# yassram/iterative-closest-point

Measured on AMD Instinct MI355X. Metric: ICP iterations/sec (synthetic 1048576-point pair, C4, exact NN), higher is better.
Workload: dtype f64 (30 exact fp64 grid searches (fp32 screen, candidates decided in fp64: the first from cell seeds, the seeded ones the fused grid iteration nn_grid_iter2_kernel, 75% of its queries kept their correspondence by the exclusion certificate without a walk); fp64 transform and reductions)

## Files before the change

### include/icp_capi.h

```cpp
#ifndef ICP_CAPI_H
#define ICP_CAPI_H

#include <stddef.h>
#include <stdint.h>

#ifdef __cplusplus
extern "C" {
#endif

#define ICP_OK 0
#define ICP_E_ARG (-1)
#define ICP_E_HIP (-2)
#define ICP_E_SIZE_MISMATCH (-3)
#define ICP_E_TOO_FEW_POINTS (-4)
#define ICP_E_NO_MODEL (-5)
#define ICP_E_RCCL (-6)
#define ICP_E_NO_DEVICE (-7)
#define ICP_E_IO (-8)
#define ICP_E_RANGE (-9)

#define ICP_NN_CERTIFIED 0
#define ICP_NN_FP64 1

#define ICP_NN_VARIANT_AUTO 0
#define ICP_NN_VARIANT_VALU 1
#define ICP_NN_VARIANT_MFMA 2
#define ICP_NN_VARIANT_MFMA16 3
#define ICP_NN_VARIANT_GRID 4
#define ICP_NN_VARIANT_BUNDLE 5

typedef struct icp_ctx icp_ctx;

typedef struct icp_result {
    int iterations;
    int converged;
    double err;
    double s;
    double R[9];
    double t[3];
} icp_result;

typedef struct icp_stats {
    double nn_ms;
    long long nn_launches;
    long long nn_pairs;
    long long ambiguous;
    long long level1_queued;
    long long level1_unrecovered;
    double iter_ms;
    long long iterations;
    long long grid_fallback;
    double allreduce_ms;
    long long allreduce_calls;
    double cert_max_err_ratio;
    double cert_min_margin;
    long long cert_audited;
    long long persistent_runs;
    long long cpu_rule_ties;
    long long cpu_rule_changed;
    long long persistent_fallbacks;
    int last_filter;
    long long bundle_builds;
    long long bundle_builds_in_run;
    long long run_bundle_searches;
    long long run_grid_searches;
    long long run_certified;
    long long run_walked;
    unsigned long long run_path_bits;
} icp_stats;
#define ICP_FILTER_VALU 0
#define ICP_FILTER_MFMA 1
#define ICP_FILTER_MFMA16 2
#define ICP_FILTER_BUNDLE 3
#define ICP_FILTER_GRID 4
#define ICP_FILTER_FP64 5
#define ICP_FILTER_ONE_LAUNCH 6

int icp_ctx_create(int device, int nn_mode, icp_ctx **out);

int icp_ctx_create_dist(int device, int nn_mode, int rank, int world_size, const void *rccl_id,
                        icp_ctx **out);
int icp_rccl_unique_id(void *out128);
typedef int (*icp_allreduce_fn)(double *buf, size_t count, void *user);
int icp_ctx_create_sharded(int device, int nn_mode, int rank, int world_size, icp_allreduce_fn fn,
                           void *user, icp_ctx **out);
void icp_ctx_destroy(icp_ctx *ctx);
const char *icp_last_error(const icp_ctx *ctx);
const char *icp_strerror(int code);
int icp_device_count(int *count);

int icp_set_model(icp_ctx *ctx, const double *m_xyz, size_t nm);
int icp_set_scene(icp_ctx *ctx, const double *p_xyz, size_t np_local, size_t np_total);
int icp_set_model_device(icp_ctx *ctx, const double *m_xyz_dev, size_t nm);
int icp_set_scene_device(icp_ctx *ctx, const double *p_xyz_dev, size_t np_local, size_t np_total);
int icp_set_model_device_stream(icp_ctx *ctx, const double *m_xyz_dev, size_t nm, void *producer);
int icp_set_scene_device_stream(icp_ctx *ctx, const double *p_xyz_dev, size_t np_local, size_t np_total,
                                void *producer);
int icp_get_scene(icp_ctx *ctx, double *p_xyz_out);
int icp_ensure_model(icp_ctx *ctx, const double *m_xyz, size_t nm, int *uploaded);
typedef void (*icp_progress_fn)(int iteration, double err, void *user);
int icp_set_progress(icp_ctx *ctx, icp_progress_fn fn, void *user);
int icp_set_allow_unequal(icp_ctx *ctx, int allow);
int icp_set_nn_variant(icp_ctx *ctx, int variant);
#define ICP_NN_RULE_SQUARED 0
#define ICP_NN_RULE_CPU_SQRT 1
int icp_set_nn_rule(icp_ctx *ctx, int rule);

#define ICP_RUN_AUTO 0
#define ICP_RUN_LAUNCHES 1
#define ICP_RUN_PERSISTENT 2
int icp_set_run_mode(icp_ctx *ctx, int mode);

int icp_set_max_distance(icp_ctx *ctx, double dmax);
int icp_get_inliers(icp_ctx *ctx, uint8_t *mask_out, long long *count_out);
int icp_get_inlier_trace(icp_ctx *ctx, long long *counts_out, size_t cap);

int icp_run(icp_ctx *ctx, int max_iter, double threshold, double *err_trace, icp_result *res);

int icp_closest_matrix(icp_ctx *ctx, const double *p_xyz, size_t np, double *y_xyz_out,
                       int32_t *idx_out);
int icp_compute_centroid(icp_ctx *ctx, const double *xyz, size_t n, double mu[3],
                         double *centred_out);
int icp_subtract_col(icp_ctx *ctx, const double *xyz, size_t n, const double m[3], double *out);
int icp_y_p_norm(icp_ctx *ctx, const double *y_xyz, const double *p_xyz, size_t n,
                 double *d_caps, double *sp);
int icp_err_compute(icp_ctx *ctx, const double *y_xyz, double *p_xyz, size_t n, int in_place,
                    const double sR[9], const double t[3], double *err);
int icp_find_alignment(icp_ctx *ctx, const double *p_xyz, const double *y_xyz, size_t n,
                       double *s, double R[9], double t[3], double *err);

int icp_horn_solve(const double S[9], const double mu_p[3], const double mu_y[3], double d_caps,
                   double sp, double *s, double R[9], double t[3]);
int icp_max_element_index(const double ev[4]);
int icp_shard_range(size_t n_total, int rank, int world_size, size_t *begin, size_t *count);
int icp_synthetic_pair(uint64_t seed, size_t n, double angle_deg, const double axis[3],
                       const double t[3], double *model_xyz_out, double *scene_xyz_out);
int icp_load_matrix(const char *path, double **xyz_out, size_t *n_out);
int icp_write_matrix(const char *path, const double *xyz, size_t n);
void icp_free(void *p);

int icp_get_indices(icp_ctx *ctx, int32_t *idx_out);
int icp_set_index_digest(icp_ctx *ctx, size_t cap);
int icp_set_cert_audit(icp_ctx *ctx, int enable);
typedef struct icp_bundle_audit_result {
    double max_err_ratio;
    double min_gap;
    long long pairs, excluded, checked, violations;
} icp_bundle_audit_result;
int icp_bundle_audit(icp_ctx *ctx, int groups, icp_bundle_audit_result *out);
int icp_get_index_digest(icp_ctx *ctx, uint64_t *out, size_t cap);

int icp_get_stats(const icp_ctx *ctx, icp_stats *out);
int icp_reset_stats(icp_ctx *ctx);
int icp_set_bundle_counters(icp_ctx *ctx, int enable);
int icp_get_bundle_counters(icp_ctx *ctx, uint64_t out[16]);
int icp_get_comm_info(icp_ctx *ctx, int *comm_count, int *comm_rank, char *bus_id, int len);
int icp_get_model_order(icp_ctx *ctx, int32_t *kd_out);
int icp_sort_pairs(int device, const uint32_t *keys, size_t n, int bits, uint32_t *keys_out, int32_t *order_out);

#ifdef __cplusplus
}
#endif
#endif
```

### iterative-closest-point_amd/csrc/icp_engine.hip

```cpp
#include <hip/hip_runtime.h>
#include <rccl/rccl.h>

#include <algorithm>
#include <chrono>
#include <thread>
#include <cmath>
#include <cstdio>
#include <climits>
#include <cstring>
#include <string>
#include <vector>

#include "icp_horn.h"
#include "icp_canon.h"
#include "icp_kernels.h"

using namespace icp;

std::vector<double> icp::persist_model_image(const double *m, size_t nm, size_t *blocks_out)
{
    std::vector<uint32_t> ord(nm);
    for (size_t j = 0; j < nm; ++j) ord[j] = (uint32_t)j;
    std::vector<std::pair<size_t, size_t>> stack{{0, nm}};
    while (!stack.empty()) {
        const auto [lo, hi] = stack.back();
        stack.pop_back();
        const size_t cnt = hi - lo;
        const size_t unit = cnt > 1024 ? 1024 : cnt > 64 ? 64 : cnt > 16 ? 16 : 0;
        if (!unit) continue;
        double bl[3] = {INFINITY, INFINITY, INFINITY}, bh[3] = {-INFINITY, -INFINITY, -INFINITY};
        for (size_t k = lo; k < hi; ++k)
            for (int a = 0; a < 3; ++a) {
                bl[a] = std::min(bl[a], m[3 * ord[k] + a]);
                bh[a] = std::max(bh[a], m[3 * ord[k] + a]);
            }
        int ax = 0;
        for (int a = 1; a < 3; ++a)
            if (bh[a] - bl[a] > bh[ax] - bl[ax]) ax = a;
        const size_t units = (cnt + unit - 1) / unit, mid = lo + unit * ((units + 1) / 2);
        if (mid >= hi) continue;
        std::nth_element(ord.begin() + lo, ord.begin() + mid, ord.begin() + hi, [&](uint32_t x, uint32_t y) {
            const double vx = m[3 * x + ax], vy = m[3 * y + ax];
            return vx < vy || (vx == vy && x < y);
        });
        stack.push_back({lo, mid});
        stack.push_back({mid, hi});
    }
    const size_t nb = (nm + 63) / 64;
    const size_t nsb = (nb + 15) / 16, nb16 = (nm + 15) / 16;
    const size_t nf32 = 6 * (nb + nb16);
    std::vector<double> img(3 * nm + 6 * nb + (nm + 1) / 2 + 6 * nsb + (nf32 + 1) / 2);
    int32_t *orig = (int32_t *)(img.data() + 3 * nm + 6 * nb);
    for (size_t k = 0; k < nm; ++k) {
        const size_t j = ord[k];
        for (int a = 0; a < 3; ++a) img[a * nm + k] = m[3 * j + a];
        orig[k] = (int32_t)j;
    }
    for (size_t b = 0; b < nb; ++b) {
        double *box = img.data() + 3 * nm + 6 * b;
        for (int a = 0; a < 3; ++a) {
            box[a] = img[a * nm + 64 * b];
            box[3 + a] = box[a];
        }
        for (size_t k = 64 * b + 1; k < std::min(nm, 64 * b + 64); ++k)
            for (int a = 0; a < 3; ++a) {
                box[a] = std::min(box[a], img[a * nm + k]);
                box[3 + a] = std::max(box[3 + a], img[a * nm + k]);
            }
    }
    double *sbox = img.data() + 3 * nm + 6 * nb + (nm + 1) / 2;
    for (size_t s = 0; s < nsb; ++s) {
        const double *first = img.data() + 3 * nm + 6 * (16 * s);
        for (int a = 0; a < 6; ++a) sbox[6 * s + a] = first[a];
        for (size_t b = 16 * s + 1; b < std::min(nb, 16 * s + 16); ++b) {
            const double *box = img.data() + 3 * nm + 6 * b;
            for (int a = 0; a < 3; ++a) {
                sbox[6 * s + a] = std::min(sbox[6 * s + a], box[a]);
                sbox[6 * s + 3 + a] = std::max(sbox[6 * s + 3 + a], box[3 + a]);
            }
        }
    }
    float *f32 = (float *)(sbox + 6 * nsb);
    auto down = [](double v) {
        float f = (float)v;
        return (double)f > v ? std::nextafter(f, -INFINITY) : f;
    };
    auto up = [](double v) {
        float f = (float)v;
        return (double)f < v ? std::nextafter(f, INFINITY) : f;
    };
    for (size_t b = 0; b < nb; ++b)
        for (int a = 0; a < 3; ++a) {
            f32[6 * b + a] = down(img[3 * nm + 6 * b + a]);
            f32[6 * b + 3 + a] = up(img[3 * nm + 6 * b + 3 + a]);
        }
    float *f16b = f32 + 6 * nb;
    for (size_t b = 0; b < nb16; ++b)
        for (int a = 0; a < 3; ++a) {
            double lo = img[a * nm + 16 * b], hi = lo;
            for (size_t k = 16 * b + 1; k < std::min(nm, 16 * b + 16); ++k) {
                lo = std::min(lo, img[a * nm + k]);
                hi = std::max(hi, img[a * nm + k]);
            }
            f16b[6 * b + a] = down(lo);
            f16b[6 * b + 3 + a] = up(hi);
        }
    *blocks_out = nb;
    return img;
}

namespace {

struct DevCloud {
    double *x = nullptr, *y = nullptr, *z = nullptr;
    float4 *f = nullptr;
    size_t n = 0, cap = 0;
};

}

struct icp_ctx {
    int device = 0;
    int nn_mode = ICP_NN_CERTIFIED;
    int rank = 0, world = 1;
    bool allow_unequal = false;
    hipStream_t st = nullptr;
    ncclComm_t comm = nullptr;
    icp_allreduce_fn host_reduce = nullptr;
    void *host_reduce_user = nullptr;
    icp_progress_fn progress_fn = nullptr;
    void *progress_user = nullptr;
    int progress_next = 0;

    DevCloud model;
    float4 *m32 = nullptr;
    float4 *mperm = nullptr;
    float *mm = nullptr;
    char *mimg16 = nullptr;
    bool mimg16_pending = false;
    float *mms16 = nullptr;
    double scale16 = 1.0;
    size_t nm = 0, nm_pad = 0, m32_cap = 0, mperm_cap = 0, mm_cap = 0, mimg16_cap = 0, mms16_cap = 0;
    int nn_variant = ICP_NN_VARIANT_AUTO;
    double c[3] = {0, 0, 0};
    std::vector<double> model_host;
    double rm = 0.0;
    double *mstat_part = nullptr, *mstat_out = nullptr, *h_mstat = nullptr;
    int *cmp_diff = nullptr;
    KdPlan kd_plan;
    char *kd_scratch = nullptr;
    size_t kd_scratch_cap = 0;
    bool has_model = false;

    DevCloud scene, Y;
    size_t np_total = 0;
    bool has_scene = false;

    DevCloud qa, qb;

    int *idx = nullptr;
    size_t idx_cap = 0;
    void *part = nullptr, *part2 = nullptr;
    size_t part_cap = 0, part2_cap = 0;
    int *amb1 = nullptr;
    size_t amb1_cap = 0;
    int *amb_count = nullptr, *amb_list = nullptr;
    double *amb_T = nullptr;
    size_t amb_cap = 0;
    GridParams grid{};
    int *g_start = nullptr;
    char *g_sort = nullptr;
    size_t g_sort_cap = 0;
    double4 *g_pts = nullptr;
    float4 *g_pts32 = nullptr;
    size_t g_pts32_cap = 0;
    size_t g_start_cap = 0, g_pts_cap = 0;
    IterState *iter_state = nullptr;
    size_t iter_state_cap = 0;
    IterState *h_iter = nullptr;
    IterState *d_iter_mirror = nullptr;
    double *h_trace = nullptr, *d_trace = nullptr;
    size_t trace_cap = 0;
    int *h_sig = nullptr, *d_sig = nullptr;
    int sig_ticket = 0;
    double *h_few = nullptr;
    double *d_few = nullptr;
    int *h_flags = nullptr;
    int *d_flags = nullptr;
    int flag_ticket = 0;
    double *err_trace_dev = nullptr;
    size_t err_trace_cap = 0;
    std::vector<hipEvent_t> iter_ev;
    unsigned long long *digest = nullptr;
    unsigned *cert_audit = nullptr;
    size_t digest_cap = 0;
    double4 *m4 = nullptr;
    size_t m4_cap = 0;
    DevCloud model_alt;
    double4 *m4_alt = nullptr;
    size_t m4_alt_cap = 0;
    hipEvent_t mstat_ev = nullptr;
    unsigned *seed16 = nullptr;
    size_t seed16_cap = 0;
    bool last_search_timed = false;
    bool seeds_valid = false;
    bool seedd_valid = false;
    int last_far = -1;
    int second_pass_items = 0;
    int last_q2 = -1;
    int *amb1_hint = nullptr, *amb_hint = nullptr;
    int *fb_list = nullptr;
    double *fb_T = nullptr;
    size_t amb1_hint_cap = 0, amb_hint_cap = 0, fb_list_cap = 0, fb_T_cap = 0;

    double *partials = nullptr;
    double *err_part = nullptr;
    size_t err_part_cap = 0;
    double *canon_rowbuf = nullptr;
    int *canon_ticket = nullptr;
    size_t canon_rowbuf_cap = 0;
    int *h_far = nullptr;
    double *sums = nullptr;
    double *h_sums = nullptr;
    int *h_amb = nullptr;
    double *stage = nullptr;
    size_t stage_cap = 0;
    double *h_io = nullptr, *d_io = nullptr;
    size_t io_cap = 0, io_off = 0;
    bool io_pending = false;

    int nn_rule = ICP_NN_RULE_SQUARED;
    CpuRuleEntry *cr_entries = nullptr;
    int *cr_count = nullptr;
    int *cr_fix = nullptr;
    size_t cr_cap = 0, cr_count_cap = 0, cr_fix_cap = 0;

    int run_mode = ICP_RUN_AUTO;
    int n_cu = 0;
    size_t lds_per_cu = 0, lds_per_block = 0;
    double *pers_part = nullptr;
    unsigned *pers_sync = nullptr;
    size_t pers_part_cap = 0, pers_sync_cap = 0;
    double *tail_part = nullptr;
    unsigned *tail_sync = nullptr;
    double *mid_q4 = nullptr;
    int *mid_res = nullptr;
    int *mid_perm = nullptr;
    char *mid_cnt = nullptr;
    double m_lo[3] = {0, 0, 0}, m_hi[3] = {0, 0, 0};
    double pm_seed_big = 0.0;
    size_t mid_q4_cap = 0, mid_res_cap = 0, mid_perm_cap = 0, mid_cnt_cap = 0;
    size_t tail_part_cap = 0, tail_sync_cap = 0;
    bool pers_sync_valid = false;
    unsigned pers_epoch_base = 0;
    int pers_grid = 0;
    unsigned long long *pers_stamps = nullptr;
    size_t pers_stamps_cap = 0;
    double *pm_img = nullptr;
    size_t pm_img_cap = 0, pm_blocks = 0;
    char *b_img = nullptr, *b_pimg = nullptr;
    int *b_kd_orig = nullptr;
    double4 *b_bctr = nullptr, *b_blk = nullptr;
    int *b_kd = nullptr;
    int nb_pad = 0;
    bool bundle_pending = false;
    size_t b_img_cap = 0, b_pimg_cap = 0, b_kd_orig_cap = 0, b_bctr_cap = 0, b_blk_cap = 0, b_kd_cap = 0;
    int *q_order = nullptr;
    int *q_pos = nullptr;
    size_t q_pos_cap = 0;
    char *q_order_tmp = nullptr;
    size_t q_order_cap = 0, q_order_tmp_cap = 0;
    const double *q_order_src = nullptr;
    size_t q_order_n = 0;
    unsigned long long *b_counters = nullptr;
    char *b_qop = nullptr, *b_gop = nullptr;
    double4 *b_qraw = nullptr;
    int *b_glist = nullptr;
    double *b_seedd = nullptr;
    size_t b_seedd_cap = 0;
    hipEvent_t order_ev = nullptr;
    int4 *cert_state = nullptr;
    size_t cert_state_cap = 0;
    unsigned long long *cert_counts = nullptr;
    size_t cert_counts_cap = 0;
    int cert_counts_rows = 0;
    char *tail_backup = nullptr;
    size_t tail_backup_cap = 0;
    double4 *b_gctr = nullptr;
    int *b_cand = nullptr, *b_cand_n = nullptr;
    int *b_wsplit = nullptr, *b_tctl = nullptr;
    int2 *b_tasks = nullptr;
    size_t b_gctr_cap = 0, b_cand_cap = 0, b_cand_n_cap = 0, b_wsplit_cap = 0, b_tctl_cap = 0, b_tasks_cap = 0;
// ... 295 lines not shown
    if (off) return ICP_OK;
    if (ctx->q_order_src != q.x || ctx->q_order_n != n) {
        TRY(grow(ctx, &ctx->q_order, &ctx->q_order_cap, n));
        TRY(grow(ctx, &ctx->q_pos, &ctx->q_pos_cap, n));
        const size_t bytes = query_order_scratch_bytes((int)n);
        TRY(grow(ctx, &ctx->q_order_tmp, &ctx->q_order_tmp_cap, bytes));
        if (launch_query_order(q.x, q.y, q.z, (int)n, ctx->m_lo, ctx->m_hi, ctx->q_order_tmp, bytes, ctx->q_order,
                               ctx->st, ctx->q_pos) != 0)
            return fail(ctx, ICP_E_HIP, "query_order: radix sort failed");
        LAUNCHCHK("query_order");
        ctx->q_order_src = q.x;
        ctx->q_order_n = n;
    }
    *order = ctx->q_order;
    return ICP_OK;
}

static bool want_slot_order(const icp_ctx *ctx, size_t n)
{
    static const bool off = [] {
        const char *e = getenv("ICP_SCENE_ORDER");
        return e && atoi(e) == 0;
    }();
    return !off && n > (size_t)kTailMaxBlocks * kBlock && ctx->nm >= (size_t)kBundleMinModel &&
           (double)n * (double)ctx->nm >= 2147483648.0;
}

static int scene_revert_now(icp_ctx *ctx)
{
    if (!ctx->scene_revert) return ICP_OK;
    DevCloud &P = ctx->scene;
    TRY(grow_cloud(ctx, ctx->s_tmp, P.n, true));
    launch_permute_cloud(ctx->s_order, (int)P.n, 1, P.x, P.y, P.z, nullptr, nullptr, ctx->s_tmp.x, ctx->s_tmp.y,
                         ctx->s_tmp.z, nullptr, nullptr, ctx->st);
    std::swap(ctx->scene, ctx->s_tmp);
    launch_make_f32(ctx->scene.x, ctx->scene.y, ctx->scene.z, ctx->scene.n, ctx->c[0], ctx->c[1], ctx->c[2],
                    ctx->scene.f, ctx->st);
    LAUNCHCHK("scene_to_file_order");
    ctx->scene_slot = false;
    ctx->scene_revert = false;
    ctx->p32_stale = false;
    return ICP_OK;
}

static int scene_to_slot_order(icp_ctx *ctx)
{
    if (ctx->scene_slot || !ctx->scene.n) return ICP_OK;
    DevCloud &P = ctx->scene;
    const size_t n = P.n;
    TRY(grow(ctx, &ctx->s_order, &ctx->s_order_cap, n));
    const size_t bytes = query_order_scratch_bytes((int)n);
    TRY(grow(ctx, &ctx->q_order_tmp, &ctx->q_order_tmp_cap, bytes));
    if (launch_query_order(P.x, P.y, P.z, (int)n, ctx->m_lo, ctx->m_hi, ctx->q_order_tmp, bytes, ctx->s_order,
                           ctx->st) != 0)
        return fail(ctx, ICP_E_HIP, "scene order: radix sort failed");
    TRY(grow_cloud(ctx, ctx->s_tmp, n, true));
    const bool with_idx = ctx->seeds_valid;
    if (with_idx) TRY(grow(ctx, &ctx->s_tmp_idx, &ctx->s_tmp_idx_cap, n));
    launch_permute_cloud(ctx->s_order, (int)n, 0, P.x, P.y, P.z, P.f, with_idx ? ctx->idx : nullptr, ctx->s_tmp.x,
                         ctx->s_tmp.y, ctx->s_tmp.z, ctx->s_tmp.f, with_idx ? ctx->s_tmp_idx : nullptr, ctx->st);
    LAUNCHCHK("scene_to_slot_order");
    std::swap(ctx->scene, ctx->s_tmp);
    if (with_idx) {
        std::swap(ctx->idx, ctx->s_tmp_idx);
        std::swap(ctx->idx_cap, ctx->s_tmp_idx_cap);
    }
    ctx->scene_slot = true;
    return ICP_OK;
}

constexpr size_t kInlineFallbackModel = 8192;

static int sum_cert_counts(const icp_ctx *ctx, long long out[2])
{
    out[0] = out[1] = 0;
    if (ctx->cert_counts_rows <= 0 || !ctx->cert_counts) return ICP_OK;
    std::vector<unsigned long long> h(2 * (size_t)ctx->cert_counts_rows);
    if (hipStreamSynchronize(ctx->st) != hipSuccess ||
        hipMemcpy(h.data(), ctx->cert_counts, h.size() * sizeof(h[0]), hipMemcpyDeviceToHost) != hipSuccess)
        return ICP_E_HIP;
    for (size_t r = 0; r < h.size(); r += 2) {
        out[0] += h[r];
        out[1] += h[r + 1];
    }
    return ICP_OK;
}

static int fold_cert_counts(icp_ctx *ctx)
{
    long long c[2];
    TRY(sum_cert_counts(ctx, c));
    ctx->stats.run_certified += c[0];
    ctx->stats.run_walked += c[1];
    ctx->cert_counts_rows = 0;
    return ICP_OK;
}

constexpr int kSeededBox = 125;
static int grid_seeded_search(icp_ctx *ctx, const DevCloud &q, size_t n, const int *stop, const double *seedd,
                              hipEvent_t ev1)
{
    TRY(grow(ctx, &ctx->amb1, &ctx->amb1_cap, n));
    TRY(grow(ctx, &ctx->amb1_hint, &ctx->amb1_hint_cap, n));
    TRY(grow(ctx, &ctx->fb_list, &ctx->fb_list_cap, n));
    TRY(grow(ctx, &ctx->fb_T, &ctx->fb_T_cap, n));
    int *kpos_out = nullptr;
    if (ctx->nn_rule == ICP_NN_RULE_SQUARED && ctx->m4kd && ctx->kd_of && ctx->nb_pad > 0) {
        TRY(grow(ctx, &ctx->kpos, &ctx->kpos_cap, n));
        kpos_out = ctx->kpos;
    }
    const bool xcd = grid_xcd() == 2 || (grid_xcd() == 1 && 4 * n <= ctx->nm);
    const DevCloud &Y = ctx->Y;
    const bool y_out = seedd && Y.x && Y.cap >= n;
    double *yx = y_out ? Y.x : nullptr, *yy = y_out ? Y.y : nullptr, *yz = y_out ? Y.z : nullptr;
    if (y_out) {
        kpos_out = nullptr;
        launch_nn_grid_seeded((int)n, q.x, q.y, q.z, grid_view(ctx), kSeededBox, seedd, ctx->m4, ctx->idx, yx, yy,
                              yz, ctx->amb_count + 2, ctx->amb1, ctx->amb1_hint, stop, xcd, ctx->st,
                              (long long)ctx->nm);
    } else {
        launch_nn_grid_resolve_all((int)n, q.x, q.y, q.z, ctx->m4, grid_view(ctx), kSeededBox, ctx->idx,
                                   ctx->amb_count + 1, ctx->fb_list, ctx->fb_T, ctx->st, stop, 0, xcd,
                                   ctx->amb_count + 2, ctx->amb1, ctx->amb1_hint, kpos_out, ctx->kd_of, seedd);
    }
    if (ev1) HIPCHK(hipEventRecord(ev1, ctx->st));
    const int sp_items = ctx->second_pass_items > 0 ? std::min(ctx->second_pass_items, 4096) : 4096;
    launch_nn_grid_resolve(ctx->amb_count + 2, (int)std::min<size_t>(n, sp_items), ctx->amb1, ctx->amb1_hint, q.x, q.y, q.z, ctx->m4,
                           grid_view(ctx), grid_budget(ctx), ctx->idx, ctx->amb_count + 1, ctx->fb_list, nullptr,
                           ctx->fb_T, ctx->st, stop, (int)ctx->nm, kpos_out, ctx->kd_of, 64, yx, yy, yz);
    LAUNCHCHK("grid_seeded_search");
    static const bool dbg_far = getenv("ICP_DEBUG_FAR") != nullptr;
    if (dbg_far) {
        int h[4];
        HIPCHK(hipMemcpy(h, ctx->amb_count, sizeof(h), hipMemcpyDeviceToHost));
        fprintf(stderr, "[far] second pass %d fallback %d\n", h[2], h[1]);
    }
    ctx->kpos_valid = kpos_out != nullptr;
    ctx->y_ready = y_out;
    return ICP_OK;
}

static int ensure_mimage16(icp_ctx *ctx)
{
    if (!ctx->mimg16_pending) return ICP_OK;
    TRY(grow(ctx, &ctx->mimg16, &ctx->mimg16_cap, ctx->nm_pad * 32));
    TRY(grow(ctx, &ctx->mms16, &ctx->mms16_cap, ctx->nm_pad));
    launch_build_mimage16(ctx->model.x, ctx->model.y, ctx->model.z, (int)ctx->nm, (int)ctx->nm_pad, ctx->c,
                          ctx->scale16, ctx->mimg16, ctx->mms16, ctx->st);
    LAUNCHCHK("build_mimage16");
    ctx->mimg16_pending = false;
    return ICP_OK;
}

static bool cell_seed_on()
{
    static const bool on = [] {
        const char *e = getenv("ICP_CELL_SEED");
        return !(e && atoi(e) == 0);
    }();
    return on;
}

static int grid_unseeded_slot(icp_ctx *ctx, const DevCloud &q, size_t n, const int *stop, hipEvent_t ev1)
{
    TRY(grow(ctx, &ctx->b_seedd, &ctx->b_seedd_cap, n));
    launch_nn_grid_cell_seed((int)n, q.x, q.y, q.z, grid_view(ctx), (int)ctx->nm, ctx->idx, ctx->b_seedd, ctx->st);
    LAUNCHCHK("nn_grid_cell_seed");
    return grid_seeded_search(ctx, q, n, stop, ctx->b_seedd, ev1);
}

struct SeedState {
    bool seedd = false;
    int seed16 = 0;
    bool records = false;
    double rec_local = -1.0;
};

int nn_search_begin(icp_ctx *ctx, const DevCloud &q, size_t n, bool seeded, hipEvent_t ev0, hipEvent_t ev1,
                    bool zero_counts = true, const SeedState *ws = nullptr, const int *stop = nullptr,
                    bool slot_order = false, bool grid_seeded = false, const double *seedd = nullptr)
{
    const SeedState none;
    const SeedState &w = ws ? *ws : none;
    TRY(grow(ctx, &ctx->idx, &ctx->idx_cap, n));
    ctx->kpos_valid = false;
    ctx->y_ready = false;
    if (!n) return ICP_OK;
    int *kpos_out = nullptr;
    const int inline_nm = ctx->nm <= (size_t)kInlineFallbackModel ? (int)ctx->nm : 0;
    TRY(ensure_queue(ctx, n));
    if (zero_counts) HIPCHK(hipMemsetAsync(ctx->amb_count, 0, sizeof(int) * 4, ctx->st));
    if (ctx->nn_mode == ICP_NN_FP64) {
        ctx->stats.last_filter = ICP_FILTER_FP64;
        const NNPlan pl = plan_nn64(n, ctx->nm);
        const size_t need = (size_t)pl.splits * n * (sizeof(double) + sizeof(int));
        TRY(grow(ctx, (char **)&ctx->part, &ctx->part_cap, need));
        double *pb = (double *)ctx->part;
        int *pi = (int *)(pb + (size_t)pl.splits * n);
        if (ev0) HIPCHK(hipEventRecord(ev0, ctx->st));
        launch_nn_fp64(q.x, q.y, q.z, (int)n, ctx->model.x, ctx->model.y, ctx->model.z, (int)ctx->nm,
                       pl, pb, pi, ctx->st, stop);
        if (ev1) HIPCHK(hipEventRecord(ev1, ctx->st));
        launch_nn_finalize64(pb, pi, pl.splits, (int)n, ctx->idx, ctx->st, stop);
        LAUNCHCHK("nn_fp64");
    } else if (seeded && slot_order && (grid_seeded || ctx->nn_variant == ICP_NN_VARIANT_GRID)) {
        ctx->stats.last_filter = ICP_FILTER_GRID;
        if (ev0) HIPCHK(hipEventRecord(ev0, ctx->st));
        TRY(grid_seeded_search(ctx, q, n, stop, seedd, ev1));
        return ICP_OK;
    } else if (ctx->nn_variant == ICP_NN_VARIANT_GRID) {
        ctx->stats.last_filter = ICP_FILTER_GRID;
        TRY(grow(ctx, &ctx->fb_list, &ctx->fb_list_cap, n));
        TRY(grow(ctx, &ctx->fb_T, &ctx->fb_T_cap, n));
        if (ev0) HIPCHK(hipEventRecord(ev0, ctx->st));
        if (!seeded && slot_order && cell_seed_on()) return grid_unseeded_slot(ctx, q, n, stop, ev1);
        if (seeded)
            launch_nn_grid_resolve_all((int)n, q.x, q.y, q.z, ctx->m4, grid_view(ctx), grid_budget(ctx), ctx->idx,
                                       ctx->amb_count + 1, ctx->fb_list, ctx->fb_T, ctx->st, stop, 0,
                                       slot_order && grid_xcd() != 0);
        else
            launch_nn_grid_search((int)n, q.x, q.y, q.z, grid_view(ctx), grid_budget(ctx), ctx->idx,
                                  ctx->amb_count + 1, ctx->fb_list, ctx->fb_T, ctx->st);
        if (ev1) HIPCHK(hipEventRecord(ev1, ctx->st));
        launch_nn_resolve(ctx->amb_count + 1, ctx->fb_list, ctx->fb_T, q.f, q.x, q.y, q.z, ctx->m32,
                          ctx->model.x, ctx->model.y, ctx->model.z, (int)ctx->nm, (int)n, ctx->idx, ctx->st,
                          stop);
        LAUNCHCHK("nn_grid_search");
    } else if (int l1 = level1_kind(ctx, n)) {
        static const bool grid_seed = [] {
            const char *e = getenv("ICP_GRID_SEED");
            return !(e && atoi(e) == 0);
        }();
        if (l1 == 3 && !seeded && !(grid_seed && ctx->g_pts)) l1 = 2;
        if (l1 == 3 && !seeded && slot_order && ctx->bundle_pending && ctx->nn_variant == ICP_NN_VARIANT_AUTO) {
            ctx->stats.last_filter = ICP_FILTER_GRID;
            TRY(grow(ctx, &ctx->fb_list, &ctx->fb_list_cap, n));
            TRY(grow(ctx, &ctx->fb_T, &ctx->fb_T_cap, n));
            if (ev0) HIPCHK(hipEventRecord(ev0, ctx->st));
            if (cell_seed_on()) return grid_unseeded_slot(ctx, q, n, stop, ev1);
            launch_nn_grid_search((int)n, q.x, q.y, q.z, grid_view(ctx), grid_budget(ctx), ctx->idx, ctx->amb_count + 1,
                                  ctx->fb_list, ctx->fb_T, ctx->st);
            if (ev1) HIPCHK(hipEventRecord(ev1, ctx->st));
            launch_nn_resolve(ctx->amb_count + 1, ctx->fb_list, ctx->fb_T, q.f, q.x, q.y, q.z, ctx->m32, ctx->model.x,
                              ctx->model.y, ctx->model.z, (int)ctx->nm, (int)n, ctx->idx, ctx->st, stop);
            LAUNCHCHK("nn_grid_search (first)");
            return ICP_OK;
        }
        if (l1 >= 2) TRY(ensure_mimage16(ctx));
        if (l1 == 3 && ctx->bundle_pending && ws) ctx->stats.bundle_builds_in_run += 1;
        if (l1 == 3) TRY(ensure_bundle(ctx));
        const bool gseed = l1 >= 2 && !seeded && grid_seed && ctx->g_pts;
        if (gseed) {
            launch_nn_grid_seed((int)n, q.x, q.y, q.z, grid_view(ctx), (int)ctx->nm, ctx->idx, ctx->st);
            LAUNCHCHK("nn_grid_seed");
        }
        const SeedState &wu = gseed ? none : w;
        const bool sd = (seeded || gseed) && l1 >= 2;
        const bool v2 = l1 == 3 && bundle_v2();
        ctx->stats.last_filter = l1 == 3 ? ICP_FILTER_BUNDLE : l1 == 2 ? ICP_FILTER_MFMA16 : ICP_FILTER_MFMA;
        const NNPlan pl = l1 == 3   ? (v2 ? plan_nn_bundle2(n, ctx->nb_pad) : plan_nn_bundle(n, ctx->nb_pad))
                          : l1 == 2 ? plan_nn_mfma16(n, ctx->nm_pad, sd)
                                    : plan_nn_mfma(n, ctx->nm_pad);
        const bool local = v2 && slot_order && ctx->b_rlmax >= 0.0 && bundle_local();
        if (local && ctx->nn_rule == ICP_NN_RULE_SQUARED && ctx->m4kd) {
            TRY(grow(ctx, &ctx->kpos, &ctx->kpos_cap, n));
            kpos_out = ctx->kpos;
        }
        const bool records_ready = v2 && wu.records && sd &&
                                   (local ? wu.rec_local >= 0.0 && wu.rec_local == ctx->b_rlmax : wu.rec_local < 0.0);
        const bool seeds_ready = local ? records_ready && wu.seed16 == 2 : wu.seed16 == 1;
        if (sd && !seeds_ready) {
            TRY(grow(ctx, &ctx->seed16, &ctx->seed16_cap, n));
            if (!local)
                launch_mfma16_seed(q.x, q.y, q.z, (int)n, ctx->idx, ctx->m4, ctx->c, ctx->scale16, ctx->seed16,
                                   ctx->st);
        }
        const unsigned *seeds = sd ? ctx->seed16 : nullptr;
        TRY(grow(ctx, (char **)&ctx->part, &ctx->part_cap,
                 (size_t)pl.splits * n * (2 * sizeof(float) + sizeof(int))));
        float *pb = (float *)ctx->part;
        float *ps = pb + (size_t)pl.splits * n;
        int *pi = (int *)(ps + (size_t)pl.splits * n);
        TRY(grow(ctx, &ctx->amb1, &ctx->amb1_cap, n));
        TRY(grow(ctx, &ctx->amb1_hint, &ctx->amb1_hint_cap, n));
        TRY(grow(ctx, &ctx->fb_list, &ctx->fb_list_cap, n));
        TRY(grow(ctx, &ctx->fb_T, &ctx->fb_T_cap, n));
        const int *order = nullptr;
        if (l1 == 3 && !slot_order) TRY(query_order(ctx, q, n, &order));
        if (v2) {
            const size_t nslots = bundle2_slots(pl);
            TRY(grow(ctx, &ctx->b_qop, &ctx->b_qop_cap, nslots * 64));
            TRY(grow(ctx, &ctx->b_qraw, &ctx->b_qraw_cap, nslots));
            TRY(grow(ctx, &ctx->b_gop, &ctx->b_gop_cap, nslots));
            TRY(grow(ctx, &ctx->b_glist, &ctx->b_glist_cap, bundle2_list_ints(pl, ctx->nb_pad)));
            TRY(grow(ctx, &ctx->b_cand, &ctx->b_cand_cap, (size_t)pl.qblocks * (ctx->nb_pad >> 5)));
            TRY(grow(ctx, &ctx->b_cand_n, &ctx->b_cand_n_cap, (size_t)pl.qblocks));
            TRY(grow(ctx, &ctx->b_wsplit, &ctx->b_wsplit_cap, (size_t)pl.qblocks));
            TRY(grow(ctx, &ctx->b_tasks, &ctx->b_tasks_cap, bundle2_task_count(pl)));
            if (ctx->b_tctl_cap < (size_t)kBundleTctlInts || !ctx->b_tctl) {
                TRY(grow(ctx, &ctx->b_tctl, &ctx->b_tctl_cap, kBundleTctlInts));
                HIPCHK(hipMemsetAsync(ctx->b_tctl, 0, sizeof(int) * kBundleTctlInts, ctx->st));
            }
            TRY(grow(ctx, &ctx->b_gctr, &ctx->b_gctr_cap, nslots / 32));
            if (ctx->b_counters && ctx->b_counters_rows < bundle2_counter_rows(pl)) {
                HIPCHK(hipFree(ctx->b_counters));
                ctx->b_counters = nullptr;
                ctx->b_counters_rows = bundle2_counter_rows(pl);
                HIPCHK(hipMalloc((void **)&ctx->b_counters,
                                 sizeof(unsigned long long) * kBundleCounterFields * ctx->b_counters_rows));
                HIPCHK(hipMemsetAsync(ctx->b_counters, 0,
                                      sizeof(unsigned long long) * kBundleCounterFields * ctx->b_counters_rows,
                                      ctx->st));
            }
            if (!records_ready) launch_bundle_prep(q.x, q.y, q.z, (int)n, order ? ctx->q_pos : nullptr, ctx->idx, ctx->m4,
                               sd && wu.seedd && ctx->b_seedd ? ctx->b_seedd : nullptr, ctx->c, ctx->scale16, sd ? ctx->seed16 : nullptr, nslots, ctx->b_qop,
                               order ? ctx->b_qraw : nullptr, ctx->st, stop, order ? nullptr : ctx->b_gop,
                               order ? nullptr : ctx->b_gctr, local ? ctx->b_rlmax : -1.0);
            if (order && !records_ready) launch_bundle_groups(ctx->b_qop, nslots, ctx->b_gop, ctx->b_gctr, ctx->st, stop);
            launch_bundle_candidates(pl, ctx->b_gctr, ctx->b_blk, ctx->nb_pad, ctx->b_cand, ctx->b_cand_n,
                                     ctx->b_wsplit, ctx->b_tasks, ctx->b_tctl, ctx->st, stop);
        }
        if (ev0) HIPCHK(hipEventRecord(ev0, ctx->st));
        if (v2)
            launch_nn_bundle2(ctx->b_qop, ctx->b_gop, (int)n, ctx->b_img, ctx->nb_pad, ctx->b_cand, ctx->b_cand_n,
                              ctx->b_tasks, ctx->b_tctl, local ? ctx->b_pimg_l : ctx->b_pimg, ctx->b_kd_orig,
                              ctx->b_glist, pl, pb, ps, pi, ctx->st, stop, ctx->b_counters,
                              local ? ctx->b_frame : nullptr);
        else if (l1 == 3)
            launch_nn_bundle(q.x, q.y, q.z, (int)n, order, ctx->idx, ctx->m4, ctx->c, ctx->scale16, seeds, ctx->b_img,
                             ctx->nb_pad, ctx->b_pimg, ctx->b_kd_orig, (int)ctx->nm, pl, pb, ps, pi, ctx->st, stop,
                             ctx->b_counters);
        else if (l1 == 2)
            launch_nn_mfma16(q.x, q.y, q.z, (int)n, ctx->c, ctx->scale16, seeds, ctx->mimg16, (int)ctx->nm_pad,
                             pl, pb, ps, pi, ctx->st, stop);
        else
            launch_nn_mfma(q.f, (int)n, ctx->mperm, (int)ctx->nm_pad, pl, pb, ps, pi, ctx->st);
        if (ev1) HIPCHK(hipEventRecord(ev1, ctx->st));
        if (l1 >= 2)
            launch_nn_finalize_mfma16(pb, ps, pi, pl.splits, q.x, q.y, q.z, (int)n, (int)ctx->nm, ctx->c,
                                      ctx->scale16, seeds, ctx->mms16, ctx->idx, ctx->amb_count + 2, ctx->amb1,
                                      ctx->amb1_hint, ctx->st, stop, ctx->m4, ctx->cert_audit,
                                      v2 && order ? ctx->b_qraw : nullptr,
                                      v2 ? ctx->b_wsplit : nullptr, v2 ? 4 * pl.q_per_lane * 32 : 0,
                                      local ? ctx->b_rlmax : -1.0, local ? ctx->b_kd_orig : nullptr, kpos_out);
        else
            launch_nn_finalize_mfma(pb, ps, pi, pl.splits, q.f, (int)n, ctx->mm, (int)ctx->nm, ctx->idx, ctx->amb_count + 2,
                                    ctx->amb1, ctx->amb1_hint, ctx->st);
        launch_nn_grid_resolve(ctx->amb_count + 2, (int)n, ctx->amb1, ctx->amb1_hint, q.x, q.y, q.z, ctx->m4,
                               grid_view(ctx), grid_budget(ctx), ctx->idx, ctx->amb_count + 1, ctx->fb_list, nullptr,
                               ctx->fb_T, ctx->st, stop, inline_nm, kpos_out, ctx->kd_of);
        if (!inline_nm)
            launch_nn_resolve(ctx->amb_count + 1, ctx->fb_list, ctx->fb_T, q.f, q.x, q.y, q.z, ctx->m32,
                              ctx->model.x, ctx->model.y, ctx->model.z, (int)ctx->nm, (int)n, ctx->idx, ctx->st,
                              stop, kpos_out, ctx->kd_of);
        LAUNCHCHK("nn_mfma");
        ctx->kpos_valid = kpos_out != nullptr;
    } else {
        ctx->stats.last_filter = ICP_FILTER_VALU;
        const NNPlan pl = plan_nn32(n, ctx->nm_pad);
        const size_t need = (size_t)pl.splits * n * (2 * sizeof(float) + sizeof(int));
        TRY(grow(ctx, (char **)&ctx->part, &ctx->part_cap, need));
        float *pb = (float *)ctx->part;
        float *ps = pb + (size_t)pl.splits * n;
        int *pi = (int *)(ps + (size_t)pl.splits * n);
        TRY(grow(ctx, &ctx->amb_hint, &ctx->amb_hint_cap, n));
        TRY(grow(ctx, &ctx->fb_list, &ctx->fb_list_cap, n));
        TRY(grow(ctx, &ctx->fb_T, &ctx->fb_T_cap, n));
        if (ev0) HIPCHK(hipEventRecord(ev0, ctx->st));
        launch_nn_filter(q.f, (int)n, ctx->m32, (int)ctx->nm_pad, pl, pb, ps, pi, ctx->st, stop);
        if (ev1) HIPCHK(hipEventRecord(ev1, ctx->st));
        CertParams cp{ctx->rm, (int)ctx->nm};
        launch_nn_finalize(pb, ps, pi, pl.splits, q.f, (int)n, cp, ctx->idx, ctx->amb_count, ctx->amb_list,
                           ctx->amb_T, ctx->amb_hint, ctx->st, stop);
        launch_nn_grid_resolve(ctx->amb_count, (int)n, ctx->amb_list, ctx->amb_hint, q.x, q.y, q.z, ctx->m4,
                               grid_view(ctx), grid_budget(ctx), ctx->idx, ctx->amb_count + 1, ctx->fb_list,
                               ctx->amb_T, ctx->fb_T, ctx->st, stop, inline_nm);
        if (!inline_nm)
            launch_nn_resolve(ctx->amb_count + 1, ctx->fb_list, ctx->fb_T, q.f, q.x, q.y, q.z, ctx->m32,
                              ctx->model.x, ctx->model.y, ctx->model.z, (int)ctx->nm, (int)n, ctx->idx, ctx->st,
                              stop);
        LAUNCHCHK("nn_certified");
    }
    return ICP_OK;
}

int nn_counts_to_host(icp_ctx *ctx)
{
    HIPCHK(hipMemcpyAsync(ctx->h_amb, ctx->amb_count, sizeof(int) * 4, hipMemcpyDeviceToHost, ctx->st));
    return ICP_OK;
}

constexpr double kTimedPairs = 4294967296.0;

int nn_search(icp_ctx *ctx, const DevCloud &q, size_t n)
{
    ctx->last_search_timed = n && (double)n * (double)ctx->nm >= kTimedPairs;
    TRY(nn_search_begin(ctx, q, n, false, ctx->last_search_timed ? ctx->ev[0] : nullptr,
                        ctx->last_search_timed ? ctx->ev[1] : nullptr));
    return n ? nn_counts_to_host(ctx) : ICP_OK;
}

static double (*volatile g_libm_pow)(double, double) = std::pow;
static double cpu_rule_distance(const double q[3], const double *m)
{
    const double dx = q[0] - m[0], dy = q[1] - m[1], dz = q[2] - m[2];
    const double t = (g_libm_pow(dx, 2.0) + g_libm_pow(dy, 2.0)) + g_libm_pow(dz, 2.0);
    return std::sqrt(t);
}

int cpu_rule_fixup(icp_ctx *ctx, const DevCloud &q, size_t n, const int *stop)
{
    if (ctx->nn_rule != ICP_NN_RULE_CPU_SQRT || n == 0) return ICP_OK;
    TRY(grow(ctx, &ctx->cr_count, &ctx->cr_count_cap, 1));
    size_t want = std::min<size_t>(n, 4096);
    for (int pass = 0; pass < 2; ++pass) {
        TRY(grow(ctx, &ctx->cr_entries, &ctx->cr_cap, want));
        HIPCHK(hipMemsetAsync(ctx->cr_count, 0, sizeof(int), ctx->st));
        launch_nn_cpu_rule_window((int)n, q.x, q.y, q.z, ctx->m4, grid_view(ctx), grid_budget(ctx), ctx->idx,
                                  ctx->cr_count, ctx->cr_entries, (int)ctx->cr_cap, ctx->st, stop);
        LAUNCHCHK("nn_cpu_rule_window");
        int cnt = 0;
        HIPCHK(hipMemcpyAsync(&cnt, ctx->cr_count, sizeof(int), hipMemcpyDeviceToHost, ctx->st));
        HIPCHK(hipStreamSynchronize(ctx->st));
        if ((size_t)cnt > ctx->cr_cap) {
            want = (size_t)cnt;
            continue;
        }
        if (cnt == 0) return ICP_OK;
        std::vector<CpuRuleEntry> h((size_t)cnt);
        HIPCHK(hipMemcpyAsync(h.data(), ctx->cr_entries, sizeof(CpuRuleEntry) * (size_t)cnt,
                              hipMemcpyDeviceToHost, ctx->st));
        HIPCHK(hipStreamSynchronize(ctx->st));
        const double *m = nullptr;
        TRY(model_host_copy(ctx, &m));
        std::vector<int> cand;
        std::vector<int> changed;
        for (const CpuRuleEntry &e : h) {
            cand.clear();
            if (e.n >= 0) {
                cand.assign(e.cand, e.cand + e.n);
                std::sort(cand.begin(), cand.end());
            } else {
                cand.resize(ctx->nm);
                for (size_t k = 0; k < ctx->nm; ++k) cand[k] = (int)k;
            }
            int best = cand.empty() ? e.h : cand[0];
            double bd = cand.empty() ? 0.0 : cpu_rule_distance(e.q, m + 3 * (size_t)best);
            for (size_t c = 1; c < cand.size(); ++c) {
                const double d = cpu_rule_distance(e.q, m + 3 * (size_t)cand[c]);
                if (d < bd) {
                    bd = d;
                    best = cand[c];
                }
            }
            ctx->stats.cpu_rule_ties += 1;
            if (best != e.h) {
                ctx->stats.cpu_rule_changed += 1;
                changed.push_back(e.j);
                changed.push_back(best);
            }
        }
        if (!changed.empty()) {
            const size_t npairs = changed.size() / 2;
            TRY(grow(ctx, &ctx->cr_fix, &ctx->cr_fix_cap, changed.size()));
            HIPCHK(hipMemcpyAsync(ctx->cr_fix, changed.data(), sizeof(int) * changed.size(), hipMemcpyHostToDevice,
                                  ctx->st));
            launch_scatter_pairs(ctx->cr_fix, (int)npairs, ctx->idx, ctx->st);
            LAUNCHCHK("scatter_pairs");
            HIPCHK(hipStreamSynchronize(ctx->st));
        }
        return ICP_OK;
    }
    return fail(ctx, ICP_E_HIP, "cpu_rule_fixup: the near-tie list kept growing");
}

void account_nn(icp_ctx *ctx, size_t n)
{
    float ms = 0.f;
    if (ctx->last_search_timed) {
        if (hipEventElapsedTime(&ms, ctx->ev[0], ctx->ev[1]) == hipSuccess) {
            ctx->stats.nn_ms += ms;
            ctx->stats.nn_launches += 1;
        } else {
            (void)hipGetLastError();
        }
    }
    ctx->stats.nn_pairs += (long long)n * (long long)ctx->nm;
    if (ctx->nn_mode == ICP_NN_CERTIFIED && n) {
        ctx->stats.ambiguous += ctx->h_amb[0];
        ctx->stats.grid_fallback += ctx->h_amb[1];
        ctx->stats.level1_queued += ctx->h_amb[2];
        ctx->stats.level1_unrecovered += ctx->h_amb[3];
    }
}

int allreduce(icp_ctx *ctx, double *buf, size_t count)
{
    if (ctx->comm) {
        RCCLCHK(ncclAllReduce(buf, buf, count, ncclDouble, ncclSum, ctx->comm, ctx->st));
        return ICP_OK;
    }
    if (ctx->world <= 1) return ICP_OK;
    if (!ctx->host_reduce) return fail(ctx, ICP_E_ARG, "world_size > 1 without a communicator");
    double tmp[32];
    HIPCHK(hipMemcpyAsync(tmp, buf, sizeof(double) * count, hipMemcpyDeviceToHost, ctx->st));
    HIPCHK(hipStreamSynchronize(ctx->st));
    if (ctx->host_reduce(tmp, count, ctx->host_reduce_user) != 0)
        return fail(ctx, ICP_E_RCCL, "host all-reduce callback failed");
    HIPCHK(hipMemcpyAsync(buf, tmp, sizeof(double) * count, hipMemcpyHostToDevice, ctx->st));
    HIPCHK(hipStreamSynchronize(ctx->st));
    return ICP_OK;
}

static int global_count(icp_ctx *ctx, int *v)
{
    if (!ctx->comm && ctx->world <= 1) return ICP_OK;
    double x = (double)*v;
    HIPCHK(hipMemcpyAsync(ctx->sums + kSumFar + 1, &x, sizeof(double), hipMemcpyHostToDevice, ctx->st));
    TRY(allreduce(ctx, ctx->sums + kSumFar + 1, 1));
    HIPCHK(hipMemcpyAsync(&x, ctx->sums + kSumFar + 1, sizeof(double), hipMemcpyDeviceToHost, ctx->st));
// ... 256 lines not shown
                    (void *)ctx->s_order, (void *)ctx->s_tmp_idx, (void *)ctx->b_pimg_l, (void *)ctx->b_frame,
                    (void *)ctx->m4kd, (void *)ctx->kd_of, (void *)ctx->kpos, (void *)ctx->canon_rowbuf,
                    (void *)ctx->canon_ticket, (void *)ctx->cert_state, (void *)ctx->cert_counts,
                    (void *)ctx->gate_mask, (void *)ctx->gate_flags, (void *)ctx->gate_part, (void *)ctx->gate_state})
        if (p) (void)hipFree(p);
    if (ctx->h_sums) (void)hipHostFree(ctx->h_sums);
    if (ctx->h_amb) (void)hipHostFree(ctx->h_amb);
    if (ctx->h_iter) (void)hipHostFree(ctx->h_iter);
    if (ctx->h_flags) (void)hipHostFree(ctx->h_flags);
    if (ctx->h_far) (void)hipHostFree(ctx->h_far);
    if (ctx->h_gate) (void)hipHostFree(ctx->h_gate);
    if (ctx->h_ktrace) (void)hipHostFree(ctx->h_ktrace);
    if (ctx->h_few) (void)hipHostFree(ctx->h_few);
    if (ctx->h_sig) (void)hipHostFree(ctx->h_sig);
    if (ctx->h_trace) (void)hipHostFree(ctx->h_trace);
    if (ctx->h_io) (void)hipHostFree(ctx->h_io);
    for (auto e : ctx->iter_ev) (void)hipEventDestroy(e);
    if (ctx->order_ev) (void)hipEventDestroy(ctx->order_ev);
    if (ctx->mstat_ev) (void)hipEventDestroy(ctx->mstat_ev);
    for (auto &e : ctx->ev)
        if (e) (void)hipEventDestroy(e);
    if (ctx->st) (void)hipStreamDestroy(ctx->st);
    delete ctx;
}

const char *icp_last_error(const icp_ctx *ctx) { return ctx ? ctx->err.c_str() : "null context"; }

int icp_set_nn_variant(icp_ctx *ctx, int variant)
{
    if (!ctx || variant < ICP_NN_VARIANT_AUTO || variant > ICP_NN_VARIANT_BUNDLE) return ICP_E_ARG;
    ctx->nn_variant = variant;
    return ICP_OK;
}

int icp_set_nn_rule(icp_ctx *ctx, int rule)
{
    if (!ctx || (rule != ICP_NN_RULE_SQUARED && rule != ICP_NN_RULE_CPU_SQRT)) return ICP_E_ARG;
    ctx->nn_rule = rule;
    return ICP_OK;
}

int icp_set_run_mode(icp_ctx *ctx, int mode)
{
    if (!ctx || mode < ICP_RUN_AUTO || mode > ICP_RUN_PERSISTENT) return ICP_E_ARG;
    ctx->run_mode = mode;
    return ICP_OK;
}

int icp_set_progress(icp_ctx *ctx, icp_progress_fn fn, void *user)
{
    if (!ctx) return ICP_E_ARG;
    ctx->progress_fn = fn;
    ctx->progress_user = user;
    return ICP_OK;
}

int icp_set_allow_unequal(icp_ctx *ctx, int allow)
{
    if (!ctx) return ICP_E_ARG;
    ctx->allow_unequal = allow != 0;
    return ICP_OK;
}

int icp_set_max_distance(icp_ctx *ctx, double dmax)
{
    if (!ctx || std::isnan(dmax) || dmax < 0.0) return ICP_E_ARG;
    ctx->gate_dmax = std::isinf(dmax) ? 0.0 : dmax;
    return ICP_OK;
}

int icp_get_inliers(icp_ctx *ctx, uint8_t *mask_out, long long *count_out)
{
    if (!ctx) return ICP_E_ARG;
    if (!ctx->has_scene || !ctx->gate_have)
        return fail(ctx, ICP_E_NO_MODEL, "no gated icp_run since icp_set_scene (icp_set_max_distance)");
    HIPCHK(hipSetDevice(ctx->device));
    if (mask_out && ctx->scene.n) {
        HIPCHK(hipMemcpyAsync(mask_out, ctx->gate_flags, ctx->scene.n, hipMemcpyDeviceToHost, ctx->st));
        HIPCHK(hipStreamSynchronize(ctx->st));
    }
    if (count_out) *count_out = ctx->h_gate->K;
    return ICP_OK;
}

int icp_get_inlier_trace(icp_ctx *ctx, long long *counts_out, size_t cap)
{
    if (!ctx || (!counts_out && cap)) return ICP_E_ARG;
    if (!ctx->has_scene || !ctx->gate_have)
        return fail(ctx, ICP_E_NO_MODEL, "no gated icp_run since icp_set_scene (icp_set_max_distance)");
    const size_t k = std::min(cap, (size_t)ctx->gate_iters);
    if (k) std::memcpy(counts_out, ctx->h_ktrace, sizeof(long long) * k);
    return ctx->gate_iters;
}

static int stage_model(icp_ctx *ctx, const double *m_xyz, size_t nm)
{
    TRY(grow(ctx, &ctx->stage, &ctx->stage_cap, 3 * nm));
    HIPCHK(hipMemcpyAsync(ctx->stage, m_xyz, sizeof(double) * 3 * nm, hipMemcpyHostToDevice, ctx->st));
    return ICP_OK;
}

static bool kd_host()
{
    static const bool on = [] {
        const char *e = getenv("ICP_KD_HOST");
        return e && atoi(e) == 1;
    }();
    return on;
}

static int set_model_staged(icp_ctx *ctx, const double *m_xyz, size_t nm, const double *aos_dev = nullptr,
                            bool stream_ordered = false)
{
    const double *aos = aos_dev ? aos_dev : ctx->stage;
    if (!ctx->mstat_part) {
        HIPCHK(hipMalloc((void **)&ctx->mstat_part, sizeof(double) * model_stats_scratch_doubles()));
        HIPCHK(hipMalloc((void **)&ctx->mstat_out, sizeof(double) * 16));
        HIPCHK(hipHostMalloc((void **)&ctx->h_mstat, sizeof(double) * 16, hipHostMallocDefault));
    }
    launch_model_stats(aos, (int)nm, ctx->mstat_part, ctx->mstat_out, ctx->st);
    LAUNCHCHK("model_stats");
    HIPCHK(hipMemcpyAsync(ctx->h_mstat, ctx->mstat_out, sizeof(double) * 10, hipMemcpyDeviceToHost, ctx->st));
    if (!ctx->mstat_ev) HIPCHK(hipEventCreateWithFlags(&ctx->mstat_ev, hipEventDisableTiming));
    HIPCHK(hipEventRecord(ctx->mstat_ev, ctx->st));
    TRY(grow_cloud(ctx, ctx->model_alt, nm, true));
    TRY(grow(ctx, &ctx->m4_alt, &ctx->m4_alt_cap, nm));
    launch_aos_to_soa4(aos, nm, ctx->model_alt.x, ctx->model_alt.y, ctx->model_alt.z, ctx->m4_alt, ctx->st);
    LAUNCHCHK("aos_to_soa4");
    HIPCHK(hipEventSynchronize(ctx->mstat_ev));
    if (ctx->h_mstat[9] != 0.0) return fail(ctx, ICP_E_RANGE, "model has non-finite coordinates");
    double c[3], lo[3], hi[3];
    for (int k = 0; k < 3; ++k) {
        c[k] = ctx->h_mstat[k] / (double)nm;
        lo[k] = ctx->h_mstat[3 + k];
        hi[k] = ctx->h_mstat[6 + k];
    }
    double rm = 0.0, rm64 = 0.0;
    for (int k = 0; k < 3; ++k)
        for (const double v : {lo[k], hi[k]}) {
            const double d = v - c[k];
            const float f = (float)d;
            if (!std::isfinite(f)) return fail(ctx, ICP_E_RANGE, "model has non-finite coordinates");
            rm = std::max(rm, std::fabs((double)f));
            rm64 = std::max(rm64, std::fabs(d));
        }
    if (rm > 1e15) return fail(ctx, ICP_E_RANGE, "model coordinates exceed 1e15 around the centroid");
    ctx->has_model = false;
    for (int k = 0; k < 3; ++k) ctx->c[k] = c[k];
    ctx->rm = rm;
    const size_t nm_pad = (nm + kTile32 - 1) / kTile32 * kTile32;
    std::swap(ctx->model, ctx->model_alt);
    std::swap(ctx->m4, ctx->m4_alt);
    std::swap(ctx->m4_cap, ctx->m4_alt_cap);
    TRY(grow(ctx, &ctx->m32, &ctx->m32_cap, nm_pad));
    TRY(grow(ctx, &ctx->mperm, &ctx->mperm_cap, nm_pad));
    TRY(grow(ctx, &ctx->mm, &ctx->mm_cap, nm_pad));
    launch_model_f32_images(aos, (int)nm, (int)nm_pad, ctx->c, ctx->m32, (float *)ctx->mperm, ctx->mm, ctx->st);
    LAUNCHCHK("model_f32_images");
    ctx->scale16 = rm64 > 0.0 ? std::ldexp(1.0, (int)std::floor(std::log2(4096.0 / rm64))) : 1.0;
    while (rm64 * ctx->scale16 >= 4096.0) ctx->scale16 *= 0.5;
    ctx->mimg16_pending = true;
    ctx->grid = grid_params_box(lo, hi, nm);
    const long long ncell = grid_cells(ctx->grid);
    TRY(grow(ctx, &ctx->g_start, &ctx->g_start_cap, (size_t)ncell + 1));
    TRY(grow(ctx, &ctx->g_pts, &ctx->g_pts_cap, nm));
    TRY(grow(ctx, &ctx->g_pts32, &ctx->g_pts32_cap, nm));
    const size_t gbytes = grid_build_scratch_bytes((int)nm, ncell);
    TRY(grow(ctx, &ctx->g_sort, &ctx->g_sort_cap, gbytes));
    if (launch_grid_build(ctx->model.x, ctx->model.y, ctx->model.z, ctx->m4, (int)nm, ctx->grid, ctx->g_sort, gbytes,
                          ctx->g_start, ctx->g_pts, ctx->g_pts32, ctx->st) != 0)
        return fail(ctx, ICP_E_HIP, "grid build: radix sort failed");
    LAUNCHCHK("grid_build");
    for (int k = 0; k < 3; ++k) {
        ctx->m_lo[k] = lo[k];
        ctx->m_hi[k] = hi[k];
    }
    ctx->nb_pad = 0;
    ctx->b_rlmax = -1.0;
    std::vector<int> kd_h;
    ctx->bundle_pending = false;
    if (nm >= (size_t)kBundleMinModel) {
        if (kd_host()) {
            kd_h = bundle_kd_order(m_xyz, nm);
            TRY(build_bundle(ctx, nm, kd_h.data()));
        } else {
            ctx->bundle_pending = true;
        }
    }
    std::vector<double> pm;
    if (nm <= (size_t)std::max(kPersistMaxModel, kPersistMidMaxModel)) {
        pm = persist_model_image(m_xyz, nm, &ctx->pm_blocks);
        TRY(grow(ctx, &ctx->pm_img, &ctx->pm_img_cap, pm.size()));
        HIPCHK(hipMemcpyAsync(ctx->pm_img, pm.data(), sizeof(double) * pm.size(), hipMemcpyHostToDevice, ctx->st));
        {
            const size_t nb16 = (nm + 15) / 16;
            std::vector<double> d2(nb16);
            for (size_t b = 0; b < nb16; ++b) {
                double acc = 0.0;
                for (int k = 0; k < 3; ++k) {
                    double blo = pm[k * nm + 16 * b], bhi = blo;
                    for (size_t j = 16 * b + 1; j < std::min(nm, 16 * b + 16); ++j) {
                        blo = std::min(blo, pm[k * nm + j]);
                        bhi = std::max(bhi, pm[k * nm + j]);
                    }
                    acc += (bhi - blo) * (bhi - blo);
                }
                d2[b] = acc;
            }
            std::nth_element(d2.begin(), d2.begin() + nb16 / 2, d2.end());
            ctx->pm_seed_big = 4.0 * d2[nb16 / 2];
        }
    }
    if (!stream_ordered || !pm.empty() || !kd_h.empty()) HIPCHK(hipStreamSynchronize(ctx->st));
    if (nm <= (size_t)std::max(kPersistMaxModel, kPersistMidMaxModel) || ctx->nn_rule == ICP_NN_RULE_CPU_SQRT)
        ctx->model_host.assign(m_xyz, m_xyz + 3 * nm);
    else
        std::vector<double>().swap(ctx->model_host);
    ctx->nm = nm;
    ctx->nm_pad = nm_pad;
    ctx->has_model = true;
    ctx->seeds_valid = false;
    ctx->seedd_valid = false;
    if (ctx->has_scene && ctx->scene.n && ctx->scene_slot) ctx->scene_revert = true;
    if (ctx->has_scene && ctx->scene.n && !ctx->scene_revert) {
        launch_make_f32(ctx->scene.x, ctx->scene.y, ctx->scene.z, ctx->scene.n, ctx->c[0], ctx->c[1],
                        ctx->c[2], ctx->scene.f, ctx->st);
        LAUNCHCHK("make_f32");
        ctx->p32_stale = false;
        if (!stream_ordered) HIPCHK(hipStreamSynchronize(ctx->st));
    }
    return ICP_OK;
}

int icp_set_model(icp_ctx *ctx, const double *m_xyz, size_t nm)
{
    if (!ctx || (!m_xyz && nm) || nm == 0) return ICP_E_ARG;
    if (nm > (size_t)0x7fffffff - kTile32) return fail(ctx, ICP_E_ARG, "model too large");
    HIPCHK(hipSetDevice(ctx->device));
    TRY(stage_model(ctx, m_xyz, nm));
    return set_model_staged(ctx, m_xyz, nm);
}

static bool model_needs_host(const icp_ctx *ctx, size_t nm)
{
    return nm <= (size_t)std::max(kPersistMaxModel, kPersistMidMaxModel) || kd_host() ||
           ctx->nn_rule == ICP_NN_RULE_CPU_SQRT;
}

static int order_after_producer(icp_ctx *ctx, void *producer, bool any_stream)
{
    if (any_stream) {
        HIPCHK(hipDeviceSynchronize());
        return ICP_OK;
    }
    if (!ctx->order_ev) HIPCHK(hipEventCreateWithFlags(&ctx->order_ev, hipEventDisableTiming));
    HIPCHK(hipEventRecord(ctx->order_ev, (hipStream_t)producer));
    HIPCHK(hipStreamWaitEvent(ctx->st, ctx->order_ev, 0));
    return ICP_OK;
}

static int set_model_device_impl(icp_ctx *ctx, const double *m_xyz_dev, size_t nm, void *producer, bool any_stream)
{
    if (!ctx || !m_xyz_dev || nm == 0) return ICP_E_ARG;
    if (nm > (size_t)0x7fffffff - kTile32) return fail(ctx, ICP_E_ARG, "model too large");
    HIPCHK(hipSetDevice(ctx->device));
    TRY(order_after_producer(ctx, producer, any_stream));
    std::vector<double> host;
    if (model_needs_host(ctx, nm)) {
        host.resize(3 * nm);
        HIPCHK(hipMemcpyAsync(host.data(), m_xyz_dev, sizeof(double) * 3 * nm, hipMemcpyDeviceToHost, ctx->st));
        HIPCHK(hipStreamSynchronize(ctx->st));
    }
    return set_model_staged(ctx, host.empty() ? nullptr : host.data(), nm, m_xyz_dev, !any_stream);
}

int icp_set_model_device(icp_ctx *ctx, const double *m_xyz_dev, size_t nm)
{
    return set_model_device_impl(ctx, m_xyz_dev, nm, nullptr, true);
}

int icp_set_model_device_stream(icp_ctx *ctx, const double *m_xyz_dev, size_t nm, void *producer)
{
    return set_model_device_impl(ctx, m_xyz_dev, nm, producer, false);
}

int icp_ensure_model(icp_ctx *ctx, const double *m_xyz, size_t nm, int *uploaded)
{
    if (!ctx || !m_xyz || nm == 0) return ICP_E_ARG;
    if (uploaded) *uploaded = 0;
    if (nm > (size_t)0x7fffffff - kTile32) return fail(ctx, ICP_E_ARG, "model too large");
    HIPCHK(hipSetDevice(ctx->device));
    if (ctx->has_model && ctx->nm == nm) {
        if (ctx->model_host.size() == 3 * nm) {
            if (std::memcmp(ctx->model_host.data(), m_xyz, sizeof(double) * 3 * nm) == 0) return ICP_OK;
        } else {
            if (!ctx->cmp_diff) HIPCHK(hipMalloc((void **)&ctx->cmp_diff, sizeof(int)));
            TRY(stage_model(ctx, m_xyz, nm));
            HIPCHK(hipMemsetAsync(ctx->cmp_diff, 0, sizeof(int), ctx->st));
            launch_model_compare(ctx->stage, (int)nm, ctx->model.x, ctx->model.y, ctx->model.z, ctx->cmp_diff,
                                 ctx->st);
            LAUNCHCHK("model_compare");
            int diff = 0;
            HIPCHK(hipMemcpyAsync(&diff, ctx->cmp_diff, sizeof(int), hipMemcpyDeviceToHost, ctx->st));
            HIPCHK(hipStreamSynchronize(ctx->st));
            if (diff == 0) return ICP_OK;
            TRY(set_model_staged(ctx, m_xyz, nm));
            if (uploaded) *uploaded = 1;
            return ICP_OK;
        }
    }
    TRY(icp_set_model(ctx, m_xyz, nm));
// ... 1542 lines not shown
    for (int k = 0; k < 9; ++k) sR[k] = *s * R[k];
    Xform xf;
    std::memcpy(xf.sR, sR, sizeof(sR));
    std::memcpy(xf.t, t, sizeof(xf.t));
    std::memcpy(xf.c, ctx->c, sizeof(xf.c));
    launch_transform_err(ctx->qb.x, ctx->qb.y, ctx->qb.z, ctx->qa.x, ctx->qa.y, ctx->qa.z, (int)n, xf,
                         0, nullptr, red_target(ctx, n, ctx->sums + kSumErr), ctx->st);
    red_finish(ctx, n, 1, ctx->sums + kSumErr);
    LAUNCHCHK("find_alignment err");
    HIPCHK(hipMemcpyAsync(ctx->h_sums + kSumErr, ctx->sums + kSumErr, sizeof(double),
                          hipMemcpyDeviceToHost, ctx->st));
    HIPCHK(hipStreamSynchronize(ctx->st));
    *err = ctx->h_sums[kSumErr];
    return ICP_OK;
}

int icp_get_indices(icp_ctx *ctx, int32_t *idx_out)
{
    if (!ctx || (!idx_out && ctx->scene.n)) return ICP_E_ARG;
    if (!ctx->has_scene || !ctx->seeds_valid)
        return fail(ctx, ICP_E_NO_MODEL, "no NN search over the resident scene since icp_set_scene");
    HIPCHK(hipSetDevice(ctx->device));
    const int *src = ctx->idx;
    if (ctx->scene_slot && ctx->scene.n) {
        TRY(grow(ctx, &ctx->s_tmp_idx, &ctx->s_tmp_idx_cap, ctx->scene.n));
        launch_permute_cloud(ctx->s_order, (int)ctx->scene.n, 1, nullptr, nullptr, nullptr, nullptr, ctx->idx, nullptr,
                             nullptr, nullptr, nullptr, ctx->s_tmp_idx, ctx->st);
        LAUNCHCHK("indices_to_file_order");
        src = ctx->s_tmp_idx;
    }
    if (ctx->scene.n)
        HIPCHK(hipMemcpyAsync(idx_out, src, sizeof(int32_t) * ctx->scene.n, hipMemcpyDeviceToHost, ctx->st));
    HIPCHK(hipStreamSynchronize(ctx->st));
    return ICP_OK;
}

int icp_set_index_digest(icp_ctx *ctx, size_t cap)
{
    if (!ctx) return ICP_E_ARG;
    HIPCHK(hipSetDevice(ctx->device));
    if (cap) {
        size_t have = ctx->digest ? ctx->digest_cap : 0;
        if (have < cap) {
            if (ctx->digest) HIPCHK(hipFree(ctx->digest));
            ctx->digest = nullptr;
            HIPCHK(hipMalloc((void **)&ctx->digest, sizeof(unsigned long long) * 3 * cap));
        }
        HIPCHK(hipMemsetAsync(ctx->digest, 0, sizeof(unsigned long long) * 3 * cap, ctx->st));
        HIPCHK(hipStreamSynchronize(ctx->st));
    }
    ctx->digest_cap = cap;
    return ICP_OK;
}

int icp_get_index_digest(icp_ctx *ctx, uint64_t *out, size_t cap)
{
    if (!ctx || !out || cap > ctx->digest_cap) return ICP_E_ARG;
    if (!cap) return ICP_OK;
    HIPCHK(hipSetDevice(ctx->device));
    HIPCHK(hipMemcpyAsync(out, ctx->digest, sizeof(uint64_t) * 3 * cap, hipMemcpyDeviceToHost, ctx->st));
    HIPCHK(hipStreamSynchronize(ctx->st));
    return ICP_OK;
}

static int cert_audit_reset(icp_ctx *ctx)
{
    const unsigned init[3] = {0u, 0x7f800000u, 0u};
    HIPCHK(hipMemcpyAsync(ctx->cert_audit, init, sizeof(init), hipMemcpyHostToDevice, ctx->st));
    HIPCHK(hipStreamSynchronize(ctx->st));
    return ICP_OK;
}

int icp_set_cert_audit(icp_ctx *ctx, int enable)
{
    if (!ctx) return ICP_E_ARG;
    HIPCHK(hipSetDevice(ctx->device));
    HIPCHK(hipStreamSynchronize(ctx->st));
    if (!enable) {
        if (ctx->cert_audit) HIPCHK(hipFree(ctx->cert_audit));
        ctx->cert_audit = nullptr;
        return ICP_OK;
    }
    if (!ctx->cert_audit) HIPCHK(hipMalloc((void **)&ctx->cert_audit, 4 * sizeof(unsigned)));
    return cert_audit_reset(ctx);
}

int icp_bundle_audit(icp_ctx *ctx, int groups, icp_bundle_audit_result *out)
{
    if (!ctx || !out || groups < 1) return ICP_E_ARG;
    HIPCHK(hipSetDevice(ctx->device));
    const DevCloud &P = ctx->scene;
    TRY(ensure_bundle(ctx));
    if (!ctx->b_img || !ctx->b_bctr || !ctx->b_kd_orig || ctx->nb_pad <= 0 || !P.n || !ctx->seeds_valid)
        return fail(ctx, ICP_E_NO_MODEL, "icp_bundle_audit: needs the bundle images and a scene with correspondences");
    unsigned long long *buf = nullptr;
    HIPCHK(hipMalloc((void **)&buf, 6 * sizeof(unsigned long long)));
    const double inf = INFINITY;
    unsigned long long init[6] = {0ull, 0ull, 0ull, 0ull, 0ull, 0ull};
    std::memcpy(&init[1], &inf, sizeof(double));
    int rc = ICP_OK;
    if (hipMemcpyAsync(buf, init, sizeof(init), hipMemcpyHostToDevice, ctx->st) != hipSuccess) rc = ICP_E_HIP;
    if (rc == ICP_OK) {
        launch_bundle_audit(P.x, P.y, P.z, ctx->idx, ctx->m4, (int)P.n, groups, ctx->b_img, ctx->b_bctr, ctx->b_kd_orig,
                            (int)ctx->nm, ctx->nb_pad, ctx->c, ctx->scale16, buf, buf + 2, ctx->st);
        unsigned long long h[6];
        if (hipGetLastError() != hipSuccess ||
            hipMemcpyAsync(h, buf, sizeof(h), hipMemcpyDeviceToHost, ctx->st) != hipSuccess ||
            hipStreamSynchronize(ctx->st) != hipSuccess) {
            rc = ICP_E_HIP;
        } else {
            std::memcpy(&out->max_err_ratio, &h[0], sizeof(double));
            std::memcpy(&out->min_gap, &h[1], sizeof(double));
            out->pairs = (long long)h[2];
            out->excluded = (long long)h[3];
            out->violations = (long long)h[4];
            out->checked = (long long)h[5];
        }
    }
    (void)hipFree(buf);
    return rc == ICP_OK ? ICP_OK : fail(ctx, rc, "icp_bundle_audit: HIP error");
}

int icp_get_model_order(icp_ctx *ctx, int32_t *kd_out)
{
    if (!ctx || !kd_out) return ICP_E_ARG;
    HIPCHK(hipSetDevice(ctx->device));
    if (ctx->has_model) TRY(ensure_bundle(ctx));
    if (!ctx->has_model || ctx->nb_pad <= 0 || !ctx->b_kd) return fail(ctx, ICP_E_NO_MODEL, "no bundle kd order");
    HIPCHK(hipMemcpyAsync(kd_out, ctx->b_kd, sizeof(int32_t) * ctx->nm, hipMemcpyDeviceToHost, ctx->st));
    HIPCHK(hipStreamSynchronize(ctx->st));
    return ICP_OK;
}

int icp_sort_pairs(int device, const uint32_t *keys, size_t n, int bits, uint32_t *keys_out, int32_t *order_out)
{
    if (bits < 0 || bits > 32 || n > (size_t)INT_MAX || (n && (!keys || !order_out))) return ICP_E_ARG;
    if (n == 0) return ICP_OK;
    if (hipSetDevice(device) != hipSuccess) return ICP_E_HIP;
    size_t temp = 0;
    (void)icp::sort_pairs_u32(nullptr, temp, nullptr, nullptr, nullptr, nullptr, (int)n, bits, nullptr);
    char *buf = nullptr;
    const size_t kb = ((n * 4 + 255) & ~(size_t)255);
    if (hipMalloc(&buf, 3 * kb + temp) != hipSuccess) return ICP_E_HIP;
    unsigned *k0 = (unsigned *)buf, *k1 = (unsigned *)(buf + kb);
    int *v1 = (int *)(buf + 2 * kb);
    bool ok = hipMemcpy(k0, keys, n * 4, hipMemcpyHostToDevice) == hipSuccess &&
              icp::sort_pairs_u32(buf + 3 * kb, temp, k0, k1, nullptr, v1, (int)n, bits, nullptr) == hipSuccess &&
              hipMemcpy(order_out, v1, n * 4, hipMemcpyDeviceToHost) == hipSuccess &&
              (!keys_out || hipMemcpy(keys_out, k1, n * 4, hipMemcpyDeviceToHost) == hipSuccess);
    ok = hipFree(buf) == hipSuccess && ok;
    return ok ? ICP_OK : ICP_E_HIP;
}

int icp_get_stats(const icp_ctx *ctx, icp_stats *out)
{
    if (!ctx || !out) return ICP_E_ARG;
    *out = ctx->stats;
    long long cc[2];
    if (sum_cert_counts(ctx, cc) != ICP_OK) return ICP_E_HIP;
    out->run_certified += cc[0];
    out->run_walked += cc[1];
    out->cert_max_err_ratio = -1.0;
    out->cert_min_margin = -1.0;
    out->cert_audited = 0;
    if (ctx->cert_audit) {
        unsigned a[3] = {0, 0, 0};
        if (hipStreamSynchronize(ctx->st) != hipSuccess ||
            hipMemcpy(a, ctx->cert_audit, sizeof(a), hipMemcpyDeviceToHost) != hipSuccess)
            return ICP_E_HIP;
        float r, mg;
        std::memcpy(&r, &a[0], 4);
        std::memcpy(&mg, &a[1], 4);
        out->cert_max_err_ratio = r;
        out->cert_min_margin = mg;
        out->cert_audited = a[2];
    }
    return ICP_OK;
}

int icp_reset_stats(icp_ctx *ctx)
{
    if (!ctx) return ICP_E_ARG;
    HIPCHK(hipSetDevice(ctx->device));
    if (ctx->cert_audit) TRY(cert_audit_reset(ctx));
    ctx->stats = icp_stats{};
    ctx->cert_counts_rows = 0;
    ctx->stats.last_filter = -1;
    return ICP_OK;
}

}
```

### iterative-closest-point_amd/csrc/icp_grid.hip

```cpp
#include <hip/hip_runtime.h>

#include <algorithm>
#include <cmath>
#include <cstdlib>
#include <string>
#include <type_traits>

#include "icp_canon.h"
#include "icp_device.h"
#include "icp_gridbox.h"
#include "icp_kernels.h"

namespace icp {
namespace {

__device__ __forceinline__ double d64g(double px, double py, double pz, double mx, double my,
                                       double mz)
{
    const double dx = px - mx;
    const double dy = py - my;
    const double dz = pz - mz;
    return (dx * dx + dy * dy) + dz * dz;
}


__global__ __launch_bounds__(kBlock) void grid_keys_kernel(const double *__restrict__ mx, const double *__restrict__ my,
                                                         const double *__restrict__ mz, int nm, GridView gv,
                                                         unsigned *__restrict__ key, int *__restrict__ val)
{
    const int i = blockIdx.x * kBlock + threadIdx.x;
    if (i >= nm) return;
    const int cx = cell1(mx[i], gv.lo[0], gv.inv_h, gv.g[0]);
    const int cy = cell1(my[i], gv.lo[1], gv.inv_h, gv.g[1]);
    const int cz = cell1(mz[i], gv.lo[2], gv.inv_h, gv.g[2]);
    key[i] = (unsigned)((cz * gv.g[1] + cy) * gv.g[0] + cx);
    val[i] = i;
}

__global__ __launch_bounds__(kBlock) void grid_starts_kernel(const unsigned *__restrict__ skey, int nm, int ncell,
                                                           int *__restrict__ start)
{
    const int c = blockIdx.x * kBlock + threadIdx.x;
    if (c > ncell) return;
    int lo = 0, hi = nm;
    while (lo < hi) {
        const int mid = (lo + hi) >> 1;
        if (skey[mid] < (unsigned)c) lo = mid + 1;
        else hi = mid;
    }
    start[c] = lo;
}

__global__ __launch_bounds__(kBlock) void grid_gather_kernel(const double4 *__restrict__ m4, int nm,
                                                           const int *__restrict__ sval, double4 *__restrict__ pts,
                                                           float4 *__restrict__ pts32, double c0, double c1, double c2)
{
    const int k = blockIdx.x * kBlock + threadIdx.x;
    if (k >= nm) return;
    const int i = sval[k];
    const double4 m = m4[i];
    const double x = m.x, y = m.y, z = m.z;
    pts[k] = make_double4(x, y, z, (double)i);
    if (pts32) pts32[k] = make_float4((float)(x - c0), (float)(y - c1), (float)(z - c2), __int_as_float(i));
}

#ifndef ICP_CELL_SEED_RUN
#define ICP_CELL_SEED_RUN 1
#endif

__device__ __forceinline__ void lex_min(double &best, int &bi, double d, int mi)
{
    if (d < best || (d == best && (unsigned)mi < (unsigned)bi)) {
        best = d;
        bi = mi;
    }
}

constexpr int kGroup = 16;

template <int G = kGroup>
__device__ __forceinline__ void scan_box(const double q[3], const int c0[3], const int c1[3], const GridView &gv,
                                         int sub, double &best, int &bi)
{
    const int ny = c1[1] - c0[1] + 1;
    const int nrows = ny * (c1[2] - c0[2] + 1);
    for (int r = sub; r < nrows; r += G) {
        const int cy = c0[1] + r % ny, cz = c0[2] + r / ny;
        const int row = (cz * gv.g[1] + cy) * gv.g[0];
        const int k1 = gv.start[row + c1[0] + 1];
        for (int k = gv.start[row + c0[0]]; k < k1; ++k) {
            const double4 m = gv.pts[k];
            lex_min(best, bi, d64g(q[0], q[1], q[2], m.x, m.y, m.z), (int)m.w);
        }
    }
}

template <int G>
__device__ __forceinline__ void scan_box_flat(const double q[3], const int c0[3], const int c1[3],
                                              const GridView &gv, int sub, double &best, int &bi)
{
    constexpr int kU = 4;
    const int ny = c1[1] - c0[1] + 1;
    const int nrows = ny * (c1[2] - c0[2] + 1);
    for (int r0 = 0; r0 < nrows; r0 += G) {
        int k0 = 0, len = 0;
        const int r = r0 + sub;
        if (r < nrows) {
            const int cy = c0[1] + r % ny, cz = c0[2] + r / ny;
            const int row = (cz * gv.g[1] + cy) * gv.g[0];
            k0 = gv.start[row + c0[0]];
            len = gv.start[row + c1[0] + 1] - k0;
        }
        int incl = len;
#pragma unroll
        for (int o = 1; o < G; o <<= 1) {
            const int v = __shfl_up(incl, o, G);
            if (sub >= o) incl += v;
        }
        const int total = __shfl(incl, G - 1, G);
        const int base = k0 - (incl - len);
        for (int b = 0; b < total; b += kU * G) {
            int k[kU];
#pragma unroll
            for (int u = 0; u < kU; ++u) {
                const int f = b + u * G + sub;
                int pos = 0;
#pragma unroll
                for (int step = G / 2; step >= 1; step >>= 1)
                    if (__shfl(incl, pos + step - 1, G) <= f) pos += step;
                const int kb = __shfl(base, pos, G);
                k[u] = f < total ? kb + f : -1;
            }
            double4 m[kU];
#pragma unroll
            for (int u = 0; u < kU; ++u)
                if (k[u] >= 0) m[u] = gv.pts[k[u]];
#pragma unroll
            for (int u = 0; u < kU; ++u)
                if (k[u] >= 0) lex_min(best, bi, d64g(q[0], q[1], q[2], m[u].x, m[u].y, m[u].z), (int)m[u].w);
        }
    }
}

template <int G>
__device__ __forceinline__ void scan_box_batched(const double q[3], const int c0[3], const int c1[3],
                                                 const GridView &gv, int sub, double &best, int &bi)
{
    constexpr int kR = 8, kU = 4;
    const int ny = c1[1] - c0[1] + 1;
    const int nrows = ny * (c1[2] - c0[2] + 1);
    for (int r0 = sub; r0 < nrows; r0 += kR * G) {
        int k0[kR], k1[kR];
#pragma unroll
        for (int u = 0; u < kR; ++u) {
            const int r = r0 + u * G;
            k0[u] = 0;
            k1[u] = 0;
            if (r < nrows) {
                const int cy = c0[1] + r % ny, cz = c0[2] + r / ny;
                const int row = (cz * gv.g[1] + cy) * gv.g[0];
                k0[u] = gv.start[row + c0[0]];
                k1[u] = gv.start[row + c1[0] + 1];
            }
        }
#pragma unroll
        for (int u = 0; u < kR; ++u)
            for (int k = k0[u]; k < k1[u]; k += kU) {
                double4 m[kU];
#pragma unroll
                for (int v = 0; v < kU; ++v)
                    if (k + v < k1[u]) m[v] = gv.pts[k + v];
#pragma unroll
                for (int v = 0; v < kU; ++v)
                    if (k + v < k1[u]) lex_min(best, bi, d64g(q[0], q[1], q[2], m[v].x, m[v].y, m[v].z), (int)m[v].w);
            }
    }
}

template <int G, bool FLAT>
__device__ __forceinline__ void scan_box_sel(const double q[3], const int c0[3], const int c1[3],
                                             const GridView &gv, int sub, double &best, int &bi)
{
    if constexpr (FLAT) scan_box_flat<G>(q, c0, c1, gv, sub, best, bi);
    else scan_box_batched<G>(q, c0, c1, gv, sub, best, bi);
}

template <int G = kGroup> __device__ __forceinline__ void group_lex_min(double &best, int &bi)
{
#pragma unroll
    for (int o = G / 2; o >= 1; o >>= 1) {
        const double ob = __shfl_xor(best, o, G);
        const int oi = __shfl_xor(bi, o, G);
        lex_min(best, bi, ob, oi);
    }
}


__device__ __forceinline__ bool trim_row(const double q[3], double best, const GridView &gv, int cy, int cz,
                                         int &x0, int &x1)
{
    float tq[3];
    bool on = true;
#pragma unroll
    for (int a = 0; a < 3; ++a) {
        double qa = q[a];
        asm volatile("" : "+v"(qa));
        const double t = (qa - gv.lo[a]) * gv.inv_h;
        on = on && fabs(t) <= 8192.0;
        tq[a] = (float)t;
    }
// ... 1585 lines not shown
    }();
    const int R = canon_rows((size_t)n);
    static const int xcd_env = [] {
        const char *e = getenv("ICP_ITER_XCD_L");
        return e ? atoi(e) : -2;
    }();
    const int xcd_l = xcd_env != -2 ? xcd_env : (canon_chunks((size_t)n) >= 8192 ? 32 : -1);
    static const bool v2 = [] {
        const char *e = getenv("ICP_ITER_V2");
        return !(e && e[0] == '0');
    }();
    if (v2 && !stage && !(wide_on && n <= kIterWideMax) && (!dbg || ICP_ITER2_DBG)) {
        static const int ch = [] {
            const char *e = getenv("ICP_ITER2_CH");
            return e && atoi(e) == 1 ? 1 : 2;
        }();
        static const int nwg = [] {
            const char *e = getenv("ICP_ITER2_NWG");
            return e && atoi(e) == 4 ? 4 : ICP_ITER2_NWG_DEFAULT;
        }();
        const int S = canon_strands((size_t)n);
        if (strands) *strands = nwg == 1 ? S : 0;
        const Iter2Args ka{n,      px, py, pz,   yx,      yy,     yz,        idx,   st_dev, p32, gv, box,
                           budget, nm, m4, rows, far_acc, far_d2, big_count, xform, xcd_l,  ca,  dbg};
        static const bool a32_on = [] {
            const char *e = getenv("ICP_ITER2_A32");
            return !(e && e[0] == '0');
        }();
        const bool a32 = a32_on && iter2_addr32(n, nm, gv);
        auto launch = [&](auto chc, auto nwgc, auto a32c) {
            constexpr int kCh = decltype(chc)::value, kNwg = decltype(nwgc)::value;
            nn_grid_iter2_kernel<ICP_ITER2_KR, ICP_ITER2_KU, kCh, kNwg, decltype(a32c)::value>
                <<<kNwg == 1 ? S : R, 64 * kNwg, 0, st>>>(ka);
        };
        auto with_a32 = [&](auto chc, auto nwgc) {
            if (a32) launch(chc, nwgc, std::true_type{});
            else launch(chc, nwgc, std::false_type{});
        };
        using I1 = std::integral_constant<int, 1>;
        using I2 = std::integral_constant<int, 2>;
        using I4 = std::integral_constant<int, 4>;
        if (ch == 2 && nwg == 1) with_a32(I2{}, I1{});
        else if (ch == 2) with_a32(I2{}, I4{});
        else if (nwg == 1) with_a32(I1{}, I1{});
        else with_a32(I1{}, I4{});
        return ca.state != nullptr;
    }
    if (!stage && wide_on && n <= kIterWideMax)
        nn_grid_iter_kernel<false, 4><<<R, 2 * kBlock, 0, st>>>(n, px, py, pz, yx, yy, yz, idx, st_dev, p32, gv, box,
                                                                 budget, nm, m4, rows, far_acc, far_d2, big_count, dbg, xform, xcd_l);
    else if (stage)
        nn_grid_iter_kernel<true, 2><<<R, kBlock, 0, st>>>(n, px, py, pz, yx, yy, yz, idx, st_dev, p32, gv, box,
                                                            budget, nm, m4, rows, far_acc, far_d2, big_count, dbg, xform, xcd_l);
    else
        nn_grid_iter_kernel<false, 2><<<R, kBlock, 0, st>>>(n, px, py, pz, yx, yy, yz, idx, st_dev, p32, gv, box,
                                                             budget, nm, m4, rows, far_acc, far_d2, big_count, dbg, xform, xcd_l);
    return false;
}

namespace {
}

GridParams grid_params(const double *m_xyz, size_t nm)
{
    double lo[3] = {INFINITY, INFINITY, INFINITY}, hi[3] = {-INFINITY, -INFINITY, -INFINITY};
    for (size_t j = 0; j < nm; ++j)
        for (int a = 0; a < 3; ++a) {
            lo[a] = std::min(lo[a], m_xyz[3 * j + a]);
            hi[a] = std::max(hi[a], m_xyz[3 * j + a]);
        }
    return grid_params_box(lo, hi, nm);
}

GridParams grid_params_box(const double lo[3], const double hi[3], size_t nm)
{
    GridParams p{};
    double ext[3], emax = 0.0;
    for (int a = 0; a < 3; ++a) {
        ext[a] = hi[a] - lo[a];
        emax = std::max(emax, ext[a]);
        p.lo[a] = lo[a];
        p.c32[a] = lo[a] + 0.5 * ext[a];
    }
    p.em32 = std::isfinite(emax) ? std::ldexp(emax, -23) : INFINITY;
    if (!(emax > 0.0) || !std::isfinite(emax)) {
        p.g[0] = p.g[1] = p.g[2] = 1;
        p.inv_h = 1.0;
        return p;
    }
    static const double ppc = [] {
        const char *e = getenv("ICP_GRID_PPC");
        const double v = e ? atof(e) : 0.0;
        return v > 0.0 ? v : 2.0;
    }();
    double vol = 1.0;
    for (int a = 0; a < 3; ++a) vol *= std::max(ext[a], emax * 1e-3);
    double h = std::cbrt(vol * ppc / (double)std::max<size_t>(nm, 1));
    auto dims = [&](double hh, int g[3]) {
        long long tot = 1;
        for (int a = 0; a < 3; ++a) {
            g[a] = (int)std::min<double>(std::floor(ext[a] / hh) + 1.0, 1 << 12);
            tot *= g[a];
        }
        return tot;
    };
    while (dims(h, p.g) > kGridMaxCells) h *= 1.25;
    p.inv_h = 1.0 / h;
    return p;
}

static bool grid_flat_scan(int g)
{
    static const int forced = [] {
        const char *e = getenv("ICP_GRID_SCAN");
        if (!e) return -1;
        return std::string(e) == "rows" ? 0 : (std::string(e) == "flat" ? 1 : -1);
    }();
    return forced >= 0 ? forced == 1 : g >= 16;
}

long long grid_cells(const GridParams &p) { return (long long)p.g[0] * p.g[1] * p.g[2]; }

static int cell_bits(long long ncell)
{
    int bits = 1;
    while (bits < 32 && (1ll << bits) <= ncell) ++bits;
    return bits;
}

static size_t grid_keys_bytes(int nm) { return (4 * (size_t)nm * sizeof(int) + 255) & ~(size_t)255; }

size_t grid_build_scratch_bytes(int nm, long long ncell)
{
    size_t temp = 0;
    (void)sort_pairs_u32(nullptr, temp, nullptr, nullptr, nullptr, nullptr, nm, cell_bits(ncell), nullptr);
    return grid_keys_bytes(nm) + ((temp + 255) & ~(size_t)255);
}

int launch_grid_build(const double *mx, const double *my, const double *mz, const double4 *m4, int nm,
                      const GridParams &p, void *scratch, size_t bytes, int *start, double4 *pts, float4 *pts32,
                      hipStream_t st)
{
    const long long ncell = grid_cells(p);
    GridView gv{};
    for (int a = 0; a < 3; ++a) {
        gv.g[a] = p.g[a];
        gv.lo[a] = p.lo[a];
    }
    gv.inv_h = p.inv_h;
    unsigned *k0 = (unsigned *)scratch, *k1 = k0 + nm;
    int *v0 = (int *)(k1 + nm), *v1 = v0 + nm;
    size_t temp_bytes = bytes - grid_keys_bytes(nm);
    const int g = (nm + kBlock - 1) / kBlock;
    grid_keys_kernel<<<g, kBlock, 0, st>>>(mx, my, mz, nm, gv, k0, v0);
    if (sort_pairs_u32((char *)scratch + grid_keys_bytes(nm), temp_bytes, k0, k1, v0, v1, nm, cell_bits(ncell), st) !=
        hipSuccess)
        return -1;
    grid_starts_kernel<<<(int)((ncell + kBlock) / kBlock), kBlock, 0, st>>>(k1, nm, (int)ncell, start);
    grid_gather_kernel<<<g, kBlock, 0, st>>>(m4, nm, v1, pts, pts32, p.c32[0], p.c32[1], p.c32[2]);
    return 0;
}

void launch_nn_grid_search(int np, const double *px, const double *py, const double *pz, const GridView &gv,
                           int budget, int *idx, int *fb_count, int *fb_list, double *fb_T, hipStream_t st)
{
    static const int forced = [] {
        const char *e = getenv("ICP_GRID_GROUP");
        return e ? atoi(e) : 0;
    }();
    const int g = forced == 4 || forced == 16 ? forced : (np >= (1 << 16) ? 4 : 16);
    const int per_block = kBlock / g;
    const int blocks = std::max(1, std::min((np + per_block - 1) / per_block, 16384));
#define SEARCH(GG, F) nn_grid_search_kernel<GG, F><<<blocks, kBlock, 0, st>>>(np, px, py, pz, gv, budget, idx, fb_count, fb_list, fb_T)
    if (grid_flat_scan(g)) {
        if (g == 4) SEARCH(4, true);
        else SEARCH(16, true);
    } else {
        if (g == 4) SEARCH(4, false);
        else SEARCH(16, false);
    }
#undef SEARCH
}

void launch_nn_grid_cell_seed(int n, const double *px, const double *py, const double *pz, const GridView &gv, int nm,
                              int *idx, double *seedd, hipStream_t st, double *yx, double *yy, double *yz)
{
    if (n <= 0) return;
    nn_grid_cell_seed_kernel<<<(n + kBlock - 1) / kBlock, kBlock, 0, st>>>(n, px, py, pz, gv, nm, idx, seedd, yx, yy,
                                                                          yz);
}

void launch_nn_grid_seed(int np, const double *px, const double *py, const double *pz, const GridView &gv,
                         int nm, int *idx, hipStream_t st)
{
    constexpr int kG = 4, kMaxRing = 2;
    const int per_block = kBlock / kG;
    const int blocks = std::max(1, std::min((np + per_block - 1) / per_block, 16384));
    if (grid_flat_scan(kG)) nn_grid_seed_kernel<kG, true><<<blocks, kBlock, 0, st>>>(np, px, py, pz, gv, kMaxRing, nm, idx);
    else nn_grid_seed_kernel<kG, false><<<blocks, kBlock, 0, st>>>(np, px, py, pz, gv, kMaxRing, nm, idx);
}

void launch_nn_grid_resolve(const int *count_ptr, int max_items, const int *list, const int *hint,
                            const double *px, const double *py, const double *pz, const double4 *m4,
                            const GridView &gv, int budget, int *idx, int *fb_count, int *fb_list,
                            const double *T_in, double *T_out, hipStream_t st, const int *stop, int inline_nm,
                            int *kpos, const int *kd_of, int group, double *yx, double *yy, double *yz)
{
    static const int forced = [] {
        const char *e = getenv("ICP_GRID_RGROUP");
        return e ? atoi(e) : 0;
    }();
    const int g = forced == 4 || forced == 16 || forced == 64 ? forced
                  : group == 4 || group == 16 || group == 64 ? group
                                                             : (max_items >= 8192 && max_items < (1 << 18) ? 64 : 16);
    const int per_block = kBlock / g;
    static const int cap = [] {
        const char *e = getenv("ICP_GRID_RBLOCKS");
        return e && atoi(e) > 0 ? atoi(e) : 4096;
    }();
    const int blocks = std::max(1, std::min((max_items + per_block - 1) / per_block, cap));
#define RESOLVE(GG, F)                                                                                  \
    nn_grid_resolve_kernel<GG, F><<<blocks, kBlock, 0, st>>>(count_ptr, list, hint, px, py, pz, m4, gv, budget, idx, \
                                                             fb_count, fb_list, T_in, T_out, stop, inline_nm, 0, \
                                                             kpos, kd_of, 0, nullptr, nullptr, nullptr, nullptr, yx, yy, yz)
    if (grid_flat_scan(g)) {
        if (g == 4) RESOLVE(4, true);
        else if (g == 64) RESOLVE(64, true);
        else RESOLVE(16, true);
    } else {
        if (g == 4) RESOLVE(4, false);
        else if (g == 64) RESOLVE(64, false);
        else RESOLVE(16, false);
    }
#undef RESOLVE
}

void launch_nn_grid_resolve_all(int n, const double *px, const double *py, const double *pz, const double4 *m4,
                                const GridView &gv, int budget, int *idx, int *fb_count, int *fb_list, double *fb_T,
                                hipStream_t st, const int *stop, int inline_nm, bool xcd_remap, int *far_count,
                                int *far_list, int *far_hint, int *kpos, const int *kd_of, const double *seedd)
{
    static const int forced = [] {
        const char *e = getenv("ICP_GRID_GROUP");
        return e ? atoi(e) : 0;
    }();
    const int g = forced == 4 || forced == 16 ? forced : (n >= (1 << 16) ? 4 : 16);
    const int per_block = kBlock / g;
    int blocks = std::max(1, std::min((n + per_block - 1) / per_block, 16384));
    if (xcd_remap) blocks = (blocks + 7) / 8 * 8;
#define RESOLVE_ALL(GG, F)                                                                                       \
    nn_grid_resolve_kernel<GG, F><<<blocks, kBlock, 0, st>>>(nullptr, nullptr, nullptr, px, py, pz, m4, gv, budget, \
                                                             idx, fb_count, fb_list, nullptr, fb_T, stop, inline_nm, n, \
                                                             kpos, kd_of, xcd_remap ? 1 : 0, far_count, far_list, far_hint, \
                                                             seedd, nullptr, nullptr, nullptr)
    if (grid_flat_scan(g)) {
        if (g == 4) RESOLVE_ALL(4, true);
        else RESOLVE_ALL(16, true);
    } else {
        if (g == 4) RESOLVE_ALL(4, false);
        else RESOLVE_ALL(16, false);
    }
#undef RESOLVE_ALL
}

void launch_nn_grid_seeded(int n, const double *px, const double *py, const double *pz, const GridView &gv,
                           int budget, const double *seedd, const double4 *m4, int *idx, double *yx, double *yy,
                           double *yz, int *far_count, int *far_list, int *far_hint, const int *stop, bool xcd_remap,
                           hipStream_t st, long long nm_hint)
{
    struct Form {
        const char *name;
        int g;
    };
    static const Form forms[] = {{"2,2,2", 2}, {"4,2,2", 4}, {"4,2,4", 4}, {"2,2,4", 2},  {"f2,2,4", 2},
                                 {"f2,2,2", 2}, {"f4,2,4", 4}, {"f2,4,4", 2}, {"f4,2,2", 4}, {"4,1,2", 4},
                                 {"f4,1,2", 4}};
    int forced = -1;
    if (const char *e = getenv("ICP_GRID_SEEDED"))
        for (int i = 0; i < (int)(sizeof(forms) / sizeof(forms[0])); ++i)
            if (std::string(e) == forms[i].name) forced = i;
    const int form = forced >= 0 ? forced : (n >= (1 << 19) && nm_hint < 2 * (long long)n) ? 0 : 1;
    static const int xcd_env = [] {
        const char *e = getenv("ICP_SEEDED_XCD_L");
        return e ? atoi(e) : -2;
    }();
    const int xcd_l = xcd_env != -2 ? xcd_env : xcd_remap ? -1 : 32;
    const int f = form >= 4 && form != 9 && !gv.pts32 ? 0 : form;
    const int per_block = kBlock / forms[f].g;
    int blocks = std::max(1, std::min((n + per_block - 1) / per_block, 16384));
    if (xcd_remap) blocks = (blocks + 7) / 8 * 8;
    const char *te = getenv("ICP_GRID_TRIM");
    const int trim = te ? (std::string(te) == "1" ? 1 : 0) : (f == 0 ? 1 : 0);
#define SEEDED(K, ...)                                                                                       \
    K<__VA_ARGS__><<<blocks, kBlock, 0, st>>>(n, px, py, pz, gv, budget, seedd, m4, idx, yx, yy, yz, far_count, \
                                              far_list, far_hint, stop, xcd_l, trim)
    static const int seeded_tb = [] {
        const char *e = getenv("ICP_SEEDED_TB");
        return e ? atoi(e) : 0;
    }();
    if (f == 0 && (seeded_tb == 64 || (seeded_tb != 256 && !xcd_remap))) {
        int b64 = std::max(1, std::min((n + 64 / 2 - 1) / (64 / 2), 65536));
        if (xcd_remap) b64 = (b64 + 7) / 8 * 8;
        nn_grid_seeded_kernel<2, 2, 2, 1, 64><<<b64, 64, 0, st>>>(n, px, py, pz, gv, budget, seedd, m4, idx, yx, yy, yz,
                                                                  far_count, far_list, far_hint, stop, xcd_l, trim);
        return;
    }
    switch (f) {
    case 1: SEEDED(nn_grid_seeded_kernel, 4, 2, 2, 1); break;
    case 2: SEEDED(nn_grid_seeded_kernel, 4, 2, 4, 1); break;
    case 3: SEEDED(nn_grid_seeded_kernel, 2, 2, 4, 1); break;
    case 4: SEEDED(nn_grid_seeded32_kernel, 2, 2, 4); break;
    case 5: SEEDED(nn_grid_seeded32_kernel, 2, 2, 2); break;
// ... 95 lines not shown
```

### iterative-closest-point_amd/csrc/icp_kernels.h

```cpp
#pragma once

#include <hip/hip_runtime.h>

#include "icp_internal.h"

namespace icp {

#if defined(__HIP_DEVICE_COMPILE__) || defined(__HIPCC__)
__device__ __forceinline__ int wave_append(int *counter, bool pred)
{
    const unsigned long long mask = __ballot(pred);
    if (mask == 0ull) return -1;
    const int lane = (int)(threadIdx.x & 63);
    const int leader = __ffsll((long long)mask) - 1;
    int base = 0;
    if (lane == leader) base = atomicAdd(counter, __popcll(mask));
    base = __shfl(base, leader, 64);
    return pred ? base + __popcll(mask & ((1ull << lane) - 1ull)) : -1;
}

__device__ __forceinline__ int block_append(int *counter, bool pred, int *counter2 = nullptr, bool pred2 = false)
{
    __shared__ int s_cnt[kBlock / 64], s_cnt2[kBlock / 64], s_base;
    const int lane = (int)(threadIdx.x & 63), wave = (int)(threadIdx.x >> 6);
// ... 339 lines not shown
void launch_canon_fold(const double *rows, int n, double *sums, int mode, const CanonStep &cs, hipStream_t st,
                       int strands = 0);
struct GridView;
struct CertArgs {
    int4 *state = nullptr;
    int valid = 0;
    int two = 1;
    double skin = 0.0;
    unsigned long long *counts = nullptr;
};
bool launch_nn_grid_iter(int n, double *px, double *py, double *pz, double *yx, double *yy, double *yz, int *idx,
                         const IterState *st_dev, float4 *p32, const GridView &gv, int box, int budget, int nm,
                         const double4 *m4, double *rows, int *far_acc, double far_d2, int *big_count, hipStream_t st,
                         unsigned long long *dbg = nullptr,
                         int xform = 1,
                         const CertArgs &ca = CertArgs{},
                         int *strands = nullptr);
void launch_shifted_moments(const int *idx, const double4 *m4, const double *px, const double *py,
                            const double *pz, int n, double *yx, double *yy, double *yz, const IterState *st_dev,
                            double *partials, hipStream_t st, const int *kpos = nullptr,
                            const double4 *m4kd = nullptr, bool y_ready = false,
                            const StepFold &fold = StepFold{});
void launch_reduce_horn(const double *partials, int nblocks, double *sums, double n_total, const double c[3],
                        int shifted, int *amb_count, IterState *st_dev, hipStream_t st);
void launch_horn_step(const double *sums, double n_total, const double c[3], int shifted, int *amb_count,
                      IterState *st_dev, hipStream_t st);
void launch_err_horn_step(double *sums, double n_total, double threshold, int max_iter, double *err_trace,
                          IterState *st_dev, int *hflag_dev, int ticket, IterState *h_state_dev, double *h_trace_dev,
                          const double c[3], int shifted, int *amb_count, hipStream_t st,
                          int far_sum = 0);
void launch_err_step(double *sums, double n_total, double threshold, int max_iter, double *err_trace,
                     IterState *st_dev, int *hflag_dev, int ticket, IterState *h_state_dev, double *h_trace_dev,
                     hipStream_t st, const double *partials = nullptr, int nblocks = 0);
void launch_iteration_tail_small(const int *idx, const double4 *m4, double *px, double *py, double *pz, int n,
                                 double *yx, double *yy, double *yz, float4 *p32, double *sums, double n_total,
                                 const double c[3], int *amb_count, IterState *st_dev, double threshold,
                                 int max_iter, double *err_trace, int *hflag_dev, int ticket,
                                 IterState *h_state_dev, double *h_trace_dev, hipStream_t st);
constexpr size_t kPersistLdsMax = 160 * 1024 - 12 * 1024;
constexpr int kPersistMaxModel = (int)(kPersistLdsMax / 24);
struct PersistArgs {
    const double *img;
    int nblk, nm, n;
    double *px, *py, *pz, *yx, *yy, *yz;
    float4 *p32;
    int *idx;
    double *part;
    unsigned *sync;
    int *h_abort;
    double N, c0, c1, c2, threshold;
    int max_iter;
    double *err_trace;
    IterState *s_glob;
    IterState *h_state;
    double *h_trace;
    unsigned long long *stamps;
    int cull;
    double m0[3];
    unsigned epoch_base;
    int *h_epochs;
    const int *seed_idx;
    const double4 *m4;
    double *q4;
    int *res;
    const int *perm;
    int test_abort;
    double seed_big;
};
size_t mid_order_scratch_bytes(int n);
int launch_mid_order(const double *px, const double *py, const double *pz, int n, const double lo[3],
                     const double hi[3], void *scratch, size_t bytes, int *pos, hipStream_t st);
constexpr int kPersistMaxStamps = 1024;
constexpr int kPersistSyncWords = 512;
void launch_icp_persistent(const PersistArgs &args, int grid, size_t lds_bytes, hipStream_t st);
constexpr int kPersistMidMaxModel = 64 * 16 * 64;
constexpr size_t kPersistMidLdsMax = 24 * (kPersistMidMaxModel / 64 + kPersistMidMaxModel / 16);
void launch_icp_persistent_mid(const PersistArgs &args, int grid, size_t lds_bytes, hipStream_t st);
size_t persistent_mid_static_lds();
size_t persistent_static_lds();
std::vector<double> persist_model_image(const double *m_xyz, size_t nm, size_t *blocks_out);
struct TailArgs {
    const int *idx;
    const double4 *m4;
    double *px, *py, *pz;
    int n;
    double *yx, *yy, *yz;
    float4 *p32;
    SeedArgs sa;
    double *part17, *part1;
    unsigned *sync;
    unsigned epoch_base;
    int *h_abort;
    double N, c0, c1, c2;
    int *cnt;
    IterState *s;
    double threshold;
    int max_iter;
    double *err_trace;
    int *hflag;
    int ticket;
    IterState *h_state;
    double *h_trace;
    double *sums_out;
    int test_abort;
};
constexpr int kTailMaxBlocks = 192;
void launch_iteration_tail_grid(const TailArgs &args, int nblocks, hipStream_t st);
void launch_signal(int *flag_dev, int ticket, hipStream_t st);
void launch_nn_lds(const double *img, int nm, int nblk, const double *q_aos, int nq, int cull, const double m0[3],
                   int *idx_out, double *y_aos, size_t lds_bytes, hipStream_t st);
void launch_small_centroid(const double *in_aos, int n, double n_total, double *sums_out, double *out_aos, hipStream_t st);
void launch_small_err(const double *y_aos, double *p_aos, int n, const Xform &xf, int write_p, double *err_out,
                      hipStream_t st);
void launch_small_alignment(const double *p_aos, const double *y_aos, int n, double *out, hipStream_t st);
void launch_run_init(IterState *st_dev, int *amb_count, hipStream_t st, const double *c = nullptr);
void launch_first_shift(IterState *st_dev, const double *sums3, double N, hipStream_t st);
void launch_first_shift_y_sample(const int *idx, const double4 *m4, const double *yx, const double *yy,
                                 const double *yz, int n, const int *kpos, const double4 *m4kd, bool y_ready,
                                 double *out4, IterState *st_dev, const double *scene3, double N, hipStream_t st);
void launch_first_shifts(IterState *st_dev, const double *sums4, const double *scene3, double N, hipStream_t st);

void launch_nn_exact_few(const double *q_aos, int nq, const double4 *m4, int nm, int *idx_out, double *y_aos,
                         hipStream_t st);

void launch_reduce_pair(const double *part17, const double *part1, int nblocks, double *out, hipStream_t st);
void launch_reduce(const double *partials, int nblocks, int K, double *out, hipStream_t st);

constexpr int kGateSums = 18, kGateCount = 17;
constexpr int kGateTooFew = 1;
struct GateState {
    int status;
    int fail_iter;
    long long K;
};
void launch_gated_moments(const int *idx, const double4 *m4, const double *px, const double *py, const double *pz,
                          int n, double *yx, double *yy, double *yz, const IterState *st_dev, double D,
                          unsigned long long *mask, double *partials, hipStream_t st, const int *kpos,
                          const double4 *m4kd, bool y_ready);
void launch_gated_horn(const double *partials, int nblocks, double *sums, bool step, const double c[3], int *amb_count,
                       IterState *st_dev, GateState *gate, GateState *h_gate, IterState *h_state, hipStream_t st);
void launch_gated_first_shift(IterState *st_dev, const double *sums, hipStream_t st);
void launch_gated_transform(double *px, double *py, double *pz, const double *yx, const double *yy, const double *yz,
                            int n, const Xform *xf, const int *done, float4 *p32, const unsigned long long *mask,
                            double *partials, hipStream_t st);
void launch_gated_err(const double *partials, int nblocks, double *sums, bool step, double threshold, int max_iter,
                      double *err_trace, IterState *st_dev, const GateState *gate, long long *h_ktrace, int *hflag_dev,
                      int ticket, IterState *h_state_dev, double *h_trace_dev, hipStream_t st);
void launch_gated_unpack(const unsigned long long *mask, const int *order, int n, unsigned char *out, hipStream_t st);

size_t model_stats_scratch_doubles();
void launch_model_stats(const double *aos, int n, double *scratch, double *out, hipStream_t st);
void launch_model_f32_images(const double *aos, int nm, int nm_pad, const double c[3], float4 *m32, float *mperm,
                             float *mm, hipStream_t st);
void launch_model_compare(const double *aos, int n, const double *x, const double *y, const double *z, int *diff,
                          hipStream_t st);
struct KdPlan {
    struct Level {
        int seg_off, nseg, mid_off;
    };
    int nm = 0, max_seg = 1, leaf_off = 0, nleaf = 0;
    std::vector<Level> levels;
    std::vector<int> ints;
};
void kd_plan(size_t nm, KdPlan &pl);
size_t kd_order_scratch_bytes(const KdPlan &pl);
int launch_kd_order(const double *mx, const double *my, const double *mz, const KdPlan &pl, void *scratch,
                    size_t bytes, int *kd, hipStream_t st);

}
```

### iterative-closest-point_amd/csrc/icp_model.hip

```cpp
#include <hip/hip_runtime.h>
#include <hipcub/device/device_radix_sort.hpp>
#include <rocprim/device/device_scan.hpp>
#include <rocprim/iterator/counting_iterator.hpp>
#include <rocprim/iterator/transform_iterator.hpp>

#include <algorithm>
#include <cmath>

#include "icp_kernels.h"

namespace icp {
namespace {

constexpr int kStatBlocks = 256;

__device__ __forceinline__ unsigned long long ord_bits(double v)
{
    if (v == 0.0) v = 0.0;
    const unsigned long long b = (unsigned long long)__double_as_longlong(v);
    return (b >> 63) ? ~b : (b | 0x8000000000000000ull);
}

__global__ __launch_bounds__(kBlock) void model_stats_kernel(const double *__restrict__ aos, int n,
                                                             double *__restrict__ part)
{
    double s[3] = {0.0, 0.0, 0.0}, lo[3] = {INFINITY, INFINITY, INFINITY}, hi[3] = {-INFINITY, -INFINITY, -INFINITY};
    double bad = 0.0;
    for (int j = blockIdx.x * kBlock + threadIdx.x; j < n; j += gridDim.x * kBlock)
        for (int a = 0; a < 3; ++a) {
            const double v = aos[3 * (size_t)j + a];
            if (!isfinite(v)) bad += 1.0;
            s[a] += v;
            lo[a] = fmin(lo[a], v);
            hi[a] = fmax(hi[a], v);
        }
    __shared__ double sh[kBlock / 64][10];
    for (int off = 32; off > 0; off >>= 1) {
        for (int a = 0; a < 3; ++a) {
            s[a] += __shfl_down(s[a], off, 64);
            lo[a] = fmin(lo[a], __shfl_down(lo[a], off, 64));
            hi[a] = fmax(hi[a], __shfl_down(hi[a], off, 64));
        }
        bad += __shfl_down(bad, off, 64);
    }
    const int lane = threadIdx.x & 63, wave = threadIdx.x >> 6;
    if (lane == 0) {
        for (int a = 0; a < 3; ++a) {
            sh[wave][a] = s[a];
            sh[wave][3 + a] = lo[a];
            sh[wave][6 + a] = hi[a];
        }
        sh[wave][9] = bad;
    }
    __syncthreads();
    if (threadIdx.x < 10) {
        const int k = threadIdx.x;
        double v = sh[0][k];
        for (int w = 1; w < kBlock / 64; ++w)
            v = k < 3 ? v + sh[w][k] : k < 6 ? fmin(v, sh[w][k]) : k < 9 ? fmax(v, sh[w][k]) : v + sh[w][k];
        part[blockIdx.x * 10 + k] = v;
    }
}


template <int K>
__global__ __launch_bounds__(kBlock) void stats_fold_kernel(const double *__restrict__ part, int G, double *__restrict__ out)
{
    __shared__ double sh[kBlock][K];
    auto kind = [](int k) { return K == 10 ? (k < 3 ? 0 : k < 6 ? 1 : k < 9 ? 2 : 0) : (k < 2 ? 2 : 0); };
    double v[K];
    for (int k = 0; k < K; ++k) v[k] = kind(k) == 0 ? 0.0 : kind(k) == 1 ? INFINITY : -INFINITY;
    for (int g = threadIdx.x; g < G; g += kBlock)
        for (int k = 0; k < K; ++k) {
            const double x = part[g * K + k];
            v[k] = kind(k) == 0 ? v[k] + x : kind(k) == 1 ? fmin(v[k], x) : fmax(v[k], x);
        }
    for (int k = 0; k < K; ++k) sh[threadIdx.x][k] = v[k];
    __syncthreads();
    for (int w = kBlock / 2; w > 0; w >>= 1) {
        if ((int)threadIdx.x < w)
            for (int k = 0; k < K; ++k) {
                const double a = sh[threadIdx.x][k], b = sh[threadIdx.x + w][k];
                sh[threadIdx.x][k] = kind(k) == 0 ? a + b : kind(k) == 1 ? fmin(a, b) : fmax(a, b);
            }
        __syncthreads();
    }
    if (threadIdx.x < K) out[threadIdx.x] = sh[0][threadIdx.x];
}

__global__ __launch_bounds__(kBlock) void model_f32_images_kernel(const double *__restrict__ aos, int nm, int nm_pad,
                                                                  double cx, double cy, double cz,
                                                                  float4 *__restrict__ m32, float *__restrict__ mperm,
                                                                  float *__restrict__ mm)
{
    const int P = blockIdx.x * kBlock + threadIdx.x;
    if (P >= nm_pad) return;
    const bool real = P < nm;
    float4 v = make_float4(1.0e18f, 1.0e18f, 1.0e18f, 0.f);
    if (real) {
        v.x = (float)(aos[3 * (size_t)P] - cx);
        v.y = (float)(aos[3 * (size_t)P + 1] - cy);
        v.z = (float)(aos[3 * (size_t)P + 2] - cz);
    }
    m32[P] = v;
    const float mmv = real ? (float)((double)v.x * v.x + (double)v.y * v.y + (double)v.z * v.z) : 1.0e30f;
    const float comp[4] = {mmv, real ? v.x : 0.f, real ? v.y : 0.f, real ? v.z : 0.f};
    const size_t g = (size_t)P >> 6, t = (P >> 4) & 3, i = P & 15;
#pragma unroll
    for (int k = 0; k < 4; ++k) mperm[g * 256 + k * 64 + i * 4 + t] = comp[k];
    mm[P] = mmv;
}

__global__ __launch_bounds__(kBlock) void model_compare_kernel(const double *__restrict__ aos, int n,
                                                               const double *__restrict__ x, const double *__restrict__ y,
                                                               const double *__restrict__ z, int *__restrict__ diff)
{
    const int j = blockIdx.x * kBlock + threadIdx.x;
    bool d = false;
    if (j < n) {
        const double *q = aos + 3 * (size_t)j;
        d = __double_as_longlong(q[0]) != __double_as_longlong(x[j]) ||
            __double_as_longlong(q[1]) != __double_as_longlong(y[j]) ||
            __double_as_longlong(q[2]) != __double_as_longlong(z[j]);
    }
    const unsigned long long m = __ballot(d);
    if ((threadIdx.x & 63) == 0 && m) atomicAdd(diff, (int)__popcll(m));
}


__global__ __launch_bounds__(kBlock) void kd_axis_keys_kernel(const double *__restrict__ v, int n,
                                                              unsigned long long *__restrict__ key, int *__restrict__ val)
{
    const int j = blockIdx.x * kBlock + threadIdx.x;
    if (j < n) {
        key[j] = ord_bits(v[j]);
        val[j] = j;
    }
}

__device__ __forceinline__ int widest_axis3(const double (&ext)[3])
{
    int ax = 0;
    for (int a = 1; a < 3; ++a)
        if (ext[a] > ext[ax]) ax = a;
    return ax;
}

__device__ __forceinline__ int seg_of(const int *__restrict__ lo, int nseg, int pos)
{
    int l = 0, h = nseg - 1;
    while (l < h) {
        const int m = (l + h + 1) >> 1;
        if (lo[m] <= pos) l = m;
        else h = m - 1;
    }
    return l;
}

struct KdLists {
    const int *a[3];
};

__global__ __launch_bounds__(kBlock) void kd_range_axis_kernel(const int *__restrict__ seg_lo,
                                                               const int *__restrict__ seg_mid, int nseg, int n,
                                                               KdLists A, const double *__restrict__ x,
                                                               const double *__restrict__ y,
                                                               const double *__restrict__ z, int *__restrict__ axis)
{
    const int s = blockIdx.x * kBlock + threadIdx.x;
    if (s >= nseg || seg_mid[s] < 0) return;
    const int lo = seg_lo[s], hi = s + 1 < nseg ? seg_lo[s + 1] : n;
    const double *c[3] = {x, y, z};
    double ext[3];
    for (int a = 0; a < 3; ++a) ext[a] = c[a][A.a[a][hi - 1]] - c[a][A.a[a][lo]];
    axis[s] = widest_axis3(ext);
}

__global__ __launch_bounds__(kBlock) void kd_flag_kernel(const int *__restrict__ seg_lo, const int *__restrict__ seg_mid,
                                                         int nseg, int n, KdLists A, const int *__restrict__ axis,
                                                         unsigned char *__restrict__ flag)
{
    const int p = blockIdx.x * kBlock + threadIdx.x;
    if (p >= n) return;
    const int s = seg_of(seg_lo, nseg, p), mid = seg_mid[s];
    if (mid < 0) return;
    flag[A.a[axis[s]][p]] = p < mid ? 1 : 0;
}

struct Cnt3 {
    int c[3];
};
struct Cnt3Sum {
    __host__ __device__ Cnt3 operator()(const Cnt3 &x, const Cnt3 &y) const
    {
        return Cnt3{{x.c[0] + y.c[0], x.c[1] + y.c[1], x.c[2] + y.c[2]}};
    }
};
struct FlagsAt {
    KdLists A;
    const unsigned char *flag;
    __host__ __device__ Cnt3 operator()(int p) const
    {
        return Cnt3{{(int)flag[A.a[0][p]], (int)flag[A.a[1][p]], (int)flag[A.a[2][p]]}};
    }
};

inline auto flags_at(const FlagsAt &f)
{
    return rocprim::make_transform_iterator(rocprim::counting_iterator<int>(0), f);
}

__global__ __launch_bounds__(kBlock) void kd_partition_kernel(const int *__restrict__ seg_lo,
                                                              const int *__restrict__ seg_mid, int nseg, int n, KdLists A,
                                                              const unsigned char *__restrict__ flag,
                                                              const Cnt3 *__restrict__ S, int *__restrict__ d0,
                                                              int *__restrict__ d1, int *__restrict__ d2)
{
    const int p = blockIdx.x * kBlock + threadIdx.x;
    if (p >= n) return;
    const int s = seg_of(seg_lo, nseg, p), mid = seg_mid[s], lo = seg_lo[s];
    int *d[3] = {d0, d1, d2};
    const Cnt3 sp = S[p], sl = S[lo];
    for (int a = 0; a < 3; ++a) {
        const int id = A.a[a][p];
        int dest = p;
        if (mid >= 0) {
            const int left_before = sp.c[a] - sl.c[a];
            dest = flag[id] ? lo + left_before : mid + (p - lo - left_before);
        }
        d[a][dest] = id;
    }
}

__global__ __launch_bounds__(kBlock) void kd_local_kernel(const int *__restrict__ leaf_lo, int nleaf, int n,
                                                          const int *__restrict__ A0, int *__restrict__ loc)
{
    const int p = blockIdx.x * kBlock + threadIdx.x;
    if (p >= n) return;
    loc[A0[p]] = p - leaf_lo[seg_of(leaf_lo, nleaf, p)];
}

constexpr int kKdLeaf = 1024;
__global__ __launch_bounds__(kBlock) void kd_leaf_kernel(const int *__restrict__ leaf_lo, KdLists A,
                                                         const int *__restrict__ loc, const double *__restrict__ x,
                                                         const double *__restrict__ y, const double *__restrict__ z,
                                                         int *__restrict__ kd)
{
    constexpr int kMaxR = kKdLeaf / 32 + 2;
    __shared__ int s_id[kKdLeaf];
    __shared__ short s_A[2][3][kKdLeaf];
    __shared__ int s_S[3][kKdLeaf];
    __shared__ unsigned char s_flag[kKdLeaf];
    __shared__ int s_rlo[kMaxR], s_rhi[kMaxR], s_rmid[kMaxR], s_rax[kMaxR];
    __shared__ int s_wsum[3][kBlock / 64];
    __shared__ int s_nr, s_active;
    const int L0 = leaf_lo[blockIdx.x], cnt = leaf_lo[blockIdx.x + 1] - L0;
    const int tid = threadIdx.x, lane = tid & 63, wave = tid >> 6;
    for (int i = tid; i < cnt; i += kBlock) {
        s_id[i] = A.a[0][L0 + i];
        s_A[0][0][i] = (short)i;
        s_A[0][1][i] = (short)loc[A.a[1][L0 + i]];
        s_A[0][2][i] = (short)loc[A.a[2][L0 + i]];
    }
    if (tid == 0) {
        s_rlo[0] = 0;
        s_rhi[0] = cnt;
        s_nr = 1;
    }
    const double *coord[3] = {x, y, z};
    int cur = 0;
    for (;;) {
        __syncthreads();
        if (tid == 0) {
            int act = 0;
            for (int r = 0; r < s_nr; ++r) {
                const int c = s_rhi[r] - s_rlo[r];
                int mid = -1;
                if (c > 32) {
                    const int units = (c + 31) / 32;
                    mid = s_rlo[r] + 32 * ((units + 1) / 2);
                    ++act;
                }
                s_rmid[r] = mid;
            }
            s_active = act;
        }
        __syncthreads();
        if (!s_active) break;
        const int nr = s_nr;
        if (tid < nr && s_rmid[tid] >= 0) {
            const int lo = s_rlo[tid], hi = s_rhi[tid];
            double ext[3];
            for (int a = 0; a < 3; ++a)
                ext[a] = coord[a][s_id[s_A[cur][a][hi - 1]]] - coord[a][s_id[s_A[cur][a][lo]]];
            s_rax[tid] = widest_axis3(ext);
        }
        __syncthreads();
        auto range_of = [&](int p) {
            int l = 0, h = nr - 1;
            while (l < h) {
                const int m = (l + h + 1) >> 1;
                if (s_rlo[m] <= p) l = m;
                else h = m - 1;
            }
            return l;
        };
        for (int p = tid; p < cnt; p += kBlock) {
            const int r = range_of(p);
            if (s_rmid[r] >= 0) s_flag[s_A[cur][s_rax[r]][p]] = p < s_rmid[r] ? 1 : 0;
        }
        __syncthreads();
        int f[3][4], t[3];
        for (int a = 0; a < 3; ++a) {
            t[a] = 0;
            for (int k = 0; k < 4; ++k) {
                const int p = 4 * tid + k;
                f[a][k] = p < cnt ? s_flag[s_A[cur][a][p]] : 0;
                t[a] += f[a][k];
            }
        }
        int incl[3] = {t[0], t[1], t[2]};
        for (int o = 1; o < 64; o <<= 1)
            for (int a = 0; a < 3; ++a) {
                const int v = __shfl_up(incl[a], o, 64);
                if (lane >= o) incl[a] += v;
            }
        if (lane == 63)
            for (int a = 0; a < 3; ++a) s_wsum[a][wave] = incl[a];
        __syncthreads();
        for (int a = 0; a < 3; ++a) {
            int base = incl[a] - t[a];
            for (int w = 0; w < wave; ++w) base += s_wsum[a][w];
            for (int k = 0; k < 4; ++k) {
                const int p = 4 * tid + k;
                if (p < cnt) s_S[a][p] = base;
                base += f[a][k];
            }
        }
        __syncthreads();
        for (int p = tid; p < cnt; p += kBlock) {
            const int r = range_of(p), mid = s_rmid[r], lo = s_rlo[r];
            for (int a = 0; a < 3; ++a) {
                const short v = s_A[cur][a][p];
                int dest = p;
                if (mid >= 0) {
                    const int left_before = s_S[a][p] - s_S[a][lo];
                    dest = s_flag[v] ? lo + left_before : mid + (p - lo - left_before);
                }
                s_A[cur ^ 1][a][dest] = v;
            }
        }
        __syncthreads();
        if (tid == 0) {
            int m = 0;
            int nlo[kMaxR], nhi[kMaxR];
            for (int r = 0; r < s_nr; ++r) {
                if (s_rmid[r] >= 0) {
                    nlo[m] = s_rlo[r];
                    nhi[m++] = s_rmid[r];
                    nlo[m] = s_rmid[r];
                    nhi[m++] = s_rhi[r];
                } else {
                    nlo[m] = s_rlo[r];
                    nhi[m++] = s_rhi[r];
                }
            }
            for (int r = 0; r < m; ++r) {
                s_rlo[r] = nlo[r];
                s_rhi[r] = nhi[r];
            }
            s_nr = m;
        }
        cur ^= 1;
    }
    for (int i = tid; i < cnt; i += kBlock) kd[L0 + i] = s_id[s_A[cur][0][i]];
}

}


size_t model_stats_scratch_doubles() { return (size_t)kStatBlocks * 10 + 16; }

void launch_model_stats(const double *aos, int n, double *scratch, double *out, hipStream_t st)
{
    model_stats_kernel<<<kStatBlocks, kBlock, 0, st>>>(aos, n, scratch);
    stats_fold_kernel<10><<<1, kBlock, 0, st>>>(scratch, kStatBlocks, out);
}

void launch_model_f32_images(const double *aos, int nm, int nm_pad, const double c[3], float4 *m32, float *mperm,
                             float *mm, hipStream_t st)
{
    model_f32_images_kernel<<<(nm_pad + kBlock - 1) / kBlock, kBlock, 0, st>>>(aos, nm, nm_pad, c[0], c[1], c[2], m32,
                                                                              mperm, mm);
}

void launch_model_compare(const double *aos, int n, const double *x, const double *y, const double *z, int *diff,
                          hipStream_t st)
{
    if (n > 0) model_compare_kernel<<<(n + kBlock - 1) / kBlock, kBlock, 0, st>>>(aos, n, x, y, z, diff);
}


void kd_plan(size_t nm, KdPlan &pl)
{
    pl = KdPlan{};
    pl.nm = (int)nm;
    std::vector<int> lo{0}, hi{(int)nm};
    for (;;) {
        std::vector<int> mid(lo.size(), -1);
        bool any = false;
        for (size_t s = 0; s < lo.size(); ++s) {
            const int c = hi[s] - lo[s];
            if (c > kKdLeaf) {
                const int units = (c + kKdLeaf - 1) / kKdLeaf;
                mid[s] = lo[s] + kKdLeaf * ((units + 1) / 2);
                any = true;
            }
        }
        if (!any) break;
        KdPlan::Level L;
        L.seg_off = (int)pl.ints.size();
        L.nseg = (int)lo.size();
        pl.ints.insert(pl.ints.end(), lo.begin(), lo.end());
        L.mid_off = (int)pl.ints.size();
        pl.ints.insert(pl.ints.end(), mid.begin(), mid.end());
        pl.levels.push_back(L);
        std::vector<int> nlo, nhi;
        for (size_t s = 0; s < lo.size(); ++s) {
            if (mid[s] >= 0) {
                nlo.push_back(lo[s]);
                nhi.push_back(mid[s]);
                nlo.push_back(mid[s]);
                nhi.push_back(hi[s]);
            } else {
                nlo.push_back(lo[s]);
                nhi.push_back(hi[s]);
            }
        }
        lo.swap(nlo);
        hi.swap(nhi);
    }
    pl.leaf_off = (int)pl.ints.size();
    pl.nleaf = (int)lo.size();
    pl.ints.insert(pl.ints.end(), lo.begin(), lo.end());
    pl.ints.push_back((int)nm);
    pl.max_seg = 1;
    for (const auto &L : pl.levels) pl.max_seg = std::max(pl.max_seg, L.nseg);
}

namespace {
struct KdScratch {
    unsigned long long *k0, *k1;
    int *A[2][3], *axis, *loc, *plan;
    Cnt3 *S;
    unsigned char *flag;
    void *temp;
    size_t temp_bytes, used;
};

size_t scan_temp_bytes(int n)
{
    size_t a = 0, b = 0;
    (void)hipcub::DeviceRadixSort::SortPairs(nullptr, a, (const unsigned long long *)nullptr,
                                             (unsigned long long *)nullptr, (const int *)nullptr, (int *)nullptr, n, 0,
                                             64);
    (void)rocprim::exclusive_scan(nullptr, b, flags_at(FlagsAt{}), (Cnt3 *)nullptr, Cnt3{{0, 0, 0}}, (size_t)n,
                                  Cnt3Sum{});
    return std::max(a, b);
}

KdScratch kd_carve(const KdPlan &pl, void *base)
{
    const size_t n = (size_t)std::max(pl.nm, 1);
    auto al = [](size_t b) { return (b + 255) & ~(size_t)255; };
    KdScratch k{};
    char *p = (char *)base;
    k.k0 = (unsigned long long *)p;
    k.k1 = k.k0 + n;
    p += al(2 * n * sizeof(unsigned long long));
    for (int b = 0; b < 2; ++b)
        for (int a = 0; a < 3; ++a) {
            k.A[b][a] = (int *)p;
            p += al(n * sizeof(int));
        }
    k.S = (Cnt3 *)p;
    p += al(n * sizeof(Cnt3));
    k.axis = (int *)p;
    p += al((size_t)pl.max_seg * sizeof(int));
    k.loc = (int *)p;
    p += al(n * sizeof(int));
    k.plan = (int *)p;
    p += al(pl.ints.size() * sizeof(int));
    k.flag = (unsigned char *)p;
    p += al(n);
    k.temp = p;
    k.used = (size_t)(p - (char *)base);
    return k;
}
}

size_t kd_order_scratch_bytes(const KdPlan &pl)
{
    const KdScratch k = kd_carve(pl, nullptr);
    return k.used + ((scan_temp_bytes(std::max(pl.nm, 1)) + 255) & ~(size_t)255);
}

int launch_kd_order(const double *mx, const double *my, const double *mz, const KdPlan &pl, void *scratch,
                    size_t bytes, int *kd, hipStream_t st)
{
    const int n = pl.nm;
    if (n <= 0) return 0;
    KdScratch k = kd_carve(pl, scratch);
    if (k.used > bytes) return -1;
    k.temp_bytes = bytes - k.used;
    if (hipMemcpyAsync(k.plan, pl.ints.data(), pl.ints.size() * sizeof(int), hipMemcpyHostToDevice, st) != hipSuccess)
        return -1;
    const int g = (n + kBlock - 1) / kBlock;
    const double *axes[3] = {mx, my, mz};
    int *ids = k.A[1][0];
    for (int a = 0; a < 3; ++a) {
        kd_axis_keys_kernel<<<g, kBlock, 0, st>>>(axes[a], n, k.k0, ids);
        if (hipcub::DeviceRadixSort::SortPairs(k.temp, k.temp_bytes, k.k0, k.k1, ids, k.A[0][a], n, 0, 64, st) !=
            hipSuccess)
            return -1;
    }
    int cur = 0;
    for (const KdPlan::Level &L : pl.levels) {
        const KdLists A{{k.A[cur][0], k.A[cur][1], k.A[cur][2]}};
        const int *lo = k.plan + L.seg_off, *mid = k.plan + L.mid_off;
        kd_range_axis_kernel<<<(L.nseg + kBlock - 1) / kBlock, kBlock, 0, st>>>(lo, mid, L.nseg, n, A, mx, my, mz,
                                                                               k.axis);
        kd_flag_kernel<<<g, kBlock, 0, st>>>(lo, mid, L.nseg, n, A, k.axis, k.flag);
        if (rocprim::exclusive_scan(k.temp, k.temp_bytes, flags_at(FlagsAt{A, k.flag}), k.S, Cnt3{{0, 0, 0}}, (size_t)n,
                                    Cnt3Sum{}, st) != hipSuccess)
            return -1;
        kd_partition_kernel<<<g, kBlock, 0, st>>>(lo, mid, L.nseg, n, A, k.flag, k.S, k.A[cur ^ 1][0], k.A[cur ^ 1][1],
                                                  k.A[cur ^ 1][2]);
        cur ^= 1;
    }
    const KdLists A{{k.A[cur][0], k.A[cur][1], k.A[cur][2]}};
    kd_local_kernel<<<g, kBlock, 0, st>>>(k.plan + pl.leaf_off, pl.nleaf, n, A.a[0], k.loc);
    kd_leaf_kernel<<<pl.nleaf, kBlock, 0, st>>>(k.plan + pl.leaf_off, A, k.loc, mx, my, mz, kd);
    return hipGetLastError() == hipSuccess ? 0 : -1;
}

}
// ... 1 lines not shown
```

### iterative-closest-point_amd/csrc/icp_sort.hip

```cpp
#include <hip/hip_runtime.h>

#include <algorithm>

#include "icp_kernels.h"

namespace icp {
namespace {

constexpr int kSortThreads = 256;
constexpr int kSortRounds = 16;
constexpr int kSortTile = kSortThreads * kSortRounds;
constexpr int kSortBins = 256;
constexpr int kRowThreads = 256;

__device__ __forceinline__ unsigned long long digit_peers(unsigned d, bool valid, int width)
{
    unsigned long long peers = __ballot(valid);
#pragma unroll
    for (int b = 0; b < 8; ++b) {
        if (b < width) {
            const bool bit = (d >> b) & 1u;
            const unsigned long long m = __ballot(bit);
            peers &= bit ? m : ~m;
        }
    }
    return peers;
}

__device__ __forceinline__ int tile_item(int tile, int w, int r, int l)
{
    return tile * kSortTile + w * (kSortTile / 4) + r * 64 + l;
}

__global__ __launch_bounds__(kSortThreads) void sort_hist_kernel(const unsigned *__restrict__ keys, int n, int shift,
                                                                 int width, int ntile, int *__restrict__ hist)
{
    __shared__ int cnt[4][kSortBins];
    const int tid = threadIdx.x, w = tid >> 6, l = tid & 63, tile = blockIdx.x;
    const unsigned mask = (1u << width) - 1u;
    for (int i = tid; i < 4 * kSortBins; i += kSortThreads) (&cnt[0][0])[i] = 0;
    unsigned k[kSortRounds];
#pragma unroll
    for (int r = 0; r < kSortRounds; ++r) {
        const int i = tile_item(tile, w, r, l);
        k[r] = i < n ? keys[i] : 0u;
    }
    __syncthreads();
#pragma unroll
    for (int r = 0; r < kSortRounds; ++r) {
        const bool valid = tile_item(tile, w, r, l) < n;
        const unsigned d = (k[r] >> shift) & mask;
        const unsigned long long peers = digit_peers(d, valid, width);
        if (valid && (peers >> l) == 1ull) cnt[w][d] += __popcll(peers);
        __builtin_amdgcn_wave_barrier();
    }
    __syncthreads();
    hist[tid * ntile + tile] = cnt[0][tid] + cnt[1][tid] + cnt[2][tid] + cnt[3][tid];
}

__device__ __forceinline__ int wave_incl_scan(int v, int l)
{
#pragma unroll
    for (int o = 1; o < 64; o <<= 1) {
        const int u = __shfl_up(v, o, 64);
        if (l >= o) v += u;
    }
    return v;
}

__global__ __launch_bounds__(kRowThreads) void sort_rows_kernel(int *__restrict__ hist, int ntile,
                                                                 int *__restrict__ totals)
{
    __shared__ int wsum[kRowThreads / 64];
    __shared__ int carry_s;
    const int tid = threadIdx.x, w = tid >> 6, l = tid & 63;
    int *row = hist + (size_t)blockIdx.x * ntile;
    int carry = 0;
    for (int base = 0; base < ntile; base += 4 * kRowThreads) {
        const int i = base + 4 * tid;
        int v[4];
#pragma unroll
        for (int j = 0; j < 4; ++j) v[j] = i + j < ntile ? row[i + j] : 0;
        const int t = v[0] + v[1] + v[2] + v[3];
        const int incl = wave_incl_scan(t, l);
        if (l == 63) wsum[w] = incl;
        __syncthreads();
        if (w == 0) {
            const int s = l < kRowThreads / 64 ? wsum[l] : 0;
            const int si = wave_incl_scan(s, l);
            if (l < kRowThreads / 64) wsum[l] = si - s;
            if (l == kRowThreads / 64 - 1) carry_s = si;
        }
        __syncthreads();
        int run = carry + wsum[w] + incl - t;
#pragma unroll
        for (int j = 0; j < 4; ++j) {
            if (i + j < ntile) row[i + j] = run;
            run += v[j];
        }
        carry += carry_s;
        __syncthreads();
    }
    if (tid == 0) totals[blockIdx.x] = carry;
}

__global__ __launch_bounds__(kSortThreads) void sort_scatter_kernel(const unsigned *__restrict__ kin,
                                                                    const int *__restrict__ vin, int n, int shift,
                                                                    int width, int ntile, const int *__restrict__ hist,
                                                                    const int *__restrict__ totals,
                                                                    unsigned *__restrict__ kout, int *__restrict__ vout)
{
    __shared__ unsigned skey[kSortTile];
    __shared__ int sval[kSortTile];
    __shared__ int cnt[4][kSortBins];
    __shared__ int goff[kSortBins];
    __shared__ int wtot[4], wbase[4];
    const int tid = threadIdx.x, w = tid >> 6, l = tid & 63, tile = blockIdx.x;
    const unsigned mask = (1u << width) - 1u;
    for (int i = tid; i < 4 * kSortBins; i += kSortThreads) (&cnt[0][0])[i] = 0;
    unsigned k[kSortRounds];
    int v[kSortRounds];
#pragma unroll
    for (int r = 0; r < kSortRounds; ++r) {
        const int i = tile_item(tile, w, r, l);
        k[r] = i < n ? kin[i] : 0u;
        v[r] = i < n ? (vin ? vin[i] : i) : 0;
    }
    __syncthreads();
    int rank[kSortRounds];
#pragma unroll
    for (int r = 0; r < kSortRounds; ++r) {
        const bool valid = tile_item(tile, w, r, l) < n;
        const unsigned d = (k[r] >> shift) & mask;
        const unsigned long long peers = digit_peers(d, valid, width);
        const int below = __popcll(peers & ((1ull << l) - 1ull));
        const int before = cnt[w][d];
        rank[r] = before + below;
        if (valid && (peers >> l) == 1ull) cnt[w][d] = before + below + 1;
        __builtin_amdgcn_wave_barrier();
    }
    __syncthreads();
    {
        const int d = tid;
        const int c0 = cnt[0][d], c1 = cnt[1][d], c2 = cnt[2][d], c3 = cnt[3][d];
        const int tot = c0 + c1 + c2 + c3, gt = totals[d];
        const int incl = wave_incl_scan(tot, l), gincl = wave_incl_scan(gt, l);
        if (l == 63) {
            wtot[w] = incl;
            wbase[w] = gincl;
        }
        __syncthreads();
        int start = incl - tot, gbase = gincl - gt;
        for (int j = 0; j < w; ++j) {
            start += wtot[j];
            gbase += wbase[j];
        }
        cnt[0][d] = start;
        cnt[1][d] = start + c0;
        cnt[2][d] = start + c0 + c1;
        cnt[3][d] = start + c0 + c1 + c2;
        goff[d] = gbase + hist[d * ntile + tile] - start;
    }
    __syncthreads();
#pragma unroll
    for (int r = 0; r < kSortRounds; ++r) {
        if (tile_item(tile, w, r, l) < n) {
            const int p = cnt[w][(k[r] >> shift) & mask] + rank[r];
            skey[p] = k[r];
            sval[p] = v[r];
        }
    }
    __syncthreads();
    const int count = min(kSortTile, n - tile * kSortTile);
#pragma unroll 4
    for (int s = tid; s < count; s += kSortThreads) {
        const unsigned key = skey[s];
        const int o = goff[(key >> shift) & mask] + s;
        kout[o] = key;
        vout[o] = sval[s];
    }
}

size_t al256(size_t b) { return (b + 255) & ~(size_t)255; }

}

hipError_t sort_pairs_u32(void *temp, size_t &temp_bytes, const unsigned *k0, unsigned *k1, const int *v0, int *v1,
                          int n, int bits, hipStream_t st)
{
    const int ntile = (std::max(n, 1) + kSortTile - 1) / kSortTile;
    const size_t need = 2 * al256((size_t)std::max(n, 1) * sizeof(int)) + al256((size_t)kSortBins * ntile * sizeof(int)) +
                        al256(kSortBins * sizeof(int));
    if (!temp) {
        temp_bytes = need;
        return hipSuccess;
    }
    if (temp_bytes < need || bits < 0 || bits > 32) return hipErrorInvalidValue;
    if (n <= 0) return hipSuccess;
    const int npass = std::max(1, (bits + 7) / 8);
    char *p = (char *)temp;
    unsigned *tk = (unsigned *)p;
    int *tv = (int *)(p + al256((size_t)n * sizeof(int)));
    int *hist = (int *)(p + 2 * al256((size_t)n * sizeof(int)));
    int *totals = (int *)((char *)hist + al256((size_t)kSortBins * ntile * sizeof(int)));
    const int width = (bits + npass - 1) / npass;
    const unsigned *ki = k0;
    const int *vi = v0;
    for (int pass = 0; pass < npass; ++pass) {
        const bool to_out = ((npass - 1 - pass) & 1) == 0;
        unsigned *ko = to_out ? k1 : tk;
        int *vo = to_out ? v1 : tv;
        const int shift = pass * width, wd = std::min(width, bits - shift);
        sort_hist_kernel<<<ntile, kSortThreads, 0, st>>>(ki, n, shift, wd, ntile, hist);
        sort_rows_kernel<<<kSortBins, kRowThreads, 0, st>>>(hist, ntile, totals);
        sort_scatter_kernel<<<ntile, kSortThreads, 0, st>>>(ki, vi, n, shift, wd, ntile, hist, totals, ko, vo);
        ki = ko;
        vi = vo;
    }
    return hipGetLastError();
}

}
```

### iterative-closest-point_amd/icp_amd.py

```python
from __future__ import annotations

import ctypes as C
import os
from dataclasses import dataclass, field

import numpy as np

_HERE = os.path.dirname(os.path.abspath(__file__))
LIB_PATH = os.environ.get("ICP_AMD_LIB") or os.path.join(_HERE, "build", "libicp_hip.so")

ICP_OK = 0
ICP_E_ARG = -1
ICP_E_HIP = -2
ICP_E_SIZE_MISMATCH = -3
ICP_E_TOO_FEW_POINTS = -4
ICP_E_NO_MODEL = -5
ICP_E_RCCL = -6
ICP_E_NO_DEVICE = -7
ICP_E_IO = -8
ICP_E_RANGE = -9

NN_CERTIFIED = 0
NN_FP64 = 1
VARIANT_AUTO = 0
VARIANT_VALU = 1
VARIANT_MFMA = 2
VARIANT_MFMA16 = 3
VARIANT_GRID = 4
VARIANT_BUNDLE = 5
RULE_SQUARED = 0
RULE_CPU_SQRT = 1
RUN_AUTO = 0
RUN_LAUNCHES = 1
RUN_PERSISTENT = 2

EXPORTED = [
    "icp_ctx_create", "icp_ctx_create_dist", "icp_rccl_unique_id", "icp_ctx_create_sharded",
    "icp_ctx_destroy",
    "icp_last_error", "icp_strerror", "icp_device_count", "icp_set_model", "icp_set_scene",
    "icp_set_model_device", "icp_set_scene_device", "icp_set_model_device_stream",
    "icp_set_scene_device_stream", "icp_set_progress",
    "icp_get_scene", "icp_set_allow_unequal", "icp_set_nn_variant", "icp_run", "icp_closest_matrix",
    "icp_compute_centroid", "icp_y_p_norm", "icp_err_compute", "icp_find_alignment",
    "icp_horn_solve", "icp_max_element_index", "icp_shard_range", "icp_synthetic_pair",
    "icp_load_matrix", "icp_write_matrix", "icp_free", "icp_get_stats", "icp_reset_stats",
    "icp_ensure_model", "icp_subtract_col", "icp_get_indices", "icp_set_index_digest",
    "icp_get_index_digest", "icp_set_cert_audit", "icp_set_run_mode", "icp_set_nn_rule",
    "icp_get_comm_info", "icp_set_bundle_counters", "icp_get_bundle_counters", "icp_get_model_order",
    "icp_bundle_audit", "icp_sort_pairs",
    "icp_set_max_distance", "icp_get_inliers", "icp_get_inlier_trace",
]


class ICPError(RuntimeError):
    def __init__(self, code: int, msg: str):
        super().__init__(f"{msg} (code {code})")
        self.code = code


class Result(C.Structure):
    _fields_ = [("iterations", C.c_int), ("converged", C.c_int), ("err", C.c_double),
                ("s", C.c_double), ("R", C.c_double * 9), ("t", C.c_double * 3)]


class Stats(C.Structure):
    _fields_ = [("nn_ms", C.c_double), ("nn_launches", C.c_longlong), ("nn_pairs", C.c_longlong),
                ("ambiguous", C.c_longlong), ("level1_queued", C.c_longlong), ("level1_unrecovered", C.c_longlong), ("iter_ms", C.c_double), ("iterations", C.c_longlong),
                ("grid_fallback", C.c_longlong), ("allreduce_ms", C.c_double),
                ("allreduce_calls", C.c_longlong), ("cert_max_err_ratio", C.c_double),
                ("cert_min_margin", C.c_double), ("cert_audited", C.c_longlong),
                ("persistent_runs", C.c_longlong), ("cpu_rule_ties", C.c_longlong),
                ("cpu_rule_changed", C.c_longlong), ("persistent_fallbacks", C.c_longlong),
                ("last_filter", C.c_int), ("bundle_builds", C.c_longlong),
                ("bundle_builds_in_run", C.c_longlong), ("run_bundle_searches", C.c_longlong),
                ("run_grid_searches", C.c_longlong), ("run_certified", C.c_longlong),
                ("run_walked", C.c_longlong), ("run_path_bits", C.c_ulonglong)]


class BundleAudit(C.Structure):
    _fields_ = [("max_err_ratio", C.c_double), ("min_gap", C.c_double), ("pairs", C.c_longlong),
                ("excluded", C.c_longlong), ("checked", C.c_longlong), ("violations", C.c_longlong)]


FILTER_NAMES = {-1: None, 0: "valu", 1: "mfma", 2: "mfma16", 3: "bundle", 4: "grid", 5: "fp64", 6: "one_launch"}


ALLREDUCE_FN = C.CFUNCTYPE(C.c_int, C.POINTER(C.c_double), C.c_size_t, C.c_void_p)
PROGRESS_FN = C.CFUNCTYPE(None, C.c_int, C.c_double, C.c_void_p)

_lib = None


def lib() -> C.CDLL:
    global _lib
    if _lib is not None:
        return _lib
    if not os.path.exists(LIB_PATH):
        raise ICPError(ICP_E_NO_DEVICE, f"{LIB_PATH} not built: run `make -C iterative-closest-point_amd`")
    L = C.CDLL(LIB_PATH)
    dp = C.POINTER(C.c_double)
    vp = C.c_void_p
    sz = C.c_size_t
    L.icp_ctx_create.argtypes = [C.c_int, C.c_int, C.POINTER(vp)]
    L.icp_ctx_create_dist.argtypes = [C.c_int, C.c_int, C.c_int, C.c_int, C.c_char_p, C.POINTER(vp)]
    L.icp_rccl_unique_id.argtypes = [C.c_char_p]
    L.icp_ctx_create_sharded.argtypes = [C.c_int, C.c_int, C.c_int, C.c_int, ALLREDUCE_FN, vp, C.POINTER(vp)]
    L.icp_ctx_destroy.argtypes = [vp]
    L.icp_ctx_destroy.restype = None
    L.icp_last_error.argtypes = [vp]
    L.icp_last_error.restype = C.c_char_p
    L.icp_strerror.argtypes = [C.c_int]
    L.icp_strerror.restype = C.c_char_p
    L.icp_device_count.argtypes = [C.POINTER(C.c_int)]
    L.icp_set_model.argtypes = [vp, dp, sz]
    L.icp_set_model_device.argtypes = [vp, vp, sz]
    L.icp_set_progress.argtypes = [vp, PROGRESS_FN, vp]
    L.icp_set_scene_device.argtypes = [vp, vp, sz, sz]
    if hasattr(L, "icp_set_model_device_stream"):
        L.icp_set_model_device_stream.argtypes = [vp, vp, sz, vp]
        L.icp_set_scene_device_stream.argtypes = [vp, vp, sz, sz, vp]
    L.icp_set_scene.argtypes = [vp, dp, sz, sz]
    L.icp_get_scene.argtypes = [vp, dp]
    L.icp_set_allow_unequal.argtypes = [vp, C.c_int]
    L.icp_set_nn_variant.argtypes = [vp, C.c_int]
    L.icp_set_run_mode.argtypes = [vp, C.c_int]
    L.icp_set_nn_rule.argtypes = [vp, C.c_int]
    L.icp_run.argtypes = [vp, C.c_int, C.c_double, dp, C.POINTER(Result)]
    L.icp_closest_matrix.argtypes = [vp, dp, sz, dp, C.POINTER(C.c_int32)]
    L.icp_compute_centroid.argtypes = [vp, dp, sz, dp, dp]
    L.icp_y_p_norm.argtypes = [vp, dp, dp, sz, dp, dp]
    L.icp_err_compute.argtypes = [vp, dp, dp, sz, C.c_int, dp, dp, dp]
    L.icp_find_alignment.argtypes = [vp, dp, dp, sz, dp, dp, dp, dp]
    L.icp_horn_solve.argtypes = [dp, dp, dp, C.c_double, C.c_double, dp, dp, dp]
    L.icp_max_element_index.argtypes = [dp]
    L.icp_shard_range.argtypes = [sz, C.c_int, C.c_int, C.POINTER(sz), C.POINTER(sz)]
    L.icp_synthetic_pair.argtypes = [C.c_uint64, sz, C.c_double, dp, dp, dp, dp]
    L.icp_load_matrix.argtypes = [C.c_char_p, C.POINTER(dp), C.POINTER(sz)]
    L.icp_write_matrix.argtypes = [C.c_char_p, dp, sz]
    L.icp_free.argtypes = [vp]
    L.icp_free.restype = None
    L.icp_ensure_model.argtypes = [vp, dp, sz, C.POINTER(C.c_int)]
    L.icp_subtract_col.argtypes = [vp, dp, sz, dp, dp]
    L.icp_get_indices.argtypes = [vp, C.POINTER(C.c_int32)]
    L.icp_get_model_order.argtypes = [vp, C.POINTER(C.c_int32)]
    L.icp_sort_pairs.argtypes = [C.c_int, C.POINTER(C.c_uint32), sz, C.c_int, C.POINTER(C.c_uint32), C.POINTER(C.c_int32)]
    L.icp_set_index_digest.argtypes = [vp, sz]
    L.icp_get_index_digest.argtypes = [vp, C.POINTER(C.c_uint64), sz]
    L.icp_set_cert_audit.argtypes = [vp, C.c_int]
    L.icp_bundle_audit.argtypes = [vp, C.c_int, C.POINTER(BundleAudit)]
    L.icp_get_stats.argtypes = [vp, C.POINTER(Stats)]
    L.icp_reset_stats.argtypes = [vp]
    L.icp_set_bundle_counters.argtypes = [vp, C.c_int]
    L.icp_get_bundle_counters.argtypes = [vp, C.POINTER(C.c_uint64)]
    L.icp_get_comm_info.argtypes = [vp, C.POINTER(C.c_int), C.POINTER(C.c_int), C.c_char_p, C.c_int]
    if hasattr(L, "icp_set_max_distance"):
        L.icp_set_max_distance.argtypes = [vp, C.c_double]
        L.icp_get_inliers.argtypes = [vp, C.POINTER(C.c_uint8), C.POINTER(C.c_longlong)]
        L.icp_get_inlier_trace.argtypes = [vp, C.POINTER(C.c_longlong), sz]
    _lib = L
    return L


def _dp(a: np.ndarray):
    return a.ctypes.data_as(C.POINTER(C.c_double))


def _cloud(a) -> np.ndarray:
    a = np.ascontiguousarray(a, dtype=np.float64)
    if a.ndim != 2 or a.shape[1] != 3:
        raise ValueError("clouds are (n, 3) float64 arrays")
    return a


def _vec(a, n) -> np.ndarray:
    a = np.ascontiguousarray(a, dtype=np.float64).reshape(-1)
    if a.size != n:
        raise ValueError(f"expected {n} values")
    return a



def strerror(code: int) -> str:
    return lib().icp_strerror(code).decode()


def device_count() -> int:
    n = C.c_int(0)
    lib().icp_device_count(C.byref(n))
    return n.value


def sort_pairs(keys, bits: int, device: int = 0):
    k = np.ascontiguousarray(keys, dtype=np.uint32)
    order = np.empty(k.size, dtype=np.int32); out = np.empty(k.size, dtype=np.uint32)
    rc = lib().icp_sort_pairs(device, k.ctypes.data_as(C.POINTER(C.c_uint32)), k.size, bits,
                              out.ctypes.data_as(C.POINTER(C.c_uint32)), order.ctypes.data_as(C.POINTER(C.c_int32)))
    if rc != ICP_OK:
        raise ICPError(rc, strerror(rc))
    return order, out


def horn_solve(S, mu_p, mu_y, d_caps: float, sp: float):
    S = _vec(S, 9); mu_p = _vec(mu_p, 3); mu_y = _vec(mu_y, 3)
    s = C.c_double(0.0); R = np.zeros(9); t = np.zeros(3)
    rc = lib().icp_horn_solve(_dp(S), _dp(mu_p), _dp(mu_y), d_caps, sp, C.byref(s), _dp(R), _dp(t))
    if rc != ICP_OK:
        raise ICPError(rc, strerror(rc))
    return s.value, R.reshape(3, 3), t


def max_element_index(ev) -> int:
    ev = _vec(ev, 4)
    return lib().icp_max_element_index(_dp(ev))


def shard_range(n_total: int, rank: int, world: int):
    b = C.c_size_t(0); c = C.c_size_t(0)
    rc = lib().icp_shard_range(n_total, rank, world, C.byref(b), C.byref(c))
    if rc != ICP_OK:
        raise ICPError(rc, strerror(rc))
    return b.value, c.value


def synthetic_pair(n: int, seed: int = 42, angle_deg: float = 5.0, axis=(1.0, 2.0, 3.0),
                   t=(0.05, -0.03, 0.02)):
    m = np.empty((n, 3)); p = np.empty((n, 3))
    ax = np.asarray(axis, dtype=np.float64); tt = np.asarray(t, dtype=np.float64)
    rc = lib().icp_synthetic_pair(seed, n, angle_deg, _dp(ax), _dp(tt), _dp(m), _dp(p))
    if rc != ICP_OK:
        raise ICPError(rc, strerror(rc))
    return m, p


def load_matrix(path: str) -> np.ndarray:
    ptr = C.POINTER(C.c_double)(); n = C.c_size_t(0)
    rc = lib().icp_load_matrix(path.encode(), C.byref(ptr), C.byref(n))
    if rc != ICP_OK:
        raise ICPError(rc, f"{path}: {strerror(rc)}")
    try:
        out = np.ctypeslib.as_array(ptr, shape=(max(n.value, 1) * 3,))[: n.value * 3].copy()
    finally:
        lib().icp_free(ptr)
    return out.reshape(n.value, 3)


def write_matrix(path: str, xyz) -> None:
    xyz = _cloud(xyz)
    rc = lib().icp_write_matrix(path.encode(), _dp(xyz), xyz.shape[0])
    if rc != ICP_OK:
        raise ICPError(rc, strerror(rc))


def rccl_unique_id() -> bytes:
    buf = C.create_string_buffer(128)
    rc = lib().icp_rccl_unique_id(buf)
    if rc != ICP_OK:
        raise ICPError(rc, strerror(rc))
    return buf.raw



class Context:

    def __init__(self, device: int = 0, nn_mode: int = NN_CERTIFIED, rank: int = 0,
                 world_size: int = 1, rccl_id: bytes | None = None, host_allreduce=None):
        L = lib()
        h = C.c_void_p()
        self._cb = None
        if host_allreduce is not None:
            def _cb(buf, count, _user):
                try:
                    host_allreduce(np.ctypeslib.as_array(buf, shape=(count,)))
                    return 0
                except Exception:
                    return 1
            self._cb = ALLREDUCE_FN(_cb)
            rc = L.icp_ctx_create_sharded(device, nn_mode, rank, world_size, self._cb, None, C.byref(h))
        elif world_size > 1 or rccl_id is not None:
            rc = L.icp_ctx_create_dist(device, nn_mode, rank, world_size, rccl_id, C.byref(h))
        else:
            rc = L.icp_ctx_create(device, nn_mode, C.byref(h))
        if rc != ICP_OK:
            raise ICPError(rc, f"context creation failed: {strerror(rc)}")
        self._h = h
        self.rank, self.world_size = rank, world_size

    def _check(self, rc: int):
        if rc != ICP_OK:
            raise ICPError(rc, f"{strerror(rc)}: {lib().icp_last_error(self._h).decode()}")

    def close(self):
        if getattr(self, "_h", None):
            lib().icp_ctx_destroy(self._h)
            self._h = None

    def __del__(self):
        try:
            self.close()
        except Exception:
            pass

    def __enter__(self):
        return self

    def __exit__(self, *a):
        self.close()

    def set_model(self, m):
        m = _cloud(m)
        self._check(lib().icp_set_model(self._h, _dp(m), m.shape[0]))

    def set_model_device(self, ptr: int, nm: int, stream=None):
        if stream is None or not hasattr(lib(), "icp_set_model_device_stream"):
            self._check(lib().icp_set_model_device(self._h, C.c_void_p(ptr), nm))
        else:
            self._check(lib().icp_set_model_device_stream(self._h, C.c_void_p(ptr), nm, C.c_void_p(stream)))

    def set_scene_device(self, ptr: int, np_local: int, np_total: int | None = None, stream=None):
        npt = np_local if np_total is None else np_total
        if stream is None or not hasattr(lib(), "icp_set_scene_device_stream"):
            self._check(lib().icp_set_scene_device(self._h, C.c_void_p(ptr), np_local, npt))
        else:
            self._check(lib().icp_set_scene_device_stream(self._h, C.c_void_p(ptr), np_local, npt,
                                                          C.c_void_p(stream)))
        self._np_local = np_local

    def set_progress(self, fn):
        self._progress = PROGRESS_FN(lambda i, e, _u: fn(i, e)) if fn is not None else None
        self._check(lib().icp_set_progress(self._h, self._progress if fn is not None else PROGRESS_FN(), None))

    def ensure_model(self, m) -> bool:
        m = _cloud(m)
        up = C.c_int(0)
        self._check(lib().icp_ensure_model(self._h, _dp(m), m.shape[0], C.byref(up)))
        return bool(up.value)

    def set_scene(self, p, np_total: int | None = None):
        p = _cloud(p)
        self._check(lib().icp_set_scene(self._h, _dp(p), p.shape[0], p.shape[0] if np_total is None else np_total))
        self._np_local = p.shape[0]

    def get_scene(self) -> np.ndarray:
        out = np.empty((self._np_local, 3))
        self._check(lib().icp_get_scene(self._h, _dp(out)))
        return out

    def set_nn_variant(self, variant: int):
        self._check(lib().icp_set_nn_variant(self._h, variant))

    def set_nn_rule(self, rule: int):
        self._check(lib().icp_set_nn_rule(self._h, rule))

    def set_run_mode(self, mode: int):
        self._check(lib().icp_set_run_mode(self._h, mode))

    def set_allow_unequal(self, allow: bool):
        self._check(lib().icp_set_allow_unequal(self._h, 1 if allow else 0))

    def set_max_distance(self, d: float):
        self._check(lib().icp_set_max_distance(self._h, float(d)))

    def inliers(self):
        mask = np.zeros(self._np_local, dtype=np.uint8)
        k = C.c_longlong(0)
        self._check(lib().icp_get_inliers(self._h, mask.ctypes.data_as(C.POINTER(C.c_uint8)), C.byref(k)))
        return mask.astype(bool), int(k.value)

    def inlier_trace(self) -> np.ndarray:
        n = lib().icp_get_inlier_trace(self._h, None, 0)
        if n < 0:
            self._check(n)
        out = np.zeros(max(n, 1), dtype=np.int64)
        rc = lib().icp_get_inlier_trace(self._h, out.ctypes.data_as(C.POINTER(C.c_longlong)), n)
        if rc < 0:
            self._check(rc)
        return out[:n]

    def run(self, max_iter: int, threshold: float = 1e-5):
        errs = np.zeros(max(max_iter, 1))
        res = Result()
        self._check(lib().icp_run(self._h, max_iter, threshold, _dp(errs), C.byref(res)))
        return res, errs[: res.iterations].copy()

    def closest_matrix(self, p):
        p = _cloud(p)
        y = np.empty_like(p); idx = np.empty(p.shape[0], dtype=np.int32)
        self._check(lib().icp_closest_matrix(self._h, _dp(p), p.shape[0], _dp(y),
                                             idx.ctypes.data_as(C.POINTER(C.c_int32))))
        return y, idx

    def subtract_col(self, xyz, m):
        xyz = _cloud(xyz)
        out = np.empty_like(xyz)
        self._check(lib().icp_subtract_col(self._h, _dp(xyz), xyz.shape[0], _dp(_vec(m, 3)), _dp(out)))
        return out

    def get_indices(self) -> np.ndarray:
        idx = np.empty(self._np_local, dtype=np.int32)
        self._check(lib().icp_get_indices(self._h, idx.ctypes.data_as(C.POINTER(C.c_int32))))
        return idx

    def model_order(self, nm: int) -> np.ndarray:
        kd = np.empty(nm, dtype=np.int32)
        self._check(lib().icp_get_model_order(self._h, kd.ctypes.data_as(C.POINTER(C.c_int32))))
        return kd

    def set_index_digest(self, cap: int):
        self._check(lib().icp_set_index_digest(self._h, cap))
        self._digest_cap = cap

    def set_cert_audit(self, on: bool):
        self._check(lib().icp_set_cert_audit(self._h, 1 if on else 0))

    def bundle_audit(self, groups: int = 64) -> dict:
        out = BundleAudit()
        self._check(lib().icp_bundle_audit(self._h, int(groups), C.byref(out)))
        return {f: getattr(out, f) for f, _ in BundleAudit._fields_}

    def index_digest(self, k: int | None = None) -> np.ndarray:
        k = self._digest_cap if k is None else k
        out = np.zeros((max(k, 1), 3), dtype=np.uint64)
        self._check(lib().icp_get_index_digest(self._h, out.ctypes.data_as(C.POINTER(C.c_uint64)), k))
        return out[:k]

    def compute_centroid(self, xyz, centred: bool = True):
        xyz = _cloud(xyz)
        mu = np.zeros(3); out = np.empty_like(xyz) if centred else None
        self._check(lib().icp_compute_centroid(self._h, _dp(xyz), xyz.shape[0], _dp(mu),
                                               _dp(out) if centred else None))
        return mu, out

    def y_p_norm(self, y, p):
        y = _cloud(y); p = _cloud(p)
        d = C.c_double(0.0); s = C.c_double(0.0)
        self._check(lib().icp_y_p_norm(self._h, _dp(y), _dp(p), y.shape[0], C.byref(d), C.byref(s)))
        return d.value, s.value

    def err_compute(self, y, p, in_place: bool, sR, t):
        y = _cloud(y); p = _cloud(p).copy()
        sR = _vec(sR, 9); t = _vec(t, 3); e = C.c_double(0.0)
        self._check(lib().icp_err_compute(self._h, _dp(y), _dp(p), y.shape[0], 1 if in_place else 0,
                                          _dp(sR), _dp(t), C.byref(e)))
        return e.value, p

    def find_alignment(self, p, y):
        p = _cloud(p); y = _cloud(y)
        s = C.c_double(0.0); R = np.zeros(9); t = np.zeros(3); e = C.c_double(0.0)
        self._check(lib().icp_find_alignment(self._h, _dp(p), _dp(y), p.shape[0], C.byref(s), _dp(R),
                                             _dp(t), C.byref(e)))
        return s.value, R.reshape(3, 3), t, e.value

    def stats(self) -> dict:
        st = Stats()
        self._check(lib().icp_get_stats(self._h, C.byref(st)))
        return {k: getattr(st, k) for k, _ in Stats._fields_}

    def reset_stats(self):
        self._check(lib().icp_reset_stats(self._h))

    def set_bundle_counters(self, on: bool):
        self._check(lib().icp_set_bundle_counters(self._h, 1 if on else 0))

    def bundle_counters(self) -> dict:
        out = (C.c_uint64 * 16)()
        self._check(lib().icp_get_bundle_counters(self._h, out))
        tasks = max(int(out[7]), 1)
        return {"stream_mfma": int(out[8]), "block_triggers": int(out[0]), "group_tests": int(out[1]),
                "pair_tests": int(out[2]), "wave_tasks": int(out[7]),
                "us_per_wave_task": {"prologue": out[3] * 0.01 / tasks, "stream": out[4] * 0.01 / tasks,
                                     "deferred": out[5] * 0.01 / tasks, "epilogue": out[6] * 0.01 / tasks},
                "deferred_us_per_wave_task": {"bound_tests": out[10] * 0.01 / tasks,
                                              "pair_block_waits": out[11] * 0.01 / tasks,
                                              "pair_tests": out[12] * 0.01 / tasks},
                "slowest_task_us_total": out[9] * 0.01}

    def comm_info(self) -> dict:
        cnt, rk = C.c_int(0), C.c_int(0)
        bus = C.create_string_buffer(64)
        self._check(lib().icp_get_comm_info(self._h, C.byref(cnt), C.byref(rk), bus, 64))
        return {"comm_count": cnt.value if cnt.value >= 0 else None, "comm_rank": rk.value,
                "pci_bus_id": bus.value.decode()}



@dataclass
class ICP:
    m: np.ndarray
    p: np.ndarray
    max_iter: int
    nn_mode: int = NN_CERTIFIED
    device: int = 0
    threshold: float = 1e-5
    allow_unequal: bool = False
    max_distance: float | None = None
    new_p: np.ndarray = field(init=False)
    s: float = field(init=False, default=1.0)
    r: np.ndarray = field(init=False)
    t: np.ndarray = field(init=False)
    errors: np.ndarray = field(init=False)

    def __post_init__(self):
        self.m = _cloud(self.m); self.p = _cloud(self.p)
        self.new_p = self.p.copy()
        self.r = np.eye(3); self.t = np.zeros(3)
        self.errors = np.zeros(0)
        self._ctx = Context(self.device, self.nn_mode)
        self._ctx.set_allow_unequal(self.allow_unequal)
        if self.max_distance is not None:
            self._ctx.set_max_distance(self.max_distance)
        self._ctx.set_model(self.m)
        self._ctx.set_scene(self.p)

    def find_corresponding_opti(self):
        res, errs = self._ctx.run(self.max_iter, self.threshold)
        self.errors = errs
        self.s, self.r, self.t = res.s, np.array(res.R).reshape(3, 3), np.array(res.t)
        self.new_p = self._ctx.get_scene()
        return res

    def find_alignment(self, y):
        s, R, t, e = self._ctx.find_alignment(self.new_p, y)
        self.s, self.r, self.t = s, R, t
        return e

    def compute_y_naive(self):
        Y = np.empty_like(self.new_p)
        for j in range(self.new_p.shape[0]):
            Y[j] = self.m[compute_distance_w_naive(self.m, self.new_p[j], self._ctx)]
        return Y

    def find_corresponding_naive(self):
        if self.p.shape[0] != self.m.shape[0] and not self.allow_unequal:
            raise ICPError(ICP_E_SIZE_MISMATCH, "Point sets need to have the same number of points.")
        if self.p.shape[0] < 4:
            raise ICPError(ICP_E_TOO_FEW_POINTS, "Need at least 4 point pairs")
        errs = []
        for _ in range(self.max_iter):
            Y = self.compute_y_naive()
            err = self.find_alignment(Y)
            e2, self.new_p = self._ctx.err_compute(Y, self.new_p, True, self.s * self.r, self.t)
            err = (err + e2) / self.p.shape[0]
            errs.append(err)
            if err < self.threshold:
                break
        self.errors = np.array(errs)
        return len(errs)


_default_ctx: Context | None = None


def _ctx_for_model(m) -> Context:
    global _default_ctx
    if _default_ctx is None:
        _default_ctx = Context()
    _default_ctx.set_model(m)
    return _default_ctx


# ... 23 lines not shown
```

Baseline: 10150.

## Lazy fp32 model images, fuse grid starts into gather, retune radix sort

The fp32 model image build becomes lazy and runs only when a path that needs it (VALU filter, level-1 or non-cell-seed grid) is taken. The grid-starts kernel is folded into the gather kernel, and the sort-value array is dropped when fused. The radix sort is templated on wave count (default 16 waves per tile) and gains an in-scatter prefix path that skips the row-scan kernel for small tile counts. A grid-inspection API is also added. Together these cut model-setup launches and work per model load, at the cost of extra complexity and env-gated paths.

```diff
diff --git a/include/icp_capi.h b/include/icp_capi.h
--- a/include/icp_capi.h
+++ b/include/icp_capi.h
@@ -157,6 +157,7 @@
 int icp_get_comm_info(icp_ctx *ctx, int *comm_count, int *comm_rank, char *bus_id, int len);
 int icp_get_model_order(icp_ctx *ctx, int32_t *kd_out);
 int icp_sort_pairs(int device, const uint32_t *keys, size_t n, int bits, uint32_t *keys_out, int32_t *order_out);
+int icp_get_grid(icp_ctx *ctx, int g[3], double lo[3], double *inv_h, int32_t *start, int32_t *order);
 
 #ifdef __cplusplus
 }
diff --git a/iterative-closest-point_amd/csrc/icp_engine.hip b/iterative-closest-point_amd/csrc/icp_engine.hip
--- a/iterative-closest-point_amd/csrc/icp_engine.hip
+++ b/iterative-closest-point_amd/csrc/icp_engine.hip
@@ -138,6 +138,7 @@
     float *mm = nullptr;
     char *mimg16 = nullptr;
     bool mimg16_pending = false;
+    bool m32_pending = false;
     float *mms16 = nullptr;
     double scale16 = 1.0;
     size_t nm = 0, nm_pad = 0, m32_cap = 0, mperm_cap = 0, mm_cap = 0, mimg16_cap = 0, mms16_cap = 0;
@@ -739,6 +740,19 @@
     return ICP_OK;
 }
 
+static int ensure_m32(icp_ctx *ctx)
+{
+    if (!ctx->m32_pending) return ICP_OK;
+    TRY(grow(ctx, &ctx->m32, &ctx->m32_cap, ctx->nm_pad));
+    TRY(grow(ctx, &ctx->mperm, &ctx->mperm_cap, ctx->nm_pad));
+    TRY(grow(ctx, &ctx->mm, &ctx->mm_cap, ctx->nm_pad));
+    launch_model_f32_images_soa(ctx->model.x, ctx->model.y, ctx->model.z, (int)ctx->nm, (int)ctx->nm_pad, ctx->c,
+                                ctx->m32, (float *)ctx->mperm, ctx->mm, ctx->st);
+    LAUNCHCHK("model_f32_images");
+    ctx->m32_pending = false;
+    return ICP_OK;
+}
+
 static bool cell_seed_on()
 {
     static const bool on = [] {
@@ -799,8 +813,10 @@
         ctx->stats.last_filter = ICP_FILTER_GRID;
         TRY(grow(ctx, &ctx->fb_list, &ctx->fb_list_cap, n));
         TRY(grow(ctx, &ctx->fb_T, &ctx->fb_T_cap, n));
+        const bool cell_seeds = !seeded && slot_order && cell_seed_on();
+        if (!cell_seeds) TRY(ensure_m32(ctx));
         if (ev0) HIPCHK(hipEventRecord(ev0, ctx->st));
-        if (!seeded && slot_order && cell_seed_on()) return grid_unseeded_slot(ctx, q, n, stop, ev1);
+        if (cell_seeds) return grid_unseeded_slot(ctx, q, n, stop, ev1);
         if (seeded)
             launch_nn_grid_resolve_all((int)n, q.x, q.y, q.z, ctx->m4, grid_view(ctx), grid_budget(ctx), ctx->idx,
                                        ctx->amb_count + 1, ctx->fb_list, ctx->fb_T, ctx->st, stop, 0,
@@ -823,6 +839,7 @@
             ctx->stats.last_filter = ICP_FILTER_GRID;
             TRY(grow(ctx, &ctx->fb_list, &ctx->fb_list_cap, n));
             TRY(grow(ctx, &ctx->fb_T, &ctx->fb_T_cap, n));
+            if (!cell_seed_on()) TRY(ensure_m32(ctx));
             if (ev0) HIPCHK(hipEventRecord(ev0, ctx->st));
             if (cell_seed_on()) return grid_unseeded_slot(ctx, q, n, stop, ev1);
             launch_nn_grid_search((int)n, q.x, q.y, q.z, grid_view(ctx), grid_budget(ctx), ctx->idx, ctx->amb_count + 1,
@@ -834,6 +851,7 @@
             return ICP_OK;
         }
         if (l1 >= 2) TRY(ensure_mimage16(ctx));
+        if (l1 == 1 || !inline_nm) TRY(ensure_m32(ctx));
         if (l1 == 3 && ctx->bundle_pending && ws) ctx->stats.bundle_builds_in_run += 1;
         if (l1 == 3) TRY(ensure_bundle(ctx));
         const bool gseed = l1 >= 2 && !seeded && grid_seed && ctx->g_pts;
@@ -953,6 +971,7 @@
         TRY(grow(ctx, &ctx->amb_hint, &ctx->amb_hint_cap, n));
         TRY(grow(ctx, &ctx->fb_list, &ctx->fb_list_cap, n));
         TRY(grow(ctx, &ctx->fb_T, &ctx->fb_T_cap, n));
+        TRY(ensure_m32(ctx));
         if (ev0) HIPCHK(hipEventRecord(ev0, ctx->st));
         launch_nn_filter(q.f, (int)n, ctx->m32, (int)ctx->nm_pad, pl, pb, ps, pi, ctx->st, stop);
         if (ev1) HIPCHK(hipEventRecord(ev1, ctx->st));
@@ -1515,11 +1534,18 @@
     std::swap(ctx->model, ctx->model_alt);
     std::swap(ctx->m4, ctx->m4_alt);
     std::swap(ctx->m4_cap, ctx->m4_alt_cap);
-    TRY(grow(ctx, &ctx->m32, &ctx->m32_cap, nm_pad));
-    TRY(grow(ctx, &ctx->mperm, &ctx->mperm_cap, nm_pad));
-    TRY(grow(ctx, &ctx->mm, &ctx->mm_cap, nm_pad));
-    launch_model_f32_images(aos, (int)nm, (int)nm_pad, ctx->c, ctx->m32, (float *)ctx->mperm, ctx->mm, ctx->st);
-    LAUNCHCHK("model_f32_images");
+    static const bool m32_lazy = [] {
+        const char *e = getenv("ICP_M32_LAZY");
+        return !(e && atoi(e) == 0);
+    }();
+    ctx->m32_pending = m32_lazy;
+    if (!m32_lazy) {
+        TRY(grow(ctx, &ctx->m32, &ctx->m32_cap, nm_pad));
+        TRY(grow(ctx, &ctx->mperm, &ctx->mperm_cap, nm_pad));
+        TRY(grow(ctx, &ctx->mm, &ctx->mm_cap, nm_pad));
+        launch_model_f32_images(aos, (int)nm, (int)nm_pad, ctx->c, ctx->m32, (float *)ctx->mperm, ctx->mm, ctx->st);
+        LAUNCHCHK("model_f32_images");
+    }
     ctx->scale16 = rm64 > 0.0 ? std::ldexp(1.0, (int)std::floor(std::log2(4096.0 / rm64))) : 1.0;
     while (rm64 * ctx->scale16 >= 4096.0) ctx->scale16 *= 0.5;
     ctx->mimg16_pending = true;
@@ -3368,6 +3394,28 @@
     return ok ? ICP_OK : ICP_E_HIP;
 }
 
+int icp_get_grid(icp_ctx *ctx, int g[3], double lo[3], double *inv_h, int32_t *start, int32_t *order)
+{
+    if (!ctx || !g || !lo || !inv_h) return ICP_E_ARG;
+    if (!ctx->has_model || !ctx->g_start || !ctx->g_pts) return fail(ctx, ICP_E_NO_MODEL, "no model grid");
+    HIPCHK(hipSetDevice(ctx->device));
+    for (int a = 0; a < 3; ++a) {
+        g[a] = ctx->grid.g[a];
+        lo[a] = ctx->grid.lo[a];
+    }
+    *inv_h = ctx->grid.inv_h;
+    HIPCHK(hipStreamSynchronize(ctx->st));
+    if (start)
+        HIPCHK(hipMemcpy(start, ctx->g_start, sizeof(int32_t) * ((size_t)grid_cells(ctx->grid) + 1),
+                         hipMemcpyDeviceToHost));
+    if (order) {
+        std::vector<double> pts(4 * ctx->nm);
+        HIPCHK(hipMemcpy(pts.data(), ctx->g_pts, sizeof(double) * 4 * ctx->nm, hipMemcpyDeviceToHost));
+        for (size_t k = 0; k < ctx->nm; ++k) order[k] = (int32_t)pts[4 * k + 3];
+    }
+    return ICP_OK;
+}
+
 int icp_get_stats(const icp_ctx *ctx, icp_stats *out)
 {
     if (!ctx || !out) return ICP_E_ARG;
diff --git a/iterative-closest-point_amd/csrc/icp_grid.hip b/iterative-closest-point_amd/csrc/icp_grid.hip
--- a/iterative-closest-point_amd/csrc/icp_grid.hip
+++ b/iterative-closest-point_amd/csrc/icp_grid.hip
@@ -34,7 +34,7 @@
     const int cy = cell1(my[i], gv.lo[1], gv.inv_h, gv.g[1]);
     const int cz = cell1(mz[i], gv.lo[2], gv.inv_h, gv.g[2]);
     key[i] = (unsigned)((cz * gv.g[1] + cy) * gv.g[0] + cx);
-    val[i] = i;
+    if (val) val[i] = i;
 }
 
 __global__ __launch_bounds__(kBlock) void grid_starts_kernel(const unsigned *__restrict__ skey, int nm, int ncell,
@@ -51,11 +51,46 @@
     start[c] = lo;
 }
 
+constexpr int kFillThread = 16;
+
 __global__ __launch_bounds__(kBlock) void grid_gather_kernel(const double4 *__restrict__ m4, int nm,
                                                            const int *__restrict__ sval, double4 *__restrict__ pts,
-                                                           float4 *__restrict__ pts32, double c0, double c1, double c2)
-{
+                                                           float4 *__restrict__ pts32, double c0, double c1, double c2,
+                                                           const unsigned *__restrict__ skey, int ncell,
+                                                           int *__restrict__ start)
+{
+    __shared__ int s_n;
+    __shared__ int s_lo[kBlock + 1], s_hi[kBlock + 1], s_val[kBlock + 1];
     const int k = blockIdx.x * kBlock + threadIdx.x;
+    if (skey) {
+        if (threadIdx.x == 0) s_n = 0;
+        __syncthreads();
+        if (k < nm) {
+            const int cur = (int)skey[k], prev = k ? (int)skey[k - 1] : -1;
+            for (int part = 0; part < (k == nm - 1 ? 2 : 1); ++part) {
+                const int lo = part ? cur + 1 : prev + 1, hi = part ? ncell + 1 : cur + 1, val = part ? nm : k;
+                if (hi - lo <= kFillThread) {
+                    for (int c = lo; c < hi; ++c) start[c] = val;
+                } else {
+                    const int s = atomicAdd(&s_n, 1);
+                    s_lo[s] = lo;
+                    s_hi[s] = hi;
+                    s_val[s] = val;
+                }
+            }
+        }
+        __syncthreads();
+        const int nlong = s_n;
+        const bool al16 = ((size_t)start & 15) == 0;
+        for (int s = 0; s < nlong; ++s) {
+            const int lo = s_lo[s], hi = s_hi[s], val = s_val[s];
+            const int a = al16 ? min(hi, (lo + 3) & ~3) : hi, b = max(a, hi & ~3);
+            for (int c = lo + (int)threadIdx.x; c < a; c += kBlock) start[c] = val;
+            for (int c = a + 4 * (int)threadIdx.x; c < b; c += 4 * kBlock)
+                *(int4 *)(start + c) = make_int4(val, val, val, val);
+            for (int c = b + (int)threadIdx.x; c < hi; c += kBlock) start[c] = val;
+        }
+    }
     if (k >= nm) return;
     const int i = sval[k];
     const double4 m = m4[i];
@@ -1947,12 +1982,18 @@
     int *v0 = (int *)(k1 + nm), *v1 = v0 + nm;
     size_t temp_bytes = bytes - grid_keys_bytes(nm);
     const int g = (nm + kBlock - 1) / kBlock;
+    static const bool fused = [] {
+        const char *e = getenv("ICP_GRID_FUSED");
+        return !(e && atoi(e) == 0);
+    }();
+    if (fused) v0 = nullptr;
     grid_keys_kernel<<<g, kBlock, 0, st>>>(mx, my, mz, nm, gv, k0, v0);
     if (sort_pairs_u32((char *)scratch + grid_keys_bytes(nm), temp_bytes, k0, k1, v0, v1, nm, cell_bits(ncell), st) !=
         hipSuccess)
         return -1;
-    grid_starts_kernel<<<(int)((ncell + kBlock) / kBlock), kBlock, 0, st>>>(k1, nm, (int)ncell, start);
-    grid_gather_kernel<<<g, kBlock, 0, st>>>(m4, nm, v1, pts, pts32, p.c32[0], p.c32[1], p.c32[2]);
+    if (!fused) grid_starts_kernel<<<(int)((ncell + kBlock) / kBlock), kBlock, 0, st>>>(k1, nm, (int)ncell, start);
+    grid_gather_kernel<<<g, kBlock, 0, st>>>(m4, nm, v1, pts, pts32, p.c32[0], p.c32[1], p.c32[2],
+                                             fused ? k1 : nullptr, (int)ncell, start);
     return 0;
 }
 
diff --git a/iterative-closest-point_amd/csrc/icp_kernels.h b/iterative-closest-point_amd/csrc/icp_kernels.h
--- a/iterative-closest-point_amd/csrc/icp_kernels.h
+++ b/iterative-closest-point_amd/csrc/icp_kernels.h
@@ -515,6 +515,8 @@
 void launch_model_stats(const double *aos, int n, double *scratch, double *out, hipStream_t st);
 void launch_model_f32_images(const double *aos, int nm, int nm_pad, const double c[3], float4 *m32, float *mperm,
                              float *mm, hipStream_t st);
+void launch_model_f32_images_soa(const double *x, const double *y, const double *z, int nm, int nm_pad,
+                                 const double c[3], float4 *m32, float *mperm, float *mm, hipStream_t st);
 void launch_model_compare(const double *aos, int n, const double *x, const double *y, const double *z, int *diff,
                           hipStream_t st);
 struct KdPlan {
diff --git a/iterative-closest-point_amd/csrc/icp_model.hip b/iterative-closest-point_amd/csrc/icp_model.hip
--- a/iterative-closest-point_amd/csrc/icp_model.hip
+++ b/iterative-closest-point_amd/csrc/icp_model.hip
@@ -88,7 +88,10 @@
     if (threadIdx.x < K) out[threadIdx.x] = sh[0][threadIdx.x];
 }
 
-__global__ __launch_bounds__(kBlock) void model_f32_images_kernel(const double *__restrict__ aos, int nm, int nm_pad,
+template <bool SOA>
+__global__ __launch_bounds__(kBlock) void model_f32_images_kernel(const double *__restrict__ aos,
+                                                                  const double *__restrict__ sy,
+                                                                  const double *__restrict__ sz, int nm, int nm_pad,
                                                                   double cx, double cy, double cz,
                                                                   float4 *__restrict__ m32, float *__restrict__ mperm,
                                                                   float *__restrict__ mm)
@@ -98,9 +101,9 @@
     const bool real = P < nm;
     float4 v = make_float4(1.0e18f, 1.0e18f, 1.0e18f, 0.f);
     if (real) {
-        v.x = (float)(aos[3 * (size_t)P] - cx);
-        v.y = (float)(aos[3 * (size_t)P + 1] - cy);
-        v.z = (float)(aos[3 * (size_t)P + 2] - cz);
+        v.x = (float)((SOA ? aos[P] : aos[3 * (size_t)P]) - cx);
+        v.y = (float)((SOA ? sy[P] : aos[3 * (size_t)P + 1]) - cy);
+        v.z = (float)((SOA ? sz[P] : aos[3 * (size_t)P + 2]) - cz);
     }
     m32[P] = v;
     const float mmv = real ? (float)((double)v.x * v.x + (double)v.y * v.y + (double)v.z * v.z) : 1.0e30f;
@@ -390,8 +393,15 @@
 void launch_model_f32_images(const double *aos, int nm, int nm_pad, const double c[3], float4 *m32, float *mperm,
                              float *mm, hipStream_t st)
 {
-    model_f32_images_kernel<<<(nm_pad + kBlock - 1) / kBlock, kBlock, 0, st>>>(aos, nm, nm_pad, c[0], c[1], c[2], m32,
-                                                                              mperm, mm);
+    model_f32_images_kernel<false><<<(nm_pad + kBlock - 1) / kBlock, kBlock, 0, st>>>(aos, nullptr, nullptr, nm, nm_pad,
+                                                                                     c[0], c[1], c[2], m32, mperm, mm);
+}
+
+void launch_model_f32_images_soa(const double *x, const double *y, const double *z, int nm, int nm_pad,
+                                 const double c[3], float4 *m32, float *mperm, float *mm, hipStream_t st)
+{
+    model_f32_images_kernel<true><<<(nm_pad + kBlock - 1) / kBlock, kBlock, 0, st>>>(x, y, z, nm, nm_pad, c[0], c[1],
+                                                                                    c[2], m32, mperm, mm);
 }
 
 void launch_model_compare(const double *aos, int n, const double *x, const double *y, const double *z, int *diff,
diff --git a/iterative-closest-point_amd/csrc/icp_sort.hip b/iterative-closest-point_amd/csrc/icp_sort.hip
--- a/iterative-closest-point_amd/csrc/icp_sort.hip
+++ b/iterative-closest-point_amd/csrc/icp_sort.hip
@@ -1,17 +1,18 @@
 #include <hip/hip_runtime.h>
 
 #include <algorithm>
+#include <cstdlib>
 
 #include "icp_kernels.h"
 
 namespace icp {
 namespace {
 
-constexpr int kSortThreads = 256;
-constexpr int kSortRounds = 16;
-constexpr int kSortTile = kSortThreads * kSortRounds;
+constexpr int kSortTile = 4096;
 constexpr int kSortBins = 256;
 constexpr int kRowThreads = 256;
+constexpr int kSortPrefixTiles = 256;
+constexpr int kSortWavesDefault = 16;
 
 __device__ __forceinline__ unsigned long long digit_peers(unsigned d, bool valid, int width)
 {
@@ -27,35 +28,43 @@
     return peers;
 }
 
-__device__ __forceinline__ int tile_item(int tile, int w, int r, int l)
-{
-    return tile * kSortTile + w * (kSortTile / 4) + r * 64 + l;
-}
-
-__global__ __launch_bounds__(kSortThreads) void sort_hist_kernel(const unsigned *__restrict__ keys, int n, int shift,
-                                                                 int width, int ntile, int *__restrict__ hist)
-{
-    __shared__ int cnt[4][kSortBins];
+template <int W> __device__ __forceinline__ int tile_item(int tile, int w, int r, int l)
+{
+    return tile * kSortTile + w * (kSortTile / W) + r * 64 + l;
+}
+
+template <int W>
+__global__ __launch_bounds__(64 * W) void sort_hist_kernel(const unsigned *__restrict__ keys, int n, int shift,
+                                                           int width, int ntile, int tile_major,
+                                                           int *__restrict__ hist)
+{
+    constexpr int kRounds = 64 / W;
+    __shared__ int cnt[W][kSortBins];
     const int tid = threadIdx.x, w = tid >> 6, l = tid & 63, tile = blockIdx.x;
     const unsigned mask = (1u << width) - 1u;
-    for (int i = tid; i < 4 * kSortBins; i += kSortThreads) (&cnt[0][0])[i] = 0;
-    unsigned k[kSortRounds];
-#pragma unroll
-    for (int r = 0; r < kSortRounds; ++r) {
-        const int i = tile_item(tile, w, r, l);
+    for (int i = tid; i < W * kSortBins; i += 64 * W) (&cnt[0][0])[i] = 0;
+    unsigned k[kRounds];
+#pragma unroll
+    for (int r = 0; r < kRounds; ++r) {
+        const int i = tile_item<W>(tile, w, r, l);
         k[r] = i < n ? keys[i] : 0u;
     }
     __syncthreads();
 #pragma unroll
-    for (int r = 0; r < kSortRounds; ++r) {
-        const bool valid = tile_item(tile, w, r, l) < n;
+    for (int r = 0; r < kRounds; ++r) {
+        const bool valid = tile_item<W>(tile, w, r, l) < n;
         const unsigned d = (k[r] >> shift) & mask;
         const unsigned long long peers = digit_peers(d, valid, width);
         if (valid && (peers >> l) == 1ull) cnt[w][d] += __popcll(peers);
         __builtin_amdgcn_wave_barrier();
     }
     __syncthreads();
-    hist[tid * ntile + tile] = cnt[0][tid] + cnt[1][tid] + cnt[2][tid] + cnt[3][tid];
+    if (tid < kSortBins) {
+        int c = 0;
+#pragma unroll
+        for (int j = 0; j < W; ++j) c += cnt[j][tid];
+        hist[tile_major ? tile * kSortBins + tid : tid * ntile + tile] = c;
+    }
 }
 
 __device__ __forceinline__ int wave_incl_scan(int v, int l)
@@ -104,33 +113,50 @@
     if (tid == 0) totals[blockIdx.x] = carry;
 }
 
-__global__ __launch_bounds__(kSortThreads) void sort_scatter_kernel(const unsigned *__restrict__ kin,
-                                                                    const int *__restrict__ vin, int n, int shift,
-                                                                    int width, int ntile, const int *__restrict__ hist,
-                                                                    const int *__restrict__ totals,
-                                                                    unsigned *__restrict__ kout, int *__restrict__ vout)
-{
+template <int W>
+__global__ __launch_bounds__(64 * W) void sort_scatter_kernel(const unsigned *__restrict__ kin,
+                                                              const int *__restrict__ vin, int n, int shift, int width,
+                                                              int ntile, const int *__restrict__ hist,
+                                                              const int *__restrict__ totals,
+                                                              unsigned *__restrict__ kout, int *__restrict__ vout)
+{
+    constexpr int kRounds = 64 / W;
     __shared__ unsigned skey[kSortTile];
     __shared__ int sval[kSortTile];
-    __shared__ int cnt[4][kSortBins];
+    __shared__ int cnt[W][kSortBins];
     __shared__ int goff[kSortBins];
+    static_assert(W * kSortBins <= kSortTile, "the prefix partials fit the staging arrays");
+    int *const ppre = (int *)skey, *const ptot = sval;
     __shared__ int wtot[4], wbase[4];
     const int tid = threadIdx.x, w = tid >> 6, l = tid & 63, tile = blockIdx.x;
     const unsigned mask = (1u << width) - 1u;
-    for (int i = tid; i < 4 * kSortBins; i += kSortThreads) (&cnt[0][0])[i] = 0;
-    unsigned k[kSortRounds];
-    int v[kSortRounds];
-#pragma unroll
-    for (int r = 0; r < kSortRounds; ++r) {
-        const int i = tile_item(tile, w, r, l);
+    for (int i = tid; i < W * kSortBins; i += 64 * W) (&cnt[0][0])[i] = 0;
+    unsigned k[kRounds];
+    int v[kRounds];
+#pragma unroll
+    for (int r = 0; r < kRounds; ++r) {
+        const int i = tile_item<W>(tile, w, r, l);
         k[r] = i < n ? kin[i] : 0u;
         v[r] = i < n ? (vin ? vin[i] : i) : 0;
     }
-    __syncthreads();
-    int rank[kSortRounds];
-#pragma unroll
-    for (int r = 0; r < kSortRounds; ++r) {
-        const bool valid = tile_item(tile, w, r, l) < n;
+    if (!totals) {
+        const int4 *rows = (const int4 *)hist;
+        int4 pre = make_int4(0, 0, 0, 0), tot = pre;
+#pragma unroll 16
+        for (int t = w; t < ntile; t += W) {
+            const int4 h = rows[t * (kSortBins / 4) + l];
+            const int m = t < tile ? -1 : 0;
+            tot.x += h.x, tot.y += h.y, tot.z += h.z, tot.w += h.w;
+            pre.x += h.x & m, pre.y += h.y & m, pre.z += h.z & m, pre.w += h.w & m;
+        }
+        ((int4 *)ppre)[w * (kSortBins / 4) + l] = pre;
+        ((int4 *)ptot)[w * (kSortBins / 4) + l] = tot;
+    }
+    __syncthreads();
+    int rank[kRounds];
+#pragma unroll
+    for (int r = 0; r < kRounds; ++r) {
+        const bool valid = tile_item<W>(tile, w, r, l) < n;
         const unsigned d = (k[r] >> shift) & mask;
         const unsigned long long peers = digit_peers(d, valid, width);
         const int below = __popcll(peers & ((1ull << l) - 1ull));
@@ -140,31 +166,48 @@
         __builtin_amdgcn_wave_barrier();
     }
     __syncthreads();
-    {
-        const int d = tid;
-        const int c0 = cnt[0][d], c1 = cnt[1][d], c2 = cnt[2][d], c3 = cnt[3][d];
-        const int tot = c0 + c1 + c2 + c3, gt = totals[d];
-        const int incl = wave_incl_scan(tot, l), gincl = wave_incl_scan(gt, l);
+    int c[W], tot = 0, gt = 0, hp = 0, incl = 0, gincl = 0;
+    if (tid < kSortBins) {
+#pragma unroll
+        for (int j = 0; j < W; ++j) {
+            c[j] = cnt[j][tid];
+            tot += c[j];
+        }
+        if (totals) {
+            gt = totals[tid];
+            hp = hist[tid * ntile + tile];
+        } else {
+#pragma unroll
+            for (int j = 0; j < W; ++j) {
+                gt += ptot[j * kSortBins + tid];
+                hp += ppre[j * kSortBins + tid];
+            }
+        }
+        incl = wave_incl_scan(tot, l);
+        gincl = wave_incl_scan(gt, l);
         if (l == 63) {
             wtot[w] = incl;
             wbase[w] = gincl;
         }
-        __syncthreads();
+    }
+    __syncthreads();
+    if (tid < kSortBins) {
         int start = incl - tot, gbase = gincl - gt;
         for (int j = 0; j < w; ++j) {
             start += wtot[j];
             gbase += wbase[j];
         }
-        cnt[0][d] = start;
-        cnt[1][d] = start + c0;
-        cnt[2][d] = start + c0 + c1;
-        cnt[3][d] = start + c0 + c1 + c2;
-        goff[d] = gbase + hist[d * ntile + tile] - start;
-    }
-    __syncthreads();
-#pragma unroll
-    for (int r = 0; r < kSortRounds; ++r) {
-        if (tile_item(tile, w, r, l) < n) {
+        goff[tid] = gbase + hp - start;
+#pragma unroll
+        for (int j = 0; j < W; ++j) {
+            cnt[j][tid] = start;
+            start += c[j];
+        }
+    }
+    __syncthreads();
+#pragma unroll
+    for (int r = 0; r < kRounds; ++r) {
+        if (tile_item<W>(tile, w, r, l) < n) {
             const int p = cnt[w][(k[r] >> shift) & mask] + rank[r];
             skey[p] = k[r];
             sval[p] = v[r];
@@ -173,7 +216,7 @@
     __syncthreads();
     const int count = min(kSortTile, n - tile * kSortTile);
 #pragma unroll 4
-    for (int s = tid; s < count; s += kSortThreads) {
+    for (int s = tid; s < count; s += 64 * W) {
         const unsigned key = skey[s];
         const int o = goff[(key >> shift) & mask] + s;
         kout[o] = key;
@@ -182,6 +225,35 @@
 }
 
 size_t al256(size_t b) { return (b + 255) & ~(size_t)255; }
+
+int sort_waves()
+{
+    static const int w = [] {
+        const char *e = getenv("ICP_SORT_WAVES");
+        const int v = e ? atoi(e) : 0;
+        return v == 4 || v == 8 || v == 16 ? v : kSortWavesDefault;
+    }();
+    return w;
+}
+
+int sort_prefix_tiles()
+{
+    static const int t = [] {
+        const char *e = getenv("ICP_SORT_PREFIX");
+        return e ? std::max(0, atoi(e)) : kSortPrefixTiles;
+    }();
+    return t;
+}
+
+template <int W>
+void sort_pass(const unsigned *ki, const int *vi, int n, int shift, int wd, int ntile, bool prefix, int *hist,
+               int *totals, unsigned *ko, int *vo, hipStream_t st)
+{
+    sort_hist_kernel<W><<<ntile, 64 * W, 0, st>>>(ki, n, shift, wd, ntile, prefix ? 1 : 0, hist);
+    if (!prefix) sort_rows_kernel<<<kSortBins, kRowThreads, 0, st>>>(hist, ntile, totals);
+    sort_scatter_kernel<W><<<ntile, 64 * W, 0, st>>>(ki, vi, n, shift, wd, ntile, hist, prefix ? nullptr : totals, ko,
+                                                     vo);
+}
 
 }
 
@@ -204,6 +276,8 @@
     int *hist = (int *)(p + 2 * al256((size_t)n * sizeof(int)));
     int *totals = (int *)((char *)hist + al256((size_t)kSortBins * ntile * sizeof(int)));
     const int width = (bits + npass - 1) / npass;
+    const int W = sort_waves();
+    const bool prefix = ntile <= sort_prefix_tiles();
     const unsigned *ki = k0;
     const int *vi = v0;
     for (int pass = 0; pass < npass; ++pass) {
@@ -211,9 +285,9 @@
         unsigned *ko = to_out ? k1 : tk;
         int *vo = to_out ? v1 : tv;
         const int shift = pass * width, wd = std::min(width, bits - shift);
-        sort_hist_kernel<<<ntile, kSortThreads, 0, st>>>(ki, n, shift, wd, ntile, hist);
-        sort_rows_kernel<<<kSortBins, kRowThreads, 0, st>>>(hist, ntile, totals);
-        sort_scatter_kernel<<<ntile, kSortThreads, 0, st>>>(ki, vi, n, shift, wd, ntile, hist, totals, ko, vo);
+        if (W == 16) sort_pass<16>(ki, vi, n, shift, wd, ntile, prefix, hist, totals, ko, vo, st);
+        else if (W == 8) sort_pass<8>(ki, vi, n, shift, wd, ntile, prefix, hist, totals, ko, vo, st);
+        else sort_pass<4>(ki, vi, n, shift, wd, ntile, prefix, hist, totals, ko, vo, st);
         ki = ko;
         vi = vo;
     }
diff --git a/iterative-closest-point_amd/icp_amd.py b/iterative-closest-point_amd/icp_amd.py
--- a/iterative-closest-point_amd/icp_amd.py
+++ b/iterative-closest-point_amd/icp_amd.py
@@ -47,7 +47,7 @@
     "icp_ensure_model", "icp_subtract_col", "icp_get_indices", "icp_set_index_digest",
     "icp_get_index_digest", "icp_set_cert_audit", "icp_set_run_mode", "icp_set_nn_rule",
     "icp_get_comm_info", "icp_set_bundle_counters", "icp_get_bundle_counters", "icp_get_model_order",
-    "icp_bundle_audit", "icp_sort_pairs",
+    "icp_bundle_audit", "icp_sort_pairs", "icp_get_grid",
     "icp_set_max_distance", "icp_get_inliers", "icp_get_inlier_trace",
 ]
 
@@ -143,6 +143,8 @@
     L.icp_subtract_col.argtypes = [vp, dp, sz, dp, dp]
     L.icp_get_indices.argtypes = [vp, C.POINTER(C.c_int32)]
     L.icp_get_model_order.argtypes = [vp, C.POINTER(C.c_int32)]
+    L.icp_get_grid.argtypes = [vp, C.POINTER(C.c_int), C.POINTER(C.c_double), C.POINTER(C.c_double),
+                               C.POINTER(C.c_int32), C.POINTER(C.c_int32)]
     L.icp_sort_pairs.argtypes = [C.c_int, C.POINTER(C.c_uint32), sz, C.c_int, C.POINTER(C.c_uint32), C.POINTER(C.c_int32)]
     L.icp_set_index_digest.argtypes = [vp, sz]
     L.icp_get_index_digest.argtypes = [vp, C.POINTER(C.c_uint64), sz]
@@ -405,6 +407,18 @@
         self._check(lib().icp_get_model_order(self._h, kd.ctypes.data_as(C.POINTER(C.c_int32))))
         return kd
 
+    def get_grid(self, nm: int) -> dict:
+        g = (C.c_int * 3)()
+        lo = (C.c_double * 3)()
+        inv_h = C.c_double()
+        self._check(lib().icp_get_grid(self._h, g, lo, C.byref(inv_h), None, None))
+        ncell = g[0] * g[1] * g[2]
+        start = np.empty(ncell + 1, dtype=np.int32)
+        order = np.empty(nm, dtype=np.int32)
+        self._check(lib().icp_get_grid(self._h, g, lo, C.byref(inv_h), start.ctypes.data_as(C.POINTER(C.c_int32)),
+                                       order.ctypes.data_as(C.POINTER(C.c_int32))))
+        return dict(g=np.array(g[:]), lo=np.array(lo[:]), inv_h=inv_h.value, start=start, order=order)
+
     def set_index_digest(self, cap: int):
         self._check(lib().icp_set_index_digest(self._h, cap))
         self._digest_cap = cap
```

Result: faster. 10390, median of 6 (+2.4%).
